# ShawnnnLiu/Robust-NeRF

Hardware: AMD Instinct MI355X
Metric: training rays/sec + test PSNR, lego 800² 64c+128f, at 1/2/4/8 MI355X (higher is better)
Workload: dtype bf16; 1 GPU; lego 800x800 hierarchical 64c+128f training step, 4096 rays per GPU; global_batch=4096, num_samples=64, num_samples_fine=128, parallelism=dp1

## Files before the change

include/nerf_hip.h:

```cpp
#ifndef NERF_HIP_H
#define NERF_HIP_H

#include <stddef.h>
#include <stdint.h>

#ifdef __cplusplus
extern "C" {
#endif

#define NR_OK 0
#define NR_EARG (-22)

typedef void* nr_stream_t;

const char* nr_last_error(void);
int nr_abi_version(void);
int nr_probe_fill(float* out, int n, float value, nr_stream_t stream);
int nr_probe_mfma(int kind, const float* A, const float* B, float* D,
                  nr_stream_t stream);

int nr_ray_directions(int H, int W, float focal, float cx, float cy,
                      float* dirs, nr_stream_t stream);

int nr_get_rays(const float* dirs, const float* c2w, int64_t N,
                float* rays_o, float* rays_d, nr_stream_t stream);
int64_t nr_get_rays_bwd_workspace_bytes(void);
int nr_get_rays_bwd(const float* dirs, const float* c2w, int64_t N,
                    const float* g_rays_o, const float* g_rays_d,
                    float* g_dirs, float* g_c2w, void* workspace,
                    nr_stream_t stream);

int nr_rays_from_pixels_fwd(const int64_t* img_idx, const float* pix,
                            const float* poses, int n_img, int H, int W,
                            float focal, int B, float* rays_o, float* rays_d,
                            int* bad_index, nr_stream_t stream);
int nr_rays_from_pixels_bwd(const int64_t* img_idx, const float* pix,
                            const float* poses, int n_img, int H, int W,
                            float focal, int B, const float* g_rays_o,
                            const float* g_rays_d, float* g_poses,
                            nr_stream_t stream);
int nr_check_index_range(const int64_t* idx, int n, int limit, int* flag,
                         nr_stream_t stream);

int nr_se3_poses_fwd(const float* init_poses, const float* rot_deltas,
                     const float* trans_deltas, const int64_t* indices, int n,
                     float* poses_out, nr_stream_t stream);
int nr_se3_poses_bwd(const float* init_poses, const float* rot_deltas,
                     const int64_t* indices, int n, int n_poses,
                     const float* g_poses,
                     int fixed_small_angle, float* g_rot, float* g_trans,
                     nr_stream_t stream);

int nr_gather_rays(const int64_t* idx, int64_t n_rays, int B,
                   const float* rays_o, const float* rays_d, const float* colors,
                   float* out_o, float* out_d, float* out_rgb, int* bad_index,
                   nr_stream_t stream);

int nr_gather_pixels(const int64_t* idx, int n_img, int H, int W,
                     const float* images, int B, int64_t* out_img,
                     float* out_pix, float* out_rgb, int* bad_index,
                     nr_stream_t stream);

int nr_stratified_sample(const float* rays_o, const float* rays_d,
                         const float* t_rand, float near_, float far_,
                         int lindisp, int B, int N, float* z_vals, float* pts,
                         float* viewdirs, nr_stream_t stream);

int nr_positional_encoding(const float* x, int64_t M, int C, int num_freqs,
                           int include_input, int log_sampling, float* out,
                           nr_stream_t stream);
int nr_positional_encoding_bwd(const float* x, int64_t M, int C, int num_freqs,
                               int include_input, int log_sampling,
                               const float* g_out, float* g_x,
                               nr_stream_t stream);

int nr_sample_pdf(const float* bins, const float* weights, const float* u,
                  int B, int Nb, int Ns, float* samples, nr_stream_t stream);

int nr_sample_hierarchical(const float* rays_o, const float* rays_d,
                           const float* z_coarse, const float* w_coarse,
                           const float* u, int B, int Nc, int Nf,
                           float* z_fine, float* pts_fine, float* viewdirs,
                           nr_stream_t stream);

int nr_composite_fwd(const float* rgb, const float* sigma, const float* z,
                     const float* rays_d, const float* sigma_noise, int B,
                     int S, int white_bg, float* rgb_map, float* depth_map,
                     float* acc_map, float* weights, nr_stream_t stream);
int nr_composite_bwd(const float* rgb, const float* sigma, const float* z,
                     const float* rays_d, const float* sigma_noise, int B,
                     int S, int white_bg, const float* g_rgb_map,
                     const float* g_depth, const float* g_acc,
                     const float* g_weights, float* g_rgb, float* g_sigma,
                     float* g_rays_d, nr_stream_t stream);

typedef struct NrMlpConfig {
    int pos_freqs;
    int dir_freqs;
    int hidden;
    int n_layers;
    uint32_t skip_mask;
    int use_view_dirs;
    int precision;
    int dense_backward;
} NrMlpConfig;

#define NR_PREC_FP32 0
#define NR_PREC_BF16 1
#define NR_PREC_FP16 2

int64_t nr_mlp_param_count(const NrMlpConfig* cfg);
int64_t nr_mlp_packed_bytes(const NrMlpConfig* cfg);
int64_t nr_mlp_saved_bytes(const NrMlpConfig* cfg, int64_t M);
int64_t nr_mlp_workspace_bytes(const NrMlpConfig* cfg, int64_t M);

int nr_mlp_pack(const NrMlpConfig* cfg, const float* params, void* packed,
                nr_stream_t stream);

int nr_mlp_forward(const NrMlpConfig* cfg, const void* packed,
                   const float* params, const float* x, const float* d,
                   int64_t M, float* rgb, float* sigma, void* saved,
                   nr_stream_t stream);

int nr_mlp_backward(const NrMlpConfig* cfg, const void* packed,
                    const float* params, const float* x, const float* d,
                    int64_t M, const float* rgb, const float* sigma,
                    const void* saved, const float* g_rgb,
                    const float* g_sigma, float* g_params, float* g_x,
                    float* g_d, void* workspace, nr_stream_t stream);

int nr_mlp_backward_dx(const NrMlpConfig* cfg, const void* packed,
                       const float* params, const float* x, const float* d,
                       int64_t M, const float* rgb, const float* sigma,
                       const void* saved, const float* g_rgb,
                       const float* g_sigma, float* g_x, float* g_d,
                       void* workspace, nr_stream_t stream);
int nr_mlp_backward_dw(const NrMlpConfig* cfg, int64_t M, const void* saved,
                       void* workspace, nr_stream_t stream);
int nr_mlp_backward_reduce(const NrMlpConfig* cfg, int64_t M,
                           const void* workspace, float* g_params,
                           nr_stream_t stream);
int64_t nr_mlp_active_tiles_offset(const NrMlpConfig* cfg, int64_t M);

int64_t nr_sumsq_workspace_bytes(void);
int nr_sumsq(const float* x, int64_t n, float* acc, void* workspace,
             nr_stream_t stream);
int nr_adam_step(float* params, float* grads, float* exp_avg,
                 float* exp_avg_sq, int64_t n, double lr, double beta1,
                 double beta2, double eps, int64_t step, const float* sumsq,
                 float max_norm, nr_stream_t stream);

int nr_sumsq_partials(const float* const* xs, const int64_t* ns, int nspan,
                      float* partials, nr_stream_t stream);
typedef struct NrAdamSpan {
    float* params;
    float* grads;
    float* exp_avg;
    float* exp_avg_sq;
    int64_t n;
    const float* sumsq_partials;
    float max_norm;
    const uint32_t* pack_table;
    void* packed;
} NrAdamSpan;
int nr_adam_multi(const NrAdamSpan* spans, int nspan, double lr, double beta1,
                  double beta2, double eps, int64_t step, const float* sched,
                  nr_stream_t stream);
int64_t nr_mlp_pack_table_bytes(const NrMlpConfig* cfg);
int nr_mlp_pack_table(const NrMlpConfig* cfg, uint32_t* table,
                      nr_stream_t stream);

int nr_expand_viewdirs(const float* rays_d, int B, int S, float* out,
                       nr_stream_t stream);
int nr_pts_bwd(const float* g_pts, const float* z, int B, int S,
               float* g_rays_o, float* g_rays_d, nr_stream_t stream);
int nr_viewdirs_bwd(const float* rays_d, const float* g_viewdirs, int B,
                    int S, float* g_rays_d, nr_stream_t stream);
int nr_mse_fwd_bwd(const float* pred, const float* target, int B, float scale,
                   float* loss_out, float* g_pred, nr_stream_t stream);
int64_t nr_composite_mse_workspace_bytes(int B);
int nr_composite_mse(const float* rgb, const float* sigma, const float* z,
                     const float* rays_d, const float* sigma_noise,
                     const float* target, int B, int S, int white,
                     float grad_scale, float* rgb_map, float* depth_map,
                     float* acc_map, float* weights, float* loss, float* g_rgb,
                     float* g_sigma, float* g_rays_d, uint32_t* ticket,
                     void* workspace, nr_stream_t stream);

int64_t nr_image_metrics_workspace_bytes(int H, int W, int C);
int nr_image_metrics(const float* pred, const float* target, int H, int W, int C,
                     const float* g, double C1, double C2, double* out,
                     void* workspace, nr_stream_t stream);
int nr_frame_u8(const float* src, int H, int W, int C, uint8_t* dst,
                int64_t dst_stride, int dst_x0, nr_stream_t stream);
int64_t nr_depth_frame_u8_workspace_bytes(void);
int nr_depth_frame_u8(const float* depth, int H, int W, uint8_t* dst,
                      void* workspace, nr_stream_t stream);

#ifdef __cplusplus
}
#endif

#endif
```

robust-nerf_amd/csrc/mlp.hip:

```cpp
#include <cmath>
#include <cstring>

#include "mlp_launch.hpp"

#include "mlp_plan.cpp.inc"

using namespace nr;

namespace {

bool plan_or_error(const NrMlpConfig* cfg, MlpPlan* p) {
    const char* why = "";
    if (!make_plan(cfg, p, &why)) {
        set_error("NrMlpConfig unsupported: %s", why);
        return false;
    }
    return true;
}

void add_stream_layer(StreamDesc& sd, int nchunks, int chunk_kb, int load_kb = -1) {
    for (int c = 0; c < nchunks && sd.nq < kMaxChunks; ++c) {
        sd.ckb[sd.nq] = load_kb < 0 ? chunk_kb : load_kb;
        sd.cadv[sd.nq++] = chunk_kb;
    }
}

}

extern "C" {

int64_t nr_mlp_param_count(const NrMlpConfig* cfg) {
    MlpPlan p;
    return plan_or_error(cfg, &p) ? p.param_count : -1;
}

int64_t nr_mlp_packed_bytes(const NrMlpConfig* cfg) {
    MlpPlan p;
    return plan_or_error(cfg, &p) ? p.packed_bytes : -1;
}

int64_t nr_mlp_saved_bytes(const NrMlpConfig* cfg, int64_t M) {
    MlpPlan p;
    if (!plan_or_error(cfg, &p) || M < 0) return -1;
    return make_sizes(p, M).saved_bytes;
}

int64_t nr_mlp_workspace_bytes(const NrMlpConfig* cfg, int64_t M) {
    MlpPlan p;
    if (!plan_or_error(cfg, &p) || M < 0) return -1;
    return make_sizes(p, M).ws_bytes;
}

int nr_mlp_pack(const NrMlpConfig* cfg, const float* params, void* packed, nr_stream_t stream) {
    MlpPlan p;
    if (!plan_or_error(cfg, &p)) return NR_EARG;
    NR_REQUIRE(params && packed, "nr_mlp_pack: null pointer");
    NR_REQUIRE((reinterpret_cast<uintptr_t>(packed) & 15) == 0, "nr_mlp_pack: packed must be 16-byte aligned");
    return launch_pack(p, params, packed, PackIdx{nullptr, 0}, false, static_cast<hipStream_t>(stream));
}

int64_t nr_mlp_pack_table_bytes(const NrMlpConfig* cfg) {
    MlpPlan p;
    return plan_or_error(cfg, &p) ? static_cast<int64_t>(kPackSlots) * p.param_count * 4 : -1;
}

int nr_mlp_pack_table(const NrMlpConfig* cfg, uint32_t* table, nr_stream_t stream) {
    MlpPlan p;
    if (!plan_or_error(cfg, &p)) return NR_EARG;
    NR_REQUIRE(table, "nr_mlp_pack_table: null pointer");
    NR_REQUIRE((reinterpret_cast<uintptr_t>(table) & 15) == 0, "nr_mlp_pack_table: table must be 16-byte aligned");
    NR_REQUIRE(p.packed_bytes < kDstMaxOff, "nr_mlp_pack_table: packed images beyond 512 MB");
    const hipStream_t s = static_cast<hipStream_t>(stream);
    hipError_t e = hipMemsetAsync(table, 0, static_cast<size_t>(kPackSlots) * p.param_count * 4, s);
    if (e != hipSuccess) {
        set_error("nr_mlp_pack_table: %s", hipGetErrorString(e));
        return static_cast<int>(e);
    }
    return launch_pack(p, nullptr, nullptr, PackIdx{table, p.param_count}, true, s);
}

int nr_adam_multi(const NrAdamSpan* spans, int nspan, double lr, double b1, double b2, double eps, int64_t step,
                  const float* sched, nr_stream_t stream) {
    NR_REQUIRE(spans && nspan >= 1 && nspan <= kMaxAdamSpans && step >= 1,
               "nr_adam_multi: bad arguments (1..%d spans, step >= 1)", kMaxAdamSpans);
    AdamMultiArgs a;
    std::memset(&a, 0, sizeof(a));
    int64_t nmax = 0;
    for (int k = 0; k < nspan; ++k) {
        const NrAdamSpan& x = spans[k];
        NR_REQUIRE(x.params && x.grads && x.exp_avg && x.exp_avg_sq && x.n >= 0, "nr_adam_multi: span %d: null buffer", k);
        NR_REQUIRE(((reinterpret_cast<uintptr_t>(x.params) | reinterpret_cast<uintptr_t>(x.grads) |
                     reinterpret_cast<uintptr_t>(x.exp_avg) | reinterpret_cast<uintptr_t>(x.exp_avg_sq) |
                     reinterpret_cast<uintptr_t>(x.pack_table)) & 15) == 0,
                   "nr_adam_multi: span %d: buffers must be 16-byte aligned", k);
        NR_REQUIRE(!x.pack_table || x.packed, "nr_adam_multi: span %d: pack_table without packed", k);
        a.s[k] = AdamSpanDev{x.params, x.grads, x.exp_avg, x.exp_avg_sq, x.n, x.sumsq_partials, x.max_norm,
                             x.pack_table, static_cast<char*>(x.packed)};
        nmax = x.n > nmax ? x.n : nmax;
    }
    if (nmax == 0) return NR_OK;
    const double bc1 = 1.0 - std::pow(b1, static_cast<double>(step));
    const double bc2 = 1.0 - std::pow(b2, static_cast<double>(step));
    a.omb1 = static_cast<float>(1.0 - b1);
    a.b2 = static_cast<float>(b2);
    a.omb2 = static_cast<float>(1.0 - b2);
    a.eps = static_cast<float>(eps);
    a.step_size = static_cast<float>(lr / bc1);
    a.bc2_sqrt = static_cast<float>(std::sqrt(bc2));
    a.sched = sched;
    const int grid = stream_grid(ceil_div_ll(nmax, 4), kSumsqThreads);
    return launch_adam_multi(a, grid, nspan, static_cast<hipStream_t>(stream));
}

int nr_mlp_forward(const NrMlpConfig* cfg, const void* packed, const float* params, const float* x, const float* d,
                   int64_t M, float* rgb, float* sigma, void* saved, nr_stream_t stream) {
    MlpPlan p;
    if (!plan_or_error(cfg, &p)) return NR_EARG;
    NR_REQUIRE(packed && params && x && rgb && sigma && M >= 0, "nr_mlp_forward: null pointer");
    NR_REQUIRE(!p.use_vd || d, "nr_mlp_forward: use_view_dirs needs d (model.py:187-191)");
    NR_REQUIRE((reinterpret_cast<uintptr_t>(saved) & 15) == 0, "nr_mlp_forward: saved must be 16-byte aligned");
    NR_REQUIRE((reinterpret_cast<uintptr_t>(packed) & 15) == 0, "nr_mlp_forward: packed must be 16-byte aligned");
    if (M == 0) return NR_OK;
    const MlpSizes z = make_sizes(p, M);
    const hipStream_t s = static_cast<hipStream_t>(stream);
    if (p.prec != NR_PREC_FP32) {
        RbmArgs r;
        std::memset(&r, 0, sizeof(r));
        r.packed = static_cast<const char*>(packed);
        r.params = params;
        r.x = x;
        r.d = d;
        r.rgb = rgb;
        r.sigma = sigma;
        r.saved = static_cast<char*>(saved);
        r.M = M;
        r.tiles = z.tiles;
        r.L = p.L;
        r.Ld = p.Ld;
        r.n_layers = p.n_layers;
        r.skips = p.skips;
        r.base = p.lin[0].pk_fwd;
        r.vhead = p.vhead;
        r.sig_b = p.sig_b;
        r.rgb_b = p.rgb_b;
        for (int t = 0; t < p.n_saved; ++t) r.sv_off[t] = z.saved_off[t];
        r.sv_feat = p.sv_feat;
        r.sv_denc = p.sv_denc;
        r.sv_hc = p.sv_hc;
        r.mask_off = z.mask_off;
        r.n_mask = p.n_mask;
        return launch_fwd_rbm(p, r, saved != nullptr, s);
    }
    FwdArgs a;
    std::memset(&a, 0, sizeof(a));
    a.packed = static_cast<const char*>(packed);
    a.params = params;
    a.x = x;
    a.d = d;
    a.rgb = rgb;
    a.sigma = sigma;
    a.saved = static_cast<char*>(saved);
    a.M = M;
    a.tiles = z.tiles;
    a.L = p.L;
    a.Ld = p.Ld;
    a.n_layers = p.n_layers;
    a.skips = p.skips;
    a.sd.base = p.lin[0].pk_fwd;
    for (int l = 0; l < p.n_lin; ++l) {
        const LinearDesc& dl = p.lin[l];
        add_stream_layer(a.sd, dl.KB, dl.NB * p.fpb);
        a.vb[l] = dl.vb;
        a.bo[l] = dl.b_off;
    }
    a.vsig = p.vsig;
    a.vrgb = p.vrgb;
    a.sig_b = p.sig_b;
    a.rgb_b = p.rgb_b;
    for (int t = 0; t < p.n_saved; ++t) a.sv_off[t] = z.saved_off[t];
    a.sv_feat = p.sv_feat;
    a.sv_denc = p.sv_denc;
    a.sv_hc = p.sv_hc;
    a.mask_off = z.mask_off;
    a.n_mask = p.n_mask;
    return launch_fwd(p, a, saved != nullptr, s);
}

int nr_mlp_backward_dx(const NrMlpConfig* cfg, const void* packed, const float* params, const float* x,
                       const float* d, int64_t M, const float* rgb, const float* sigma, const void* saved,
                       const float* g_rgb, const float* g_sigma, float* g_x, float* g_d, void* workspace,
                       nr_stream_t stream) {
    MlpPlan p;
    if (!plan_or_error(cfg, &p)) return NR_EARG;
    NR_REQUIRE(packed && params && x && rgb && sigma && saved && g_rgb && g_sigma && workspace && M >= 0,
               "nr_mlp_backward_dx: null pointer");
    NR_REQUIRE(!g_d || (d && p.use_vd), "nr_mlp_backward_dx: g_d needs d and use_view_dirs");
    NR_REQUIRE((reinterpret_cast<uintptr_t>(workspace) & 15) == 0,
               "nr_mlp_backward_dx: workspace must be 16-byte aligned");
    if (M == 0) return NR_OK;
    const hipStream_t s = static_cast<hipStream_t>(stream);
    const MlpSizes z = make_sizes(p, M);
    NR_REQUIRE(z.tiles_alloc < (int64_t{1} << 32), "nr_mlp_backward_dx: M beyond 2^37 samples");
    char* wsb = static_cast<char*>(workspace);
    uint8_t* tflags = reinterpret_cast<uint8_t*>(wsb + z.flags_off);
    uint32_t* blkcnt = reinterpret_cast<uint32_t*>(wsb + z.blkcnt_off);
    uint32_t* dwlist = reinterpret_cast<uint32_t*>(wsb + z.dwlist_off);
    uint32_t* tcount = reinterpret_cast<uint32_t*>(wsb + z.count_off);
    if (const int rc = launch_tile_flags(g_rgb, g_sigma, M, p.dense_bwd, z.nseg, tflags, blkcnt, s)) return rc;
    const int n = p.n_layers;
    if (p.prec != NR_PREC_FP32) {
        BwdrArgs r;
        std::memset(&r, 0, sizeof(r));
        r.gscale = grad_scale(p.prec);
        r.packed = static_cast<const char*>(packed);
        r.rgb = rgb;
        r.sigma = sigma;
        r.g_rgb = g_rgb;
        r.g_sigma = g_sigma;
        r.saved = static_cast<const char*>(saved);
        r.ws = wsb;
        r.M = M;
        r.tiles = z.tiles;
        r.flags = tflags;
        r.blk_count = blkcnt;
        r.nseg = z.nseg;
        r.dw_list = dwlist;
        r.count = tcount;
        r.scratch_base = z.tiles_alloc - kScratchTiles;
        r.n_layers = n;
        r.base = p.lin[n + 1].pk_bwdr;
        r.vrgb = p.vrgb;
        r.vhead = p.vhead;
        r.mask_off = z.mask_off;
        r.n_mask = p.n_mask;
        for (int t = 0; t < p.n_ws; ++t) r.ws_off[t] = z.ws_off[t];
        r.ws_feat = p.ws_feat;
        r.ws_dir = p.ws_dir;
        r.ws_heads = p.ws_heads;
        const int rc = launch_bwd_rbm(p, r, s);
        if (rc != NR_OK || !(g_x || g_d)) return rc;
        return input_grads16(p, z, r.packed, x, d, g_x, g_d, wsb, M, s);
    }
    const bool wx = g_x != nullptr || g_d != nullptr;
    BwdArgs b;
    std::memset(&b, 0, sizeof(b));
    b.packed = static_cast<const char*>(packed);
    b.gscale = grad_scale(p.prec);
    b.inv_gscale = 1.0f / b.gscale;
    b.params = params;
    b.x = x;
    b.d = d;
    b.rgb = rgb;
    b.sigma = sigma;
    b.g_rgb = g_rgb;
    b.g_sigma = g_sigma;
    b.g_x = g_x;
    b.g_d = g_d;
    b.saved = static_cast<const char*>(saved);
    b.ws = wsb;
    b.M = M;
    b.tiles = z.tiles;
    b.flags = tflags;
    b.blk_count = blkcnt;
    b.nseg = z.nseg;
    b.dw_list = dwlist;
    b.count = tcount;
    b.L = p.L;
    b.Ld = p.Ld;
    b.n_layers = n;
    b.skips = p.skips;
    auto add_T = [&](int l) {
        const bool partial = !wx && ((l > 0 && l < n && is_skip(p, l - 1)) || l == n + 1);
        add_stream_layer(b.sd, p.lin[l].NB, p.lin[l].KB * p.fpb, partial ? kHB * p.fpb : -1);
    };
    b.sd.base = p.lin[n + 1].pk_bwd;
    add_T(n + 1);
    add_T(n);
    for (int i = n - 1; i >= 1; --i) add_T(i);
    if (wx) add_T(0);
    b.vsig = p.vsig;
    b.vrgb = p.vrgb;
    b.mask_off = z.mask_off;
    b.n_mask = p.n_mask;
    for (int t = 0; t < p.n_ws; ++t) b.ws_off[t] = z.ws_off[t];
    b.ws_feat = p.ws_feat;
    b.ws_dir = p.ws_dir;
    b.ws_heads = p.ws_heads;
    if (!p.dense_bwd) {
        for (float* g : {g_x, g_d})
            if (g) {
                const hipError_t e = hipMemsetAsync(g, 0, sizeof(float) * 3 * static_cast<size_t>(M), s);
                if (e != hipSuccess) {
                    set_error("nr_mlp_backward_dx: %s", hipGetErrorString(e));
                    return static_cast<int>(e);
                }
            }
    }
    return launch_bwd(p, b, wx, s);
}

int nr_mlp_backward_dw(const NrMlpConfig* cfg, int64_t M, const void* saved, void* workspace, nr_stream_t stream) {
    MlpPlan p;
    if (!plan_or_error(cfg, &p)) return NR_EARG;
    NR_REQUIRE(saved && workspace && M >= 0, "nr_mlp_backward_dw: null pointer");
    NR_REQUIRE((reinterpret_cast<uintptr_t>(saved) & 15) == 0 && (reinterpret_cast<uintptr_t>(workspace) & 15) == 0,
               "nr_mlp_backward_dw: saved and workspace must be 16-byte aligned");
    if (M == 0) return NR_OK;
    const hipStream_t s = static_cast<hipStream_t>(stream);
    const MlpSizes z = make_sizes(p, M);
    const char* sv = static_cast<const char*>(saved);
    char* ws = static_cast<char*>(workspace);
    DwArgs w;
    std::memset(&w, 0, sizeof(w));
    w.slabs = reinterpret_cast<float*>(ws + z.slab_off);
    w.tiles = z.tiles;
    w.list = reinterpret_cast<const uint32_t*>(ws + z.dwlist_off);
    w.count = reinterpret_cast<const uint32_t*>(ws + z.count_off);
    w.njobs = p.n_jobs;
    int nwg = 0;
    NR_REQUIRE(p.n_jobs <= 32 && z.max_chunks < 2048, "nr_mlp_backward_dw: %d jobs x %d chunks beyond the map",
               p.n_jobs, z.max_chunks);
    for (int c = 0; c < z.max_chunks; ++c)
        for (int j = 0; j < p.n_jobs; ++j)
            if (c < z.job_chunks[j]) {
                NR_REQUIRE(nwg < kDwMaxWgs, "nr_mlp_backward_dw: more than %d workgroups", kDwMaxWgs);
                w.wg_map[nwg++] = static_cast<uint16_t>(j | c << 5);
            }
    for (int j = 0; j < p.n_jobs; ++j) w.job_chunks[j] = z.job_chunks[j];
    w.slab_floats_per_chunk = p.slab_floats_per_chunk;
    int max_blk = 0;
    for (int j = 0; j < p.n_jobs; ++j) {
        const DwJob& jb = p.job[j];
        w.job_NBz[j] = jb.NBz;
        w.job_KB[j] = jb.KB;
        for (int v = 0; v < kDwWaves; ++v) {
            if (v >= jb.nwaves) {
                w.job_wave[j][v] = 0;
                continue;
            }
            const DwWave& sh = jb.w[v];
            NR_REQUIRE(sh.np >= 1 && sh.np <= kDwMaxP && sh.nq >= 1 && sh.nq <= kDwMaxQ && sh.row0 >= 0 &&
                           sh.row0 + sh.np <= jb.NBz && sh.col0 >= 0 && sh.col0 + sh.nq <= jb.KB && jb.NBz < 64 &&
                           jb.KB < 64,
                       "nr_mlp_backward_dw: job %d wave %d share out of its %dx%d grid", j, v, jb.NBz, jb.KB);
            w.job_wave[j][v] = dw_wave_pack(sh.row0, sh.np, sh.col0, sh.nq, sh.bias);
        }
        int ns = 0;
        for (int q = 0; q < jb.ndz; ++q, ++ns) {
            w.seg_ptr[j][ns] = (jb.dz[q].is_ws ? ws : sv) + (jb.dz[q].is_ws ? z.ws_off : z.saved_off)[jb.dz[q].tensor];
            w.seg_blocks[j][ns] = static_cast<uint8_t>(jb.dz[q].blocks);
        }
        for (int q = 0; q < jb.nin; ++q, ++ns) {
            w.seg_ptr[j][ns] = (jb.in[q].is_ws ? ws : sv) + (jb.in[q].is_ws ? z.ws_off : z.saved_off)[jb.in[q].tensor];
            w.seg_blocks[j][ns] = static_cast<uint8_t>(jb.in[q].blocks);
        }
        w.job_slab[j] = jb.slab_off;
        NR_REQUIRE((jb.NBz + jb.KB) * p.fpb <= kDwWaves * dw_max_pieces(p.fpb == 2),
                   "nr_mlp_backward_dw: job %d stages %d blocks, beyond the kernel's per-wave pieces", j, jb.NBz + jb.KB);
        max_blk = jb.NBz + jb.KB > max_blk ? jb.NBz + jb.KB : max_blk;
    }
    w.stage_bytes = max_blk * p.fpb * kFragBytes;
    w.nstage = static_cast<int>((160 * 1024 - kFragBytes) / w.stage_bytes);
    if (w.nstage > NR_DW_NSTAGE) w.nstage = NR_DW_NSTAGE;
    size_t lds = static_cast<size_t>(w.nstage) * w.stage_bytes + kFragBytes;
    int min_chunks = z.job_chunks[0];
    for (int j = 1; j < p.n_jobs; ++j) min_chunks = z.job_chunks[j] < min_chunks ? z.job_chunks[j] : min_chunks;
    const size_t list_bytes = (static_cast<size_t>(ceil_div_ll(z.tiles, min_chunks)) * 4 + 15) / 16 * 16;
    if (lds + list_bytes <= 160 * 1024) {
        w.list_lds = static_cast<int>(lds);
        lds += list_bytes;
    }
    NR_REQUIRE(w.nstage >= 2, "nr_mlp_backward_dw: a %d-byte stage does not fit twice in LDS", w.stage_bytes);
    NR_REQUIRE(lds <= 160 * 1024, "nr_mlp_backward_dw: %zu bytes of LDS staging exceeds 160 KiB", lds);
    return launch_dw(p.prec, w, nwg, lds, s);
}

int nr_mlp_backward_reduce(const NrMlpConfig* cfg, int64_t M, const void* workspace, float* g_params,
                           nr_stream_t stream) {
    MlpPlan p;
    if (!plan_or_error(cfg, &p)) return NR_EARG;
    NR_REQUIRE(workspace && g_params && M >= 0, "nr_mlp_backward_reduce: null pointer");
    const hipStream_t s = static_cast<hipStream_t>(stream);
    if (M == 0) {
        (void)hipMemsetAsync(g_params, 0, sizeof(float) * p.param_count, s);
        return check_launch("nr_mlp_backward_reduce");
    }
    const MlpSizes z = make_sizes(p, M);
    ReduceArgs r;
    std::memset(&r, 0, sizeof(r));
    r.slabs = reinterpret_cast<const float*>(static_cast<const char*>(workspace) + z.slab_off);
    r.g = g_params;
    r.inv_gscale = 1.0f / grad_scale(p.prec);
    r.param_count = p.param_count;
    r.slab_floats_per_chunk = p.slab_floats_per_chunk;
    r.n_red = p.n_red;
    for (int k = 0; k < p.n_red; ++k) {
        const ReduceRange& rr = p.red[k];
        r.rows[k] = rr.rows;
        r.in[k] = rr.in;
        r.nseg[k] = rr.nseg;
        r.bjob[k] = rr.bjob;
        r.brow0[k] = rr.brow0;
        r.w_off[k] = rr.w_off;
        r.b_off[k] = rr.b_off;
        for (int q = 0; q < rr.nseg; ++q) r.seg[k][q] = rr.seg[q];
    }
    for (int j = 0; j < p.n_jobs; ++j) {
        r.job_slab[j] = p.job[j].slab_off;
        r.job_KB[j] = p.job[j].KB;
        r.job_chunks[j] = z.job_chunks[j];
    }
    int max_rows = 1;
    for (int k = 0; k < p.n_red; ++k) max_rows = p.red[k].rows > max_rows ? p.red[k].rows : max_rows;
    return launch_dw_reduce(r, max_rows, s);
}

int64_t nr_mlp_active_tiles_offset(const NrMlpConfig* cfg, int64_t M) {
    MlpPlan p;
    if (!plan_or_error(cfg, &p) || M <= 0) return -1;
    return make_sizes(p, M).count_off;
}

int nr_mlp_backward(const NrMlpConfig* cfg, const void* packed, const float* params, const float* x, const float* d,
                    int64_t M, const float* rgb, const float* sigma, const void* saved, const float* g_rgb,
                    const float* g_sigma, float* g_params, float* g_x, float* g_d, void* workspace,
                    nr_stream_t stream) {
    NR_REQUIRE(g_params, "nr_mlp_backward: null g_params");
    int rc = nr_mlp_backward_dx(cfg, packed, params, x, d, M, rgb, sigma, saved, g_rgb, g_sigma, g_x, g_d, workspace,
                                stream);
    if (rc) return rc;
    rc = nr_mlp_backward_dw(cfg, M, saved, workspace, stream);
    if (rc) return rc;
    return nr_mlp_backward_reduce(cfg, M, workspace, g_params, stream);
}

}
```

robust-nerf_amd/csrc/mlp_16.hip:

```cpp
#include <algorithm>
#include <cstring>

#include "mlp_dev.hpp"
#include "mlp_launch.hpp"

namespace nr {

#include "mlp_fwd_rbm.inc"
#include "mlp_bwd_rbm.inc"

struct DinArgs {
    const char* packed;
    const char* ws;
    const float* x;
    const float* d;
    float* g_x;
    float* g_d;
    int64_t M, tiles;
    const uint8_t* flags;
    int L, Ld;
    float inv_gscale;
    int nsrc;
    int64_t a_off[kMaxTrunk];
    int a_kb[kMaxTrunk];
    int a_p0[kMaxTrunk];
    int64_t dz_off[kMaxTrunk];
    int64_t dir_a_off, dz_dir_off;
    int dir_kb, dir_p0, nc;
};

constexpr int kDinNT = 512;

__host__ __device__ inline int din_frags(int nsrc, int XB, int DB, int nc) { return 2 * (nsrc * kHB * XB + nc * DB); }

template <int PREC, int XB, int DB, bool ALDS>
__global__ __launch_bounds__(kDinNT) void mlp_dinput_kernel(DinArgs a) {
    static_assert(k16<PREC>, "16-bit images only");
    extern __shared__ __attribute__((aligned(16))) char lds[];
    const int lane = threadIdx.x & 63, h = lane >> 5, ml = lane & 31;
    auto frag_src = [&](int f) -> const char* {
        const int nx = 2 * a.nsrc * kHB * XB;
        if (f < nx) {
            const int s = f / (2 * kHB * XB), r = f % (2 * kHB * XB);
            const int ob = r / (2 * XB), q = r % (2 * XB);
            return a.packed + a.a_off[s] + static_cast<int64_t>((ob * a.a_kb[s] + a.a_p0[s]) * 2 + q) * kFragBytes;
        }
        const int r = f - nx, ob = r / (2 * DB > 0 ? 2 * DB : 1), q = r % (2 * DB > 0 ? 2 * DB : 1);
        return a.packed + a.dir_a_off + static_cast<int64_t>((ob * a.dir_kb + a.dir_p0) * 2 + q) * kFragBytes;
    };
    if constexpr (ALDS) {
        const int nf = din_frags(a.nsrc, XB, DB, a.nc);
        for (int i = threadIdx.x; i < nf * 64; i += kDinNT) {
            const int f = i >> 6, l = i & 63;
            *reinterpret_cast<u32x4*>(lds + f * kFragBytes + l * 16) =
                *reinterpret_cast<const u32x4*>(frag_src(f) + l * 16);
        }
        __syncthreads();
    }
    auto afrag = [&](int f) -> bf16x8 {
        if constexpr (ALDS)
            return *reinterpret_cast<const bf16x8*>(lds + f * kFragBytes + lane * 16);
        else
            return *reinterpret_cast<const bf16x8*>(frag_src(f) + lane * 16);
    };
    const int64_t waves = static_cast<int64_t>(gridDim.x) * (kDinNT / 64);
    for (int64_t tile = static_cast<int64_t>(blockIdx.x) * (kDinNT / 64) + (threadIdx.x >> 6); tile < a.tiles;
         tile += waves) {
        const int64_t tile_u = __builtin_amdgcn_readfirstlane(static_cast<int>(tile));
        const int64_t m = tile * 32 + ml;
        const bool valid = m < a.M;
        if (!a.flags[tile_u]) {
            if (valid && h == 0)
#pragma unroll
                for (int c = 0; c < 3; ++c) {
                    if (a.g_x) a.g_x[3 * m + c] = 0.f;
                    if (a.g_d) a.g_d[3 * m + c] = 0.f;
                }
            continue;
        }
        if (a.g_x) {
            f32x16 dxe[XB];
#pragma unroll
            for (int q = 0; q < XB; ++q) zero(dxe[q]);
            for (int s = 0; s < a.nsrc; ++s) {
                InBlk<PREC> b[kHB];
#pragma unroll
                for (int ob = 0; ob < kHB; ++ob) load_img<PREC>(a.ws + a.dz_off[s], tile_u, kHB, ob, b[ob], lane);
#pragma unroll
                for (int ob = 0; ob < kHB; ++ob)
#pragma unroll
                    for (int q = 0; q < XB; ++q) {
                        const int f = ((s * kHB + ob) * XB + q) * 2;
                        dxe[q] = mfma16<PREC>(afrag(f), b[ob].s[0], dxe[q]);
                        dxe[q] = mfma16<PREC>(afrag(f + 1), b[ob].s[1], dxe[q]);
                    }
            }
            const PeRev pr = pe_rev(valid ? a.x[3 * m] : 0.f, valid ? a.x[3 * m + 1] : 0.f,
                                    valid ? a.x[3 * m + 2] : 0.f);
            float g0 = 0.f, g1 = 0.f, g2 = 0.f;
#pragma unroll
            for (int kb = 0; kb < XB; ++kb)
#pragma unroll
                for (int r = 0; r < 16; ++r)
                    pe_fast_bwd(pr, 32 * kb + acc_row(r, 0), 32 * kb + acc_row(r, 1), h != 0, a.L, dxe[kb][r], g0, g1,
                                g2);
            g0 += __shfl_xor(g0, 32);
            g1 += __shfl_xor(g1, 32);
            g2 += __shfl_xor(g2, 32);
            if (valid && h == 0) {
                a.g_x[3 * m] = g0 * a.inv_gscale;
                a.g_x[3 * m + 1] = g1 * a.inv_gscale;
                a.g_x[3 * m + 2] = g2 * a.inv_gscale;
            }
        }
        if constexpr (DB > 0) {
            if (a.g_d) {
                f32x16 dd[DB];
#pragma unroll
                for (int q = 0; q < DB; ++q) zero(dd[q]);
                const int f0 = 2 * a.nsrc * kHB * XB;
                for (int ob = 0; ob < a.nc; ++ob) {
                    InBlk<PREC> b;
                    load_img<PREC>(a.ws + a.dz_dir_off, tile_u, a.nc, ob, b, lane);
#pragma unroll
                    for (int q = 0; q < DB; ++q) {
                        const int f = f0 + (ob * DB + q) * 2;
                        dd[q] = mfma16<PREC>(afrag(f), b.s[0], dd[q]);
                        dd[q] = mfma16<PREC>(afrag(f + 1), b.s[1], dd[q]);
                    }
                }
                const PeRev pr = pe_rev(valid ? a.d[3 * m] : 0.f, valid ? a.d[3 * m + 1] : 0.f,
                                        valid ? a.d[3 * m + 2] : 0.f);
                float g0 = 0.f, g1 = 0.f, g2 = 0.f;
#pragma unroll
                for (int kb = 0; kb < DB; ++kb)
#pragma unroll
                    for (int r = 0; r < 16; ++r)
                        pe_fast_bwd(pr, 32 * kb + acc_row(r, 0), 32 * kb + acc_row(r, 1), h != 0, a.Ld, dd[kb][r], g0,
                                    g1, g2);
                g0 += __shfl_xor(g0, 32);
                g1 += __shfl_xor(g1, 32);
                g2 += __shfl_xor(g2, 32);
                if (valid && h == 0) {
                    a.g_d[3 * m] = g0 * a.inv_gscale;
                    a.g_d[3 * m + 1] = g1 * a.inv_gscale;
                    a.g_d[3 * m + 2] = g2 * a.inv_gscale;
                }
            }
        }
    }
}

namespace {

template <int PREC, bool TRAIN>
int launch_fwd_rbm_t(const MlpPlan& p, const RbmArgs& a, hipStream_t s) {
    constexpr int W = kRbmWaves;
    const dim3 grid(static_cast<unsigned>(ceil_div_ll(a.tiles, W))), block(W * 64);
    const size_t lds = rbm_lds_bytes(p.XB, W);
#define NR_FWDR(XB_, DB_)                                                                           \
    if (p.XB == XB_ && p.DB == DB_) {                                                               \
        hipLaunchKernelGGL((mlp_fwd_rbm_kernel<PREC, XB_, DB_, TRAIN, W>), grid, block, lds, s, a); \
        return check_launch("nr_mlp_forward");                                                      \
    }
    NR_FWDR(2, 1)
#ifndef NR_MLP_DEV
    NR_FWDR(2, 0)
    NR_FWDR(1, 1)
    NR_FWDR(1, 0)
#endif
#undef NR_FWDR
    set_error("nr_mlp_forward: no kernel instance for XB=%d DB=%d", p.XB, p.DB);
    return NR_EARG;
}

template <int PREC>
int launch_bwd_rbm_t(const MlpPlan& p, const BwdrArgs& a, hipStream_t s) {
    constexpr int W = kRbmWaves;
    const size_t lds = bwdr_lds_bytes(p.n_mask, W);
    if (lds > 160 * 1024) {
        set_error("nr_mlp_backward_dx: %zu bytes of LDS exceed 160 KiB", lds);
        return NR_EARG;
    }
    const dim3 grid(static_cast<unsigned>(a.nseg * (kSegTiles / W))), block(W * 64);
    hipLaunchKernelGGL((mlp_bwd_rbm_kernel<PREC, W>), grid, block, lds, s, a);
    return check_launch("nr_mlp_backward_dx");
}

template <int PREC>
int launch_dinput(const MlpPlan& p, const DinArgs& a, hipStream_t s) {
    const size_t lds = static_cast<size_t>(din_frags(a.nsrc, p.XB, p.DB, a.nc)) * kFragBytes;
    const bool alds = lds <= 160 * 1024;
    const dim3 grid(static_cast<unsigned>(std::min<int64_t>(ceil_div_ll(a.tiles, kDinNT / 64), 512))),
        block(kDinNT);
#define NR_DIN(XB_, DB_)                                                                                  \
    if (p.XB == XB_ && p.DB == DB_) {                                                                     \
        if (alds)                                                                                         \
            hipLaunchKernelGGL((mlp_dinput_kernel<PREC, XB_, DB_, true>), grid, block, lds, s, a);        \
        else                                                                                              \
            hipLaunchKernelGGL((mlp_dinput_kernel<PREC, XB_, DB_, false>), grid, block, 0, s, a);         \
        return check_launch("nr_mlp_backward_dx (input gradients)");                                     \
    }
    NR_DIN(2, 1)
#ifndef NR_MLP_DEV
    NR_DIN(2, 0)
    NR_DIN(1, 1)
    NR_DIN(1, 0)
#endif
#undef NR_DIN
    set_error("nr_mlp_backward_dx: no input-gradient kernel for XB=%d DB=%d", p.XB, p.DB);
    return NR_EARG;
}

}

int launch_fwd_rbm(const MlpPlan& p, const RbmArgs& a, bool train, hipStream_t s) {
    if (p.prec == NR_PREC_BF16)
        return train ? launch_fwd_rbm_t<NR_PREC_BF16, true>(p, a, s) : launch_fwd_rbm_t<NR_PREC_BF16, false>(p, a, s);
    return train ? launch_fwd_rbm_t<NR_PREC_FP16, true>(p, a, s) : launch_fwd_rbm_t<NR_PREC_FP16, false>(p, a, s);
}

int launch_bwd_rbm(const MlpPlan& p, const BwdrArgs& a, hipStream_t s) {
    return p.prec == NR_PREC_BF16 ? launch_bwd_rbm_t<NR_PREC_BF16>(p, a, s) : launch_bwd_rbm_t<NR_PREC_FP16>(p, a, s);
}

int input_grads16(const MlpPlan& p, const MlpSizes& z, const char* packed, const float* x, const float* d, float* g_x,
                  float* g_d, const char* ws, int64_t M, hipStream_t s) {
    const int n = p.n_layers;
    DinArgs da;
    std::memset(&da, 0, sizeof(da));
    da.packed = packed;
    da.ws = ws;
    da.flags = reinterpret_cast<const uint8_t*>(ws + z.flags_off);
    da.x = x;
    da.d = d;
    da.g_x = g_x;
    da.g_d = g_d;
    da.M = M;
    da.tiles = z.tiles;
    da.L = p.L;
    da.Ld = p.Ld;
    da.inv_gscale = 1.0f / grad_scale(p.prec);
    for (int l = 0; l < n; ++l) {
        if (l > 0 && !is_skip(p, l - 1)) continue;
        da.a_off[da.nsrc] = p.lin[l].pk_bwd;
        da.a_kb[da.nsrc] = p.lin[l].KB;
        da.a_p0[da.nsrc] = p.lin[l].KB - p.XB;
        da.dz_off[da.nsrc] = z.ws_off[WS_DZ0 + l];
        da.nsrc++;
    }
    da.dir_a_off = p.lin[n + 1].pk_bwd;
    da.dir_kb = p.lin[n + 1].KB;
    da.dir_p0 = kHB;
    da.nc = p.lin[n + 1].NB;
    da.dz_dir_off = z.ws_off[p.ws_dir];
    return p.prec == NR_PREC_BF16 ? launch_dinput<NR_PREC_BF16>(p, da, s) : launch_dinput<NR_PREC_FP16>(p, da, s);
}

}
```

robust-nerf_amd/csrc/mlp_bwd_rbm.inc:

```

constexpr int kBwdrSlot = 32 * 1024;
__host__ __device__ constexpr int bwdr_mask_off() { return 2 * kBwdrSlot; }
__host__ __device__ constexpr int bwdr_sig_off(int n_mask, int W) { return 2 * kBwdrSlot + W * n_mask * 1024; }
__host__ __device__ constexpr int bwdr_lds_bytes(int n_mask, int W) { return bwdr_sig_off(n_mask, W) + 1024; }

template <int PREC>
struct BwdrTrunkFin {
    InBlk<PREC> (&out)[kHB];
    u32x4 mw;
    char* dst;
    int64_t tile;
    int& nvm;
    bool sig;
    float dzs;
    const float* wsig;
    __device__ __forceinline__ void operator()(int rb, f32x16& a, const bf16x8&) const {
        if (sig)
#pragma unroll
            for (int g = 0; g < 4; ++g) {
                const f32x4 w = *reinterpret_cast<const f32x4*>(wsig + rb * 32 + 4 * g);
#pragma unroll
                for (int e = 0; e < 4; ++e) a[4 * g + e] = fmaf(w[e], dzs, a[4 * g + e]);
            }
        to_in_masked<PREC>(a, mw, rb, out[rb]);
        store_img<PREC>(dst, tile, kHB, rb, out[rb], 0);
        nvm += 2;
    }
};

template <int PREC>
struct BwdrFeatFin {
    InBlk<PREC> (&out)[kHB];
    char* dst;
    int64_t tile;
    int& nvm;
    __device__ __forceinline__ void operator()(int rb, f32x16& a, const bf16x8&) const {
        to_in<PREC>(a, out[rb]);
        store_img<PREC>(dst, tile, kHB, rb, out[rb], 0);
        nvm += 2;
    }
};

template <int PREC, int W>
__global__ __launch_bounds__(W * 64, 1) void mlp_bwd_rbm_kernel(BwdrArgs a) {
    static_assert(kSegTiles % W == 0, "whole parts per segment");
    extern __shared__ __attribute__((aligned(16))) char lds[];
    const int tid = threadIdx.x, lane = tid & 63, h = lane >> 5, ml = lane & 31;
    const int wv = __builtin_amdgcn_readfirstlane(tid >> 6);
    const TileSel ts = select_tile(a.flags, a.blk_count, a.nseg, a.tiles, W, wv);
    if (ts.idle) {
        finish_tiles(ts, a.nseg, a.tiles, a.dw_list, a.count);
        return;
    }
    const int64_t tile = ts.live ? ts.tile : a.scratch_base + ((blockIdx.x * W + wv) & (kScratchTiles - 1));
    const int64_t m = tile * 32 + ml;
    const bool valid = m < a.M;
    const int n = a.n_layers;
    constexpr int NC = kHB / 2;

    char* mlds = lds + bwdr_mask_off() + wv * a.n_mask * 1024;
    const char* msrc = a.saved + a.mask_off + tile * a.n_mask * 1024;
    for (int l = 0; l < a.n_mask; ++l)
        __builtin_amdgcn_global_load_lds((const __attribute__((address_space(1))) void*)(msrc + l * 1024 + lane16()),
                                         (__attribute__((address_space(3))) void*)(mlds + l * 1024), 16, 0, 0);
    if (wv == 0)
        __builtin_amdgcn_global_load_lds(
            (const __attribute__((address_space(1))) void*)(a.packed + a.vhead + lane16()),
            (__attribute__((address_space(3))) void*)(lds + bwdr_sig_off(a.n_mask, W)), 16, 0, 0);
    const u32x4 mwc = *reinterpret_cast<const u32x4*>(msrc + n * 1024 + lane16());
    auto mask_of = [&](int layer) { return *reinterpret_cast<const u32x4*>(mlds + layer * 1024 + lane16()); };
    const float* wsig = reinterpret_cast<const float*>(lds + bwdr_sig_off(a.n_mask, W)) + 16 * h;

    RStream s{lds, a.packed + a.base, -1, 0, wv, kBwdrSlot, W};
    constexpr int CK_DIR = rbm_chunk_kb(NC, 0), CK_H = rbm_chunk_kb(kHB, 0);
    static_assert(CK_DIR * 1024 <= kBwdrSlot && CK_H * 1024 <= kBwdrSlot, "dX chunk");
    rbm_dma(s, CK_DIR);
    s.q = 0;

    float dr[3] = {0.f, 0.f, 0.f}, dzs = 0.f;
    if (valid) {
#pragma unroll
        for (int c = 0; c < 3; ++c) {
            const float y = a.rgb[3 * m + c];
            dr[c] = ((a.g_rgb[3 * m + c] * (1.0f - y)) * y) * a.gscale;
        }
        dzs = (a.sigma[m] > 0.f ? a.g_sigma[m] : 0.f) * a.gscale;
    }
    {
        f32x16 hb;
        zero(hb);
        if (h == 0) {
            hb[0] = dzs;
            hb[1] = dr[0];
            hb[2] = dr[1];
            hb[3] = dr[2];
        }
        InBlk<PREC> hv;
        to_in<PREC>(hb, hv);
        store_img<PREC>(a.ws + a.ws_off[a.ws_heads], tile, 1, 0, hv, 0);
        s.nvm += 2;
    }
    InBlk<PREC> cin[NC];
    {
        const PImg wr0 = pimg(a.packed, a.vrgb), wr1 = pimg(a.packed, a.vrgb + NC * 128),
                   wr2 = pimg(a.packed, a.vrgb + 2 * NC * 128);
#pragma unroll
        for (int nb = 0; nb < NC; ++nb) {
            f32x16 dc;
#pragma unroll
            for (int r = 0; r < 16; ++r) {
                f32x2 v = wr0.at(nb, r) * bcast2(dr[0]);
                v = __builtin_elementwise_fma(wr1.at(nb, r), bcast2(dr[1]), v);
                v = __builtin_elementwise_fma(wr2.at(nb, r), bcast2(dr[2]), v);
                dc[r] = h ? v[1] : v[0];
            }
            to_in_masked<PREC>(dc, mwc, nb, cin[nb]);
            store_img<PREC>(a.ws + a.ws_off[a.ws_dir], tile, NC, nb, cin[nb], 0);
            s.nvm += 2;
        }
    }

    InBlk<PREC> hA[kHB], hB[kHB];
    {
        BwdrFeatFin<PREC> fin{hA, a.ws + a.ws_off[a.ws_feat], tile, s.nvm};
        auto in = [&](int kb) -> const InBlk<PREC>& { return cin[kb]; };
        rbm_layer<PREC, NC, kHB, 0, decltype(in), decltype(fin), 0>(s, CK_H, in, fin);
    }
    {
        BwdrTrunkFin<PREC> fin{hB, mask_of(n - 1), a.ws + a.ws_off[WS_DZ0 + n - 1], tile, s.nvm, true, dzs, wsig};
        auto in = [&](int kb) -> const InBlk<PREC>& { return hA[kb]; };
        rbm_layer<PREC, kHB, kHB, 0, decltype(in), decltype(fin), 0>(s, n > 1 ? CK_H : 0, in, fin);
    }
    auto trunk = [&](int i, InBlk<PREC>(&hin)[kHB], InBlk<PREC>(&hout)[kHB]) {
        BwdrTrunkFin<PREC> fin{hout, mask_of(i - 1), a.ws + a.ws_off[WS_DZ0 + i - 1], tile, s.nvm, false, 0.f, wsig};
        auto in = [&](int kb) -> const InBlk<PREC>& { return hin[kb]; };
        rbm_layer<PREC, kHB, kHB, 0, decltype(in), decltype(fin), 0>(s, i > 1 ? CK_H : 0, in, fin);
    };
    for (int i = n - 1; i >= 1; i -= 2) {
        trunk(i, hB, hA);
        if (i == 1) break;
        trunk(i - 1, hA, hB);
    }
    finish_tiles(ts, a.nseg, a.tiles, a.dw_list, a.count);
}
```

robust-nerf_amd/csrc/mlp_dev.hpp:

```cpp
#pragma once

#include <type_traits>
#include <utility>

#include "common.hpp"
#include "mfma.hpp"
#include "mlp_plan.hpp"

namespace nr {

template <int PREC>
constexpr bool k16 = PREC != NR_PREC_FP32;

template <int PREC>
struct InBlk {
    bf16x8 s[2];
};
template <>
struct InBlk<NR_PREC_FP32> {
    f32x16 v;
};

template <int PREC>
constexpr int kFPB = k16<PREC> ? 2 : 4;

typedef _Float16 f16x8 __attribute__((ext_vector_type(8)));
typedef _Float16 f16x2 __attribute__((ext_vector_type(2)));

template <int PREC>
__device__ __forceinline__ f32x16 mfma16(bf16x8 a, bf16x8 b, f32x16 c) {
    if constexpr (PREC == NR_PREC_FP16)
        return __builtin_amdgcn_mfma_f32_32x32x16_f16(__builtin_bit_cast(f16x8, a), __builtin_bit_cast(f16x8, b), c,
                                                      0, 0, 0);
    else
        return mfma_bf16(a, b, c);
}

typedef float f32x2 __attribute__((ext_vector_type(2)));
typedef __bf16 bf16x2 __attribute__((ext_vector_type(2)));
__device__ __forceinline__ unsigned cvt_pk_bf16(float lo, float hi) {
    return __builtin_bit_cast(unsigned, __builtin_convertvector(f32x2{lo, hi}, bf16x2));
}
template <int PREC>
__device__ __forceinline__ unsigned cvt_pk16(float lo, float hi) {
    if constexpr (PREC == NR_PREC_FP16)
        return __builtin_bit_cast(unsigned, __builtin_convertvector(f32x2{lo, hi}, f16x2));
    else
        return cvt_pk_bf16(lo, hi);
}
template <int PREC>
__device__ __forceinline__ float from16_lo(unsigned w) {
    if constexpr (PREC == NR_PREC_FP16)
        return static_cast<float>(__builtin_bit_cast(f16x2, w)[0]);
    else
        return __uint_as_float(w << 16);
}

template <int PREC = NR_PREC_BF16>
__device__ __forceinline__ bf16x8 pack8(const f32x16& a, int hf) {
    u32x4 w;
#pragma unroll
    for (int m = 0; m < 4; ++m) w[m] = cvt_pk16<PREC>(a[8 * hf + 2 * m], a[8 * hf + 2 * m + 1]);
    return __builtin_bit_cast(bf16x8, w);
}

template <int PREC>
__device__ __forceinline__ void to_in(const f32x16& a, InBlk<PREC>& o) {
    if constexpr (k16<PREC>) {
        o.s[0] = pack8<PREC>(a, 0);
        o.s[1] = pack8<PREC>(a, 1);
    } else {
        o.v = a;
    }
}

__device__ __forceinline__ void zero(f32x16& a) {
#pragma unroll
    for (int r = 0; r < 16; ++r) a[r] = 0.f;
}

#ifndef NR_SIN
#define NR_SIN sinf
#define NR_COS cosf
#endif
__device__ __forceinline__ uint32_t lane16() {
    uint32_t v;
    asm volatile("v_mbcnt_lo_u32_b32 %0, -1, 0\n\tv_mbcnt_hi_u32_b32 %0, -1, %0\n\tv_lshlrev_b32 %0, 4, %0" : "=v"(v));
    return v;
}

__device__ __forceinline__ float pe_feat(float x0, float x1, float x2, int f, int L) {
    if (f < 3) return f == 0 ? x0 : (f == 1 ? x1 : x2);
    const int fp = f - 3;
    const int k = fp / 6;
    if (k >= L) return 0.f;
    const int rem = fp - 6 * k;
    const int c = rem % 3;
    const float xv = c == 0 ? x0 : (c == 1 ? x1 : x2);
    const float v = exp2f(static_cast<float>(k)) * xv;
    return rem < 3 ? NR_SIN(v) : NR_COS(v);
}

__device__ __forceinline__ void pe_feat_bwd(float x0, float x1, float x2, int f, int L, float g, float& g0,
                                            float& g1, float& g2) {
    int c;
    float d;
    if (f < 3) {
        c = f;
        d = g;
    } else {
        const int fp = f - 3;
        const int k = fp / 6;
        if (k >= L) return;
        const int rem = fp - 6 * k;
        c = rem % 3;
        const float xv = c == 0 ? x0 : (c == 1 ? x1 : x2);
        const float fr = exp2f(static_cast<float>(k));
        const float v = fr * xv;
        d = rem < 3 ? (g * cosf(v)) * fr : (g * -sinf(v)) * fr;
    }
    g0 += c == 0 ? d : 0.f;
    g1 += c == 1 ? d : 0.f;
    g2 += c == 2 ? d : 0.f;
}

struct PeRev {
    float x[3], hi[3], lo[3];
};

__device__ __forceinline__ PeRev pe_rev(float x0, float x1, float x2) {
    constexpr float C1 = 0.15915494f, C2 = 6.4206382e-09f;
    PeRev p;
    const float xs[3] = {x0, x1, x2};
#pragma unroll
    for (int c = 0; c < 3; ++c) {
        p.x[c] = xs[c];
        p.hi[c] = xs[c] * C1;
        p.lo[c] = fmaf(xs[c], C1, -p.hi[c]) + xs[c] * C2;
    }
    return p;
}

__device__ __forceinline__ float pe_fast(const PeRev& p, int f0, int f1, bool h1, int L) {
    auto kind = [](int f) { return f < 3 ? 0 : 1; };
    auto trig = [&](int f, float& hi, float& lo) {
        const int fp = f - 3, k = fp / 6, rem = fp - 6 * k, c = rem % 3;
        const float sc = static_cast<float>(1 << (k < 24 ? k : 0));
        hi = p.hi[c] * sc;
        lo = fmaf(p.lo[c], sc, rem < 3 ? 0.f : 0.25f);
        return k < L;
    };
    if (kind(f0) == 1 && kind(f1) == 1) {
        float h0, l0, hh, lh;
        const bool v0 = trig(f0, h0, l0), v1 = trig(f1, hh, lh);
        const float hi = h1 ? hh : h0, lo = h1 ? lh : l0;
        const float v = __builtin_amdgcn_sinf(__builtin_amdgcn_fractf(hi) + lo);
        return (h1 ? v1 : v0) ? v : 0.f;
    }
    auto one = [&](int f) -> float {
        if (f < 3) return p.x[f];
        float hi, lo;
        const bool ok = trig(f, hi, lo);
        return ok ? __builtin_amdgcn_sinf(__builtin_amdgcn_fractf(hi) + lo) : 0.f;
    };
    const float a0 = one(f0), a1 = one(f1);
    return h1 ? a1 : a0;
}

__device__ __forceinline__ void pe_fast_bwd(const PeRev& p, int f0, int f1, bool h1, int L, float g, float& g0,
                                            float& g1, float& g2) {
    auto chan = [](int f) { return f < 3 ? f : ((f - 3) - 6 * ((f - 3) / 6)) % 3; };
    auto sel = [](const float (&v)[3], int c) { return c == 0 ? v[0] : (c == 1 ? v[1] : v[2]); };
    auto live = [&](int f) { return f < 3 || (f - 3) / 6 < L; };
    auto dgamma = [&](int f) -> float {
        const int fp = f - 3, k = fp / 6, rem = fp - 6 * k, c = rem % 3;
        const float sc = static_cast<float>(1 << (k < 24 ? k : 0));
        const float hi = sel(p.hi, c) * sc, lo = fmaf(sel(p.lo, c), sc, rem < 3 ? 0.25f : 0.5f);
        return __builtin_amdgcn_sinf(__builtin_amdgcn_fractf(hi) + lo) * sc;
    };
    float d;
    if (f0 >= 3 && f1 >= 3) {
        const int fp0 = f0 - 3, k0 = fp0 / 6, r0 = fp0 - 6 * k0;
        const int fp1 = f1 - 3, k1 = fp1 / 6, r1 = fp1 - 6 * k1;
        const float s0 = static_cast<float>(1 << (k0 < 24 ? k0 : 0)), s1 = static_cast<float>(1 << (k1 < 24 ? k1 : 0));
        const float hi = h1 ? sel(p.hi, r1 % 3) * s1 : sel(p.hi, r0 % 3) * s0;
        const float lo = h1 ? fmaf(sel(p.lo, r1 % 3), s1, r1 < 3 ? 0.25f : 0.5f) : fmaf(sel(p.lo, r0 % 3), s0, r0 < 3 ? 0.25f : 0.5f);
        d = g * (__builtin_amdgcn_sinf(__builtin_amdgcn_fractf(hi) + lo) * (h1 ? s1 : s0));
    } else {
        const float a0 = f0 < 3 ? 1.f : (live(f0) ? dgamma(f0) : 0.f);
        const float a1 = f1 < 3 ? 1.f : (live(f1) ? dgamma(f1) : 0.f);
        d = g * (h1 ? a1 : a0);
    }
    if (!(h1 ? live(f1) : live(f0))) return;
    const int c = h1 ? chan(f1) : chan(f0);
    g0 += c == 0 ? d : 0.f;
    g1 += c == 1 ? d : 0.f;
    g2 += c == 2 ? d : 0.f;
}

template <int PREC>
__device__ __forceinline__ bf16x8 bias_frag(float b) {
    const unsigned w0 = cvt_pk16<PREC>(b, 0.f);
    const float r1 = b - from16_lo<PREC>(w0);
    const unsigned w1 = cvt_pk16<PREC>(r1, 0.f);
    const float r2 = r1 - from16_lo<PREC>(w1);
    const unsigned w2 = cvt_pk16<PREC>(r2, 0.f);
    return __builtin_bit_cast(bf16x8, u32x4{w0 | (w1 << 16), w2, 0u, 0u});
}

template <int PREC>
__device__ __forceinline__ bf16x8 ones16() {
    const unsigned one = PREC == NR_PREC_FP16 ? 0x3C003C00u : 0x3F803F80u;
    return __builtin_bit_cast(bf16x8, u32x4{one, one, one, one});
}

typedef short s16x2 __attribute__((ext_vector_type(2)));
typedef unsigned short u16x2 __attribute__((ext_vector_type(2)));

__device__ __forceinline__ unsigned relu_pk(unsigned w) {
    return __builtin_bit_cast(unsigned, __builtin_elementwise_max(__builtin_bit_cast(s16x2, w), s16x2{0, 0}));
}
__device__ __forceinline__ unsigned nz_pk(unsigned w) {
    unsigned r;
    asm("v_pk_min_u16 %0, %1, %2" : "=v"(r) : "v"(w), "s"(0x10001u));
    return r;
}

template <int PREC, bool RELU, bool MASK>
__device__ __forceinline__ void epi16_blk(const f32x16& a, bf16x8 (&out)[2], unsigned* mw, int nb) {
#pragma unroll
    for (int hf = 0; hf < 2; ++hf) {
        u32x4 wd = __builtin_bit_cast(u32x4, pack8<PREC>(a, hf));
#pragma unroll
        for (int m = 0; m < 4; ++m) {
            if constexpr (RELU) wd[m] = relu_pk(wd[m]);
            if constexpr (MASK) mw[nb >> 1] |= nz_pk(wd[m]) << (8 * (nb & 1) + 4 * hf + m);
        }
        out[hf] = __builtin_bit_cast(bf16x8, wd);
    }
}

__device__ __forceinline__ void mask_pk(bf16x8 (&v)[2], unsigned word, int nb) {
#pragma unroll
    for (int hf = 0; hf < 2; ++hf) {
        u32x4 wd = __builtin_bit_cast(u32x4, v[hf]);
#pragma unroll
        for (int m = 0; m < 4; ++m) {
            const unsigned t = (word >> (8 * (nb & 1) + 4 * hf + m)) & 0x10001u;
            wd[m] &= t * 0xFFFFu;
        }
        v[hf] = __builtin_bit_cast(bf16x8, wd);
    }
}

template <int PREC>
__device__ __forceinline__ void to_in_masked(f32x16 a, const u32x4& mw, int nb, InBlk<PREC>& o) {
    if constexpr (k16<PREC>) {
        to_in<PREC>(a, o);
        mask_pk(o.s, mw[nb >> 1], nb);
    } else {
#pragma unroll
        for (int r = 0; r < 16; ++r) {
            const unsigned bit = (mw[nb >> 1] >> ((nb & 1) * 16 + r)) & 1u;
            a[r] = bit ? a[r] : 0.f;
        }
        o.v = a;
    }
}

template <int PREC>
__device__ __forceinline__ void store_img(char* __restrict__ region, int64_t tile, int nblk, int blk,
                                          const InBlk<PREC>& v, int) {
    char* base = region + ((tile * nblk + blk) * kFPB<PREC>) * static_cast<int64_t>(kFragBytes) + lane16();
    if constexpr (k16<PREC>) {
        __builtin_nontemporal_store(__builtin_bit_cast(u32x4, v.s[0]), reinterpret_cast<u32x4*>(base));
        __builtin_nontemporal_store(__builtin_bit_cast(u32x4, v.s[1]), reinterpret_cast<u32x4*>(base + kFragBytes));
    } else {
#pragma unroll
        for (int tq = 0; tq < 4; ++tq)
            *reinterpret_cast<f32x4*>(base + tq * kFragBytes) =
                f32x4{v.v[4 * tq], v.v[4 * tq + 1], v.v[4 * tq + 2], v.v[4 * tq + 3]};
    }
}

template <int PREC>
__device__ __forceinline__ void load_img(const char* __restrict__ region, int64_t tile, int nblk, int blk,
                                         InBlk<PREC>& v, int) {
    const char* base = region + ((tile * nblk + blk) * kFPB<PREC>) * static_cast<int64_t>(kFragBytes) + lane16();
    if constexpr (k16<PREC>) {
        v.s[0] = *reinterpret_cast<const bf16x8*>(base);
        v.s[1] = *reinterpret_cast<const bf16x8*>(base + kFragBytes);
    } else {
#pragma unroll
        for (int tq = 0; tq < 4; ++tq) {
            const f32x4 q = *reinterpret_cast<const f32x4*>(base + tq * kFragBytes);
#pragma unroll
            for (int e = 0; e < 4; ++e) v.v[4 * tq + e] = q[e];
        }
    }
}

typedef const __attribute__((address_space(4))) float cfloat;

struct VImg {
    cfloat* p;
    bool hi;
    __device__ __forceinline__ f32x4 g4(int nb, int g) const {
        f32x4 r;
#pragma unroll
        for (int e = 0; e < 4; ++e) {
            const float lo = p[(2 * nb) * 16 + 4 * g + e], up = p[(2 * nb + 1) * 16 + 4 * g + e];
            r[e] = hi ? up : lo;
        }
        return r;
    }
};

__device__ __forceinline__ VImg vimg(const char* packed, int64_t off, int lane) {
    const char* q = packed + off;
    asm volatile("" : "+s"(q));
    return VImg{(cfloat*)(q), (lane >> 5) != 0};
}
#define NR_VEC(img, nb, g) ((img).g4((nb), (g)))

typedef const __attribute__((address_space(4))) f32x2 cf32x2;
struct PImg {
    cf32x2* p;
    __device__ __forceinline__ f32x2 at(int nb, int r) const { return p[nb * 16 + r]; }
};
__device__ __forceinline__ PImg pimg(const char* packed, int64_t off) {
    const char* q = packed + off;
    asm volatile("" : "+s"(q));
    return PImg{(cf32x2*)(q)};
}
__device__ __forceinline__ f32x2 bcast2(float x) { return f32x2{x, x}; }
__device__ __forceinline__ float relu_f(float x) { return __int_as_float(max(__float_as_int(x), 0)); }

struct SegFlags {
    uint32_t word;
    int count, incl, total;
};
__device__ __forceinline__ uint32_t seg_flag_word(const uint8_t* __restrict__ flags, int64_t sg) {
    static_assert(kSegTiles == 4 * 64, "one flag word per lane");
    return reinterpret_cast<const uint32_t*>(flags + sg * kSegTiles)[threadIdx.x & 63];
}
__device__ __forceinline__ SegFlags seg_scan(uint32_t word) {
    const int lane = threadIdx.x & 63;
    SegFlags f;
    f.word = word;
    f.count = __popc(f.word);
    f.incl = f.count;
#pragma unroll
    for (int d = 1; d < 64; d <<= 1) {
        const int o = __shfl_up(f.incl, d);
        if (lane >= d) f.incl += o;
    }
    f.total = __builtin_amdgcn_readfirstlane(__shfl(f.incl, 63));
    return f;
}

__device__ __forceinline__ int64_t seg_entry(const SegFlags& f, int64_t sg, int k) {
    const uint64_t over = __ballot(f.incl > k);
    const int L = __builtin_ctzll(over);
    const uint32_t w = __builtin_amdgcn_readfirstlane(__shfl(f.word, L));
    int r = k - __builtin_amdgcn_readfirstlane(__shfl(f.incl - f.count, L));
    int b = 0;
#pragma unroll
    for (int q = 0; q < 4; ++q) {
        const bool set = (w >> (8 * q)) & 1u;
        if (set && r == 0) b = q;
        r -= set ? 1 : 0;
        if (r < 0) r = 1 << 20;
    }
    return sg * kSegTiles + 4 * L + b;
}

__device__ __forceinline__ void place_segment(const SegFlags& f, uint32_t before, int64_t nseg, int64_t sg,
                                              uint32_t* __restrict__ list, uint32_t* __restrict__ count) {
    const int lane = threadIdx.x & 63;
    uint32_t slot = before + static_cast<uint32_t>(f.incl - f.count);
#pragma unroll
    for (int q = 0; q < 4; ++q)
        if ((f.word >> (8 * q)) & 1u) list[slot++] = static_cast<uint32_t>(sg * kSegTiles + 4 * lane + q);
    if (sg == nseg - 1 && lane == 0) *count = before + static_cast<uint32_t>(f.total);
}

constexpr int64_t kDenseCheckSegs = 1024;

struct TileSel {
    SegFlags sf;
    int64_t seg, tile;
    uint32_t before;
    bool dense, live, idle, leader;
};
__device__ __forceinline__ TileSel select_tile(const uint8_t* __restrict__ flags,
                                               const uint32_t* __restrict__ blk_count, int64_t nseg,
                                               int64_t tiles, int W, int wv) {
    constexpr int BPS = kSegTiles / 64;
    const int lane = threadIdx.x & 63;
    const int64_t b = blockIdx.x;
    TileSel t;
    const int part = static_cast<int>(b / nseg);
    t.seg = (b % nseg + nseg - part % nseg) % nseg;
    static_assert(BPS == 4, "a segment's block counts are one uint4");
    const bool check = nseg <= kDenseCheckSegs;
    const int64_t lim = check ? nseg : (part == 0 && wv == 0 ? t.seg : 0);
    const uint32_t word = seg_flag_word(flags, t.seg);
    const uint4* __restrict__ bc4 = reinterpret_cast<const uint4*>(blk_count);
    uint32_t all = 0, before = 0;
    for (int64_t s0 = 0; s0 < lim; s0 += 4 * 64) {
        uint4 c[4];
#pragma unroll
        for (int i = 0; i < 4; ++i) {
            const int64_t sg = s0 + i * 64 + lane;
            c[i] = sg < lim ? bc4[sg] : uint4{0u, 0u, 0u, 0u};
        }
#pragma unroll
        for (int i = 0; i < 4; ++i) {
            const uint32_t n = ((c[i].x + c[i].y) + c[i].z) + c[i].w;
            all += n;
            before += (s0 + i * 64 + lane) < t.seg ? n : 0u;
        }
    }
    t.sf = seg_scan(word);
#pragma unroll
    for (int d = 32; d > 0; d >>= 1) {
        all += __shfl_xor(all, d);
        before += __shfl_xor(before, d);
    }
    t.before = __builtin_amdgcn_readfirstlane(before);
    t.dense = check && static_cast<int64_t>(__builtin_amdgcn_readfirstlane(all)) == tiles;
    if (t.dense) {
        const int64_t first = b * W;
        t.tile = first + wv;
        t.live = t.tile < tiles;
        t.idle = first >= tiles;
        t.leader = b == 0 && wv == 0;
    } else {
        const int k = part * W + wv;
        t.idle = part * W >= t.sf.total;
        t.live = k < t.sf.total;
        t.tile = t.live ? seg_entry(t.sf, t.seg, k) : 0;
        t.leader = part == 0 && wv == 0;
    }
    return t;
}

__device__ __forceinline__ void finish_tiles(const TileSel& t, int64_t nseg, int64_t tiles, uint32_t* __restrict__ list,
                                             uint32_t* __restrict__ count) {
    if (!t.leader) return;
    if (t.dense) {
        if ((threadIdx.x & 63) == 0) *count = static_cast<uint32_t>(tiles);
    } else {
        place_segment(t.sf, t.before, nseg, t.seg, list, count);
    }
}

template <int... Js, class F>
__device__ __forceinline__ void rbm_static_for(std::integer_sequence<int, Js...>, F&& f) {
    (f(std::integral_constant<int, Js>{}), ...);
}
template <int NN, class F>
__device__ __forceinline__ void rbm_static_for(F&& f) {
    rbm_static_for(std::make_integer_sequence<int, NN>{}, f);
}

}
```

robust-nerf_amd/csrc/mlp_dw.hip:

```cpp
#include "mlp_dev.hpp"
#include "mlp_launch.hpp"

namespace nr {

constexpr int kTileFlagThreads = 256;

__global__ __launch_bounds__(kTileFlagThreads) void tile_flags_kernel(const float* __restrict__ g_rgb,
                                                                      const float* __restrict__ g_sigma, int64_t M,
                                                                      int dense,
                                                                      uint8_t* __restrict__ flags,
                                                                      uint32_t* __restrict__ blk_count) {
    __shared__ uint32_t wcnt[kTileFlagThreads / 64];
    const int lane = threadIdx.x & 63, wv = threadIdx.x >> 6;
    const int64_t tw = static_cast<int64_t>(blockIdx.x) * 64 + wv * 16;
    bool nz[8];
#pragma unroll
    for (int it = 0; it < 8; ++it) {
        const int64_t m = (tw + 2 * it + (lane >> 5)) * 32 + (lane & 31);
        bool v = false;
        if (m < M) {
            if (dense) {
                v = true;
            } else {
                const float r0 = g_rgb[3 * m], r1 = g_rgb[3 * m + 1], r2 = g_rgb[3 * m + 2], s0 = g_sigma[m];
                v = (r0 != 0.f) | (r1 != 0.f) | (r2 != 0.f) | (s0 != 0.f);
            }
        }
        nz[it] = v;
    }
    uint32_t mask = 0;
#pragma unroll
    for (int it = 0; it < 8; ++it) {
        const uint64_t b = __ballot(nz[it]);
        mask |= (static_cast<uint32_t>(b & 0xffffffffull) != 0 ? 1u : 0u) << (2 * it);
        mask |= (static_cast<uint32_t>(b >> 32) != 0 ? 1u : 0u) << (2 * it + 1);
    }
    if (lane < 16) flags[tw + lane] = static_cast<uint8_t>((mask >> lane) & 1u);
    if (lane == 0) wcnt[wv] = __popc(mask);
    __syncthreads();
    if (threadIdx.x == 0) blk_count[blockIdx.x] = ((wcnt[0] + wcnt[1]) + wcnt[2]) + wcnt[3];
}

#ifndef NR_DW_AUX
#define NR_DW_AUX 0
#endif

__device__ __forceinline__ int dw_feat(int r) { return acc_row(r & 15, r >> 4); }

__device__ __forceinline__ int dw_slot(int L, int s) { return L ^ (((L >> 5) & 1) << 2) ^ (s << 3); }
__device__ __forceinline__ int dw_slot32(int L, int f) { return L ^ (2 * (f + 4 * ((L >> 5) & 1))); }

template <int OFF>
__device__ __forceinline__ void tr16(uint64_t& out, uint32_t addr) {
    asm volatile("ds_read_b64_tr_b16 %0, %1 offset:%2" : "=v"(out) : "v"(addr), "i"(OFF));
}

typedef unsigned long long u64x2_t __attribute__((ext_vector_type(2)));
template <int OFF>
__device__ __forceinline__ void ds_rd32(float& out, uint32_t addr) {
    asm volatile("ds_read_b32 %0, %1 offset:%2" : "=v"(out) : "v"(addr), "i"(OFF));
}

__device__ __forceinline__ bf16x8 tr_pair(uint64_t lo, uint64_t hi) {
    return __builtin_bit_cast(bf16x8, u64x2_t{lo, hi});
}

__device__ __forceinline__ uint32_t dw_tr_off(int ks, int half, int lane) {
    const int g = lane >> 4, h = g & 1, hh = g >> 1;
    const int lam = lane & 15, q = lam >> 2, p = lam & 3;
    const int s = p >> 1;
    const int L = 16 * ks + 8 * hh + q + 32 * h + 4 * half;
    return static_cast<uint32_t>(s * kFragBytes + dw_slot(L, s) * 16 + 8 * (p & 1));
}

template <int PREC>
__device__ __forceinline__ float dw_acc4(uint64_t v, float acc) {
    const unsigned w0 = static_cast<unsigned>(v), w1 = static_cast<unsigned>(v >> 32);
    if constexpr (PREC == NR_PREC_FP16) {
        typedef _Float16 h2 __attribute__((ext_vector_type(2)));
        const h2 one = __builtin_bit_cast(h2, 0x3c003c00u);
        acc = __builtin_amdgcn_fdot2(__builtin_bit_cast(h2, w0), one, acc, false);
        return __builtin_amdgcn_fdot2(__builtin_bit_cast(h2, w1), one, acc, false);
    } else {
        typedef __bf16 b2 __attribute__((ext_vector_type(2)));
        const b2 one = __builtin_bit_cast(b2, 0x3f803f80u);
        acc = __builtin_amdgcn_fdot2_f32_bf16(__builtin_bit_cast(b2, w0), one, acc, false);
        return __builtin_amdgcn_fdot2_f32_bf16(__builtin_bit_cast(b2, w1), one, acc, false);
    }
}

template <int PREC>
__global__ __launch_bounds__(kDwThreads, 1) void mlp_dw_kernel(DwArgs a) {
    extern __shared__ __attribute__((aligned(16))) char lds[];
    const int tid = threadIdx.x, lane = tid & 63;
    const int wv = __builtin_amdgcn_readfirstlane(tid >> 6);
    const int wmap = a.wg_map[blockIdx.x];
    const int j = wmap & 31, chunk = wmap >> 5;
    const int NBz = a.job_NBz[j], KB = a.job_KB[j];
    const int winfo = a.job_wave[j][wv];
    const int row0 = winfo & 63, np = (winfo >> 6) & 7, col0 = (winfo >> 9) & 63, nq = (winfo >> 15) & 3;
    const bool active = np > 0;
    const bool do_bias = active && ((winfo >> 17) & 1);
    const int64_t cnt = *a.count;
    const int64_t tpc = (cnt + a.job_chunks[j] - 1) / a.job_chunks[j];
    const int64_t t0 = static_cast<int64_t>(chunk) * tpc;
    int64_t t1 = t0 + tpc;
    if (t1 > cnt) t1 = cnt;
    constexpr int FPB = kFPB<PREC>;
    constexpr int BLK = FPB * kFragBytes;

    const int total = (NBz + KB) * FPB;
    const int per_wave = (total + kDwWaves - 1) / kDwWaves;
    constexpr int kMaxPW = dw_max_pieces(k16<PREC>);
    const char* psrc[kMaxPW];
    int64_t pstride[kMaxPW];
    int pdst[kMaxPW];
#pragma unroll
    for (int k = 0; k < kMaxPW; ++k) {
        psrc[k] = nullptr;
        pstride[k] = 0;
        pdst[k] = -1;
        if (k < per_wave) {
            int pc = wv + k * kDwWaves;
            const bool pad = pc >= total;
            if (pad) pc = 0;
            int sg = 0, p0 = 0;
            while (pc >= p0 + a.seg_blocks[j][sg] * FPB) p0 += a.seg_blocks[j][sg++] * FPB;
            const int nb = a.seg_blocks[j][sg];
            const int L = k16<PREC> ? dw_slot(lane, (pc - p0) % FPB) : dw_slot32(lane, (pc - p0) % FPB);
            pstride[k] = static_cast<int64_t>(nb) * BLK;
            psrc[k] = a.seg_ptr[j][sg] + (pc - p0) * kFragBytes + L * 16;
            pdst[k] = pad ? -1 : pc * kFragBytes;
        }
    }
    const uint32_t* lds_list = nullptr;
    if (a.list_lds && cnt != a.tiles) {
        uint32_t* dst = reinterpret_cast<uint32_t*>(lds + a.list_lds);
        for (int64_t q = t0 + tid; q < t1; q += kDwThreads) dst[q - t0] = a.list[q];
        __syncthreads();
        lds_list = dst;
    }
    const bool ident = cnt == a.tiles;
    const uint32_t list_base = static_cast<uint32_t>(reinterpret_cast<uintptr_t>(lds_list));
    auto tile_at = [&](int64_t pos) -> int64_t {
        if (ident) return pos;
        if (!lds_list) return a.list[pos];
        uint32_t v;
        asm volatile("ds_read_b32 %0, %1\n\ts_waitcnt lgkmcnt(0)"
                     : "=v"(v)
                     : "v"(list_base + 4u * static_cast<uint32_t>(pos - t0))
                     : "memory");
        return __builtin_amdgcn_readfirstlane(v);
    };
    auto stage = [&](int b, int64_t tile) {
        char* dst = lds + b * a.stage_bytes;
        char* scratch = lds + a.nstage * a.stage_bytes;
#pragma unroll
        for (int k = 0; k < kMaxPW; ++k) {
            if (k < per_wave) {
                char* d = pdst[k] < 0 ? scratch : dst + pdst[k];
                __builtin_amdgcn_global_load_lds(
                    (const __attribute__((address_space(1))) void*)(psrc[k] + tile * pstride[k]),
                    (__attribute__((address_space(3))) void*)(d), 16, 0, NR_DW_AUX);
            }
        }
    };
    auto wait_pieces = [](int n) {
        switch (n) {
            case 4: asm volatile("s_waitcnt vmcnt(4)" ::: "memory"); break;
            case 5: asm volatile("s_waitcnt vmcnt(5)" ::: "memory"); break;
            case 8: asm volatile("s_waitcnt vmcnt(8)" ::: "memory"); break;
            case 10: asm volatile("s_waitcnt vmcnt(10)" ::: "memory"); break;
            default: asm volatile("s_waitcnt vmcnt(0)" ::: "memory"); break;
        }
    };

    uint32_t trof[2][2];
#pragma unroll
    for (int ks = 0; ks < 2; ++ks)
#pragma unroll
        for (int hf = 0; hf < 2; ++hf) trof[ks][hf] = dw_tr_off(ks, hf, lane);
    const int NS = a.nstage;
    float* slab = a.slabs + static_cast<int64_t>(chunk) * a.slab_floats_per_chunk + a.job_slab[j];
    const int ld = KB * 32 + 1;
    const int hl = lane >> 5, ml = lane & 31;

    using std::integral_constant;
    auto run = [&](auto npc, auto nqc) {
        constexpr int NP = decltype(npc)::value, NQ = decltype(nqc)::value;
        f32x16 acc[NP][NQ];
#pragma unroll
        for (int p = 0; p < NP; ++p)
#pragma unroll
            for (int q = 0; q < NQ; ++q) zero(acc[p][q]);
        float bsum[NP];
#pragma unroll
        for (int p = 0; p < NP; ++p) bsum[p] = 0.f;
        bool nval[NP], kval[NQ];
#pragma unroll
        for (int p = 0; p < NP; ++p) nval[p] = p < np;
#pragma unroll
        for (int q = 0; q < NQ; ++q) kval[q] = q < nq;

        for (int k = 0; k < NS - 1; ++k)
            if (t0 + k < t1) stage(k, tile_at(t0 + k));
        int bcur = 0, bnext = NS - 1;
        for (int64_t t = t0; t < t1; ++t) {
            int64_t ahead = t1 - 1 - t;
            if (ahead > NS - 2) ahead = NS - 2;
            wait_pieces(per_wave * static_cast<int>(ahead));
            asm volatile("s_waitcnt lgkmcnt(0)" ::: "memory");
            __builtin_amdgcn_s_barrier();
            if (t + NS - 1 < t1) stage(bnext, tile_at(t + NS - 1));
            bnext = bnext + 1 == NS ? 0 : bnext + 1;
            const char* buf = lds + bcur * a.stage_bytes;
            bcur = bcur + 1 == NS ? 0 : bcur + 1;
            if (!active) continue;
            if constexpr (k16<PREC>) {
                const uint32_t base = static_cast<uint32_t>(reinterpret_cast<uintptr_t>(buf));
                const uint32_t bufA = base + row0 * BLK, bufB = base + (NBz + col0) * BLK;
#pragma unroll
                for (int ks = 0; ks < 2; ++ks) {
                    uint64_t ra[NP][2], rb[NQ][2];
#pragma unroll
                    for (int hf = 0; hf < 2; ++hf) {
                        const uint32_t oa = bufA + trof[ks][hf], ob = bufB + trof[ks][hf];
                        rbm_static_for<NP>(
                            [&](auto pp) { tr16<decltype(pp)::value * BLK>(ra[decltype(pp)::value][hf], oa); });
                        rbm_static_for<NQ>(
                            [&](auto qq) { tr16<decltype(qq)::value * BLK>(rb[decltype(qq)::value][hf], ob); });
                    }
                    asm volatile("s_waitcnt lgkmcnt(0)" ::: "memory");
#pragma unroll
                    for (int hf = 0; hf < 2; ++hf) {
#pragma unroll
                        for (int p = 0; p < NP; ++p) asm volatile("" : "+v"(ra[p][hf]));
#pragma unroll
                        for (int q = 0; q < NQ; ++q) asm volatile("" : "+v"(rb[q][hf]));
                    }
                    bf16x8 A[NP], Bm[NQ];
#pragma unroll
                    for (int p = 0; p < NP; ++p) A[p] = tr_pair(ra[p][0], ra[p][1]);
#pragma unroll
                    for (int q = 0; q < NQ; ++q) Bm[q] = tr_pair(rb[q][0], rb[q][1]);
#pragma unroll
                    for (int p = 0; p < NP; ++p)
#pragma unroll
                        for (int q = 0; q < NQ; ++q) acc[p][q] = mfma16<PREC>(A[p], Bm[q], acc[p][q]);
                    if (do_bias)
#pragma unroll
                        for (int p = 0; p < NP; ++p) bsum[p] = dw_acc4<PREC>(ra[p][1], dw_acc4<PREC>(ra[p][0], bsum[p]));
                }
            } else {
                const int r = lane & 31, kk = lane >> 5;
                const int hh = r >> 4, i = r & 15;
                const int k2 = (i >> 2) + 4 * hh;
                const uint32_t base = static_cast<uint32_t>(reinterpret_cast<uintptr_t>(buf)) +
                                      ((i >> 2) * 64 + 32 * hh + kk) * 16 + (i & 3) * 4;
                const uint32_t bufA = base + row0 * BLK, bufB = base + (NBz + col0) * BLK;
                const uint32_t kx = static_cast<uint32_t>(k2) << 5;
                float Ar[2][NP], Br[2][NQ];
                auto rd = [&](auto sc) {
                    constexpr int ss = decltype(sc)::value;
                    uint32_t o;
                    asm volatile("v_xor_b32 %0, %1, %2" : "=v"(o) : "i"(ss << 5), "v"(kx));
                    const uint32_t oa = bufA + o, ob = bufB + o;
                    rbm_static_for<NP>([&](auto pp) { ds_rd32<decltype(pp)::value * BLK>(Ar[ss & 1][decltype(pp)::value], oa); });
                    rbm_static_for<NQ>([&](auto qq) { ds_rd32<decltype(qq)::value * BLK>(Br[ss & 1][decltype(qq)::value], ob); });
                };
                rd(integral_constant<int, 0>{});
                rbm_static_for<16>([&](auto sc) {
                    constexpr int ss = decltype(sc)::value;
                    if constexpr (ss + 1 < 16) {
                        rd(integral_constant<int, ss + 1>{});
                        asm volatile("s_waitcnt lgkmcnt(%0)" ::"n"(NP + NQ) : "memory");
                    } else {
                        asm volatile("s_waitcnt lgkmcnt(0)" ::: "memory");
                    }
#pragma unroll
                    for (int p = 0; p < NP; ++p) asm volatile("" : "+v"(Ar[ss & 1][p]));
#pragma unroll
                    for (int q = 0; q < NQ; ++q) asm volatile("" : "+v"(Br[ss & 1][q]));
#pragma unroll
                    for (int p = 0; p < NP; ++p) {
                        bsum[p] += Ar[ss & 1][p];
#pragma unroll
                        for (int q = 0; q < NQ; ++q) acc[p][q] = mfma_f32(Ar[ss & 1][p], Br[ss & 1][q], acc[p][q]);
                    }
                });
            }
        }
        if (!active) return;
#pragma unroll
        for (int p = 0; p < NP; ++p) {
            if (!nval[p]) continue;
#pragma unroll
            for (int q = 0; q < NQ; ++q) {
                if (!kval[q]) continue;
#pragma unroll
                for (int r = 0; r < 16; ++r) {
                    const int row = 32 * (row0 + p) + dw_feat(acc_row(r, hl));
                    const int col = 32 * (col0 + q) + dw_feat(ml);
                    slab[static_cast<int64_t>(row) * ld + col] = acc[p][q][r];
                }
            }
            if (do_bias) {
                const float tot = bsum[p] + __shfl_xor(bsum[p], 32);
                if (hl == 0) slab[static_cast<int64_t>(32 * (row0 + p) + dw_feat(ml)) * ld + KB * 32] = tot;
            }
        }
    };
    if constexpr (!k16<PREC>) {
        run(integral_constant<int, 4>{}, integral_constant<int, kDwMaxQ>{});
    } else {
        if (np <= 1)
            run(integral_constant<int, 1>{}, integral_constant<int, 2>{});
        else if (np <= 4 && nq <= 1)
            run(integral_constant<int, 4>{}, integral_constant<int, 1>{});
        else if (np <= 4)
            run(integral_constant<int, 4>{}, integral_constant<int, 2>{});
        else
            run(integral_constant<int, kDwMaxP>{}, integral_constant<int, kDwMaxQ>{});
    }
}

__global__ void mlp_dw_reduce_kernel(ReduceArgs a) {
    const int k = blockIdx.y, r = blockIdx.x;
    if (r >= a.rows[k]) return;
    const int in = a.in[k];
    const int64_t st = a.slab_floats_per_chunk;
    for (int c = threadIdx.x; c <= in; c += blockDim.x) {
        int job = -1, row = 0, col = 0;
        int64_t dst;
        if (c < in) {
            for (int q = 0; q < a.nseg[k]; ++q) {
                const RedSeg& sg = a.seg[k][q];
                if (c >= sg.col0 && c < sg.col0 + sg.width) {
                    job = sg.job;
                    row = sg.slab_row0 + r;
                    col = sg.slab_col0 + (c - sg.col0);
                }
            }
            dst = a.w_off[k] + static_cast<int64_t>(r) * in + c;
        } else {
            job = a.bjob[k];
            row = a.brow0[k] + r;
            col = a.job_KB[job] * 32;
            dst = a.b_off[k] + r;
        }
        if (job < 0) continue;
        const int ld = a.job_KB[job] * 32 + 1;
        const float* s = a.slabs + a.job_slab[job] + static_cast<int64_t>(row) * ld + col;
        const int nch = a.job_chunks[job];
        float acc = 0.f;
        int ch = 0;
        for (; ch + 4 <= nch; ch += 4) {
            const float v0 = s[ch * st], v1 = s[(ch + 1) * st], v2 = s[(ch + 2) * st], v3 = s[(ch + 3) * st];
            acc = (((acc + v0) + v1) + v2) + v3;
        }
        for (; ch < nch; ++ch) acc += s[ch * st];
        a.g[dst] = acc * a.inv_gscale;
    }
}

int launch_tile_flags(const float* g_rgb, const float* g_sigma, int64_t M, int dense, int64_t nseg, uint8_t* flags,
                      uint32_t* blk_count, hipStream_t s) {
    hipLaunchKernelGGL(tile_flags_kernel, dim3(static_cast<unsigned>(nseg * (kSegTiles / 64))), dim3(kTileFlagThreads),
                       0, s, g_rgb, g_sigma, M, dense, flags, blk_count);
    return check_launch("nr_mlp_backward_dx (tile flags)");
}

int launch_dw(int prec, const DwArgs& a, int nwg, size_t lds, hipStream_t s) {
    const dim3 grid(static_cast<unsigned>(nwg)), block(kDwThreads);
    if (prec == NR_PREC_BF16)
        hipLaunchKernelGGL(mlp_dw_kernel<NR_PREC_BF16>, grid, block, lds, s, a);
    else if (prec == NR_PREC_FP16)
        hipLaunchKernelGGL(mlp_dw_kernel<NR_PREC_FP16>, grid, block, lds, s, a);
    else
        hipLaunchKernelGGL(mlp_dw_kernel<NR_PREC_FP32>, grid, block, lds, s, a);
    return check_launch("nr_mlp_backward_dw");
}

int launch_dw_reduce(const ReduceArgs& a, int max_rows, hipStream_t s) {
    hipLaunchKernelGGL(mlp_dw_reduce_kernel, dim3(static_cast<unsigned>(max_rows), static_cast<unsigned>(a.n_red)),
                       dim3(256), 0, s, a);
    return check_launch("nr_mlp_backward_reduce");
}

}
```

robust-nerf_amd/csrc/mlp_fp32.hip:

```cpp
#include "mlp_dev.hpp"
#include "mlp_launch.hpp"

namespace nr {

constexpr int kNT = 256;
constexpr int TPW = 1;
constexpr int kFP = NR_PREC_FP32;
typedef InBlk<kFP> Blk;
constexpr int kFPB32 = kFPB<kFP>;

template <int NBO, bool RELU>
__device__ __forceinline__ void bias_act(f32x16 (&acc)[NBO], const VImg& bias, unsigned (&w)[4]) {
#pragma unroll
    for (int q = 0; q < 4; ++q) w[q] = 0u;
#pragma unroll
    for (int nb = 0; nb < NBO; ++nb) {
#pragma unroll
        for (int g = 0; g < 4; ++g) {
            const f32x4 b = NR_VEC(bias, nb, g);
#pragma unroll
            for (int e = 0; e < 4; ++e) {
                const int r = 4 * g + e;
                float v = acc[nb][r] + b[e];
                if (RELU) v = v > 0.f ? v : 0.f;
                acc[nb][r] = v;
                w[nb >> 1] |= (v > 0.f ? 1u : 0u) << ((nb & 1) * 16 + r);
            }
        }
    }
}

struct Ring {
    char* lds;
    int slot_bytes;
    int q;
    const char* src;
    int wv;
};

#ifndef NR_APF
#define NR_APF 3
#endif

struct Stager {
    __device__ __forceinline__ void load(Ring& ring, const StreamDesc& sd, int q) {
        if (q >= sd.nq) return;
        load_sized(ring, q, sd.ckb[q], sd.cadv[q]);
    }
    __device__ __forceinline__ void load_sized(Ring& ring, int q, int ckb, int cadv) {
        const int bytes = ckb * 1024;
        char* slot = ring.lds + (q & 1) * ring.slot_bytes;
        const uint32_t l16 = lane16();
        for (int pc = ring.wv; pc * 1024 < bytes; pc += kNT / 64)
            __builtin_amdgcn_global_load_lds(
                (const __attribute__((address_space(1))) void*)(ring.src + pc * 1024 + l16),
                (__attribute__((address_space(3))) void*)(slot + pc * 1024), 16, 0, 0);
        ring.src += cadv * 1024;
    }

    __device__ __forceinline__ void wait(int after = 0) {
        switch (after) {
            case 2: asm volatile("s_waitcnt vmcnt(2)" ::: "memory"); break;
            case 4: asm volatile("s_waitcnt vmcnt(4)" ::: "memory"); break;
            case 8: asm volatile("s_waitcnt vmcnt(8)" ::: "memory"); break;
            default: asm volatile("s_waitcnt vmcnt(0)" ::: "memory"); break;
        }
    }
};

template <int NBLK>
struct Act {
    Blk v[TPW][NBLK];
    __device__ __forceinline__ Blk operator()(int t, int kb) const { return v[t][kb]; }
    __device__ __forceinline__ void put(int t, int nb, const Blk& x) { v[t][nb] = x; }
};

struct Sink {
    char* region;
    int nblk;
    int64_t tile0;
    unsigned tok;
    __device__ __forceinline__ void operator()(int t, int kb, const Blk& v) const {
        if (region != nullptr && ((tok >> t) & 1u)) store_img(region, tile0 + t, nblk, kb, v, 0);
    }
    __device__ __forceinline__ int stores() const {
        return region == nullptr ? 0 : kFPB32 * __builtin_popcount(tok & ((1u << TPW) - 1u));
    }
};

__device__ __forceinline__ void stream_barrier() {
    asm volatile("s_waitcnt lgkmcnt(0)" ::: "memory");
    __builtin_amdgcn_s_barrier();
    asm volatile("" ::: "memory");
}

__device__ __forceinline__ void ds_read_quad(f32x4 (&dst)[4], uint32_t addr) {
    asm volatile("ds_read_b128 %0, %1" : "=v"(dst[0]) : "v"(addr));
    asm volatile("ds_read_b128 %0, %1 offset:1024" : "=v"(dst[1]) : "v"(addr));
    asm volatile("ds_read_b128 %0, %1 offset:2048" : "=v"(dst[2]) : "v"(addr));
    asm volatile("ds_read_b128 %0, %1 offset:3072" : "=v"(dst[3]) : "v"(addr));
}
__device__ __forceinline__ void lgkm_wait_one(int n, f32x4& a) {
    switch (n) {
        case 0: asm volatile("s_waitcnt lgkmcnt(0)" : "+v"(a)); break;
        case 1: asm volatile("s_waitcnt lgkmcnt(1)" : "+v"(a)); break;
        case 2: asm volatile("s_waitcnt lgkmcnt(2)" : "+v"(a)); break;
        case 3: asm volatile("s_waitcnt lgkmcnt(3)" : "+v"(a)); break;
        case 4: asm volatile("s_waitcnt lgkmcnt(4)" : "+v"(a)); break;
        case 5: asm volatile("s_waitcnt lgkmcnt(5)" : "+v"(a)); break;
        case 6: asm volatile("s_waitcnt lgkmcnt(6)" : "+v"(a)); break;
        default: asm volatile("s_waitcnt lgkmcnt(7)" : "+v"(a)); break;
    }
}

template <int N1, int N2, int KBN, class Src>
__device__ __forceinline__ void stream_gemm(f32x16 (&acc1)[TPW][N1 > 0 ? N1 : 1],
                                            f32x16 (&acc2)[TPW][N2 > 0 ? N2 : 1], int nb0, const Src& src,
                                            Ring& ring, Stager& st, const StreamDesc& sd,
                                            const Sink& sink = Sink{nullptr, 0, 0, 0u}) {
    const int q0 = ring.q;
    const int ckb_this = sd.ckb[q0], adv_this = sd.cadv[q0];
    const bool has_next = q0 + KBN < sd.nq;
    const int ckb_next = has_next ? sd.ckb[q0 + KBN] : 0, adv_next = has_next ? sd.cadv[q0 + KBN] : 0;
#pragma unroll
    for (int kb = 0; kb < KBN; ++kb) {
        if (kb < KBN - 1)
            st.load_sized(ring, ring.q + 1, ckb_this, adv_this);
        else if (has_next)
            st.load_sized(ring, ring.q + 1, ckb_next, adv_next);
        asm volatile("" ::: "memory");
        const char* slot = ring.lds + (ring.q & 1) * ring.slot_bytes + lane16();
        Blk in[TPW];
#pragma unroll
        for (int t = 0; t < TPW; ++t) in[t] = src(t, kb);
        constexpr int NRB = N1 + N2;
        const uint32_t abase = static_cast<uint32_t>(reinterpret_cast<uintptr_t>(slot)) +
                               static_cast<uint32_t>(nb0 * kFPB32 * kFragBytes);
        f32x4 aq[2][4];
        if constexpr (NR_APF > 0) ds_read_quad(aq[0], abase);
#pragma unroll
        for (int t = 0; t < TPW; ++t) sink(t, kb, in[t]);
#pragma unroll
        for (int r = 0; r < NRB; ++r) {
            const char* fp = slot + (nb0 + r) * kFPB32 * kFragBytes;
            constexpr int I2 = N2 > 0 ? N2 : 1;
            const int r1 = r < N1 ? r : 0;
            const int r2 = r >= N1 ? (r - N1) % I2 : 0;
            if constexpr (NR_APF > 0)
                if (r + 1 < NRB) ds_read_quad(aq[(r + 1) & 1], abase + (r + 1) * 4 * kFragBytes);
#pragma unroll
            for (int tq = 0; tq < 4; ++tq) {
                f32x4 a;
                if constexpr (NR_APF > 0) {
                    a = aq[r & 1][tq];
                    lgkm_wait_one((r + 1 < NRB ? 4 : 0) + 3 - tq, a);
                } else {
                    a = *reinterpret_cast<const f32x4*>(fp + tq * kFragBytes);
                }
#pragma unroll
                for (int e = 0; e < 4; ++e)
#pragma unroll
                    for (int t = 0; t < TPW; ++t) {
                        if (r < N1)
                            acc1[t][r1] = mfma_f32(a[e], in[t].v[4 * tq + e], acc1[t][r1]);
                        else
                            acc2[t][r2] = mfma_f32(a[e], in[t].v[4 * tq + e], acc2[t][r2]);
                    }
            }
        }
        st.wait(sink.stores());
        stream_barrier();
        ++ring.q;
    }
}

__device__ __forceinline__ void stream_begin(Ring& ring, Stager& st, const char* __restrict__ packed,
                                             const StreamDesc& sd) {
    ring.q = 0;
    ring.src = packed + sd.base;
    st.load(ring, sd, 0);
    st.wait();
    __syncthreads();
}

template <int XB, int DB, bool TRAIN>
__global__ __launch_bounds__(kNT, 1) void mlp_fwd_kernel(FwdArgs a) {
    extern __shared__ __attribute__((aligned(16))) char lds[];
    const int tid = threadIdx.x, lane = tid & 63, h = lane >> 5, ml = lane & 31;
    const int wv = __builtin_amdgcn_readfirstlane(tid >> 6);
    const int64_t tile0 = (static_cast<int64_t>(blockIdx.x) * (kNT / 64) + wv) * TPW;
    const int n = a.n_layers;
    float px[TPW][3];
    bool tok[TPW];
#pragma unroll
    for (int t = 0; t < TPW; ++t) {
        const int64_t m = (tile0 + t) * 32 + ml;
        tok[t] = tile0 + t < a.tiles;
        const bool valid = m < a.M;
        px[t][0] = valid ? a.x[3 * m] : 0.f;
        px[t][1] = valid ? a.x[3 * m + 1] : 0.f;
        px[t][2] = valid ? a.x[3 * m + 2] : 0.f;
    }
    u32x4* masks = reinterpret_cast<u32x4*>(a.saved + a.mask_off);
    unsigned tokm = 0u;
#pragma unroll
    for (int t = 0; t < TPW; ++t) tokm |= (tok[t] ? 1u : 0u) << t;
    auto sink_of = [&](int sv, int nblk) {
        return Sink{TRAIN ? a.saved + a.sv_off[sv] : nullptr, nblk, tile0, tokm};
    };

    Ring ring{lds, a.slot_bytes, 0, nullptr, wv};
    Stager st;
    stream_begin(ring, st, a.packed, a.sd);

    f32x16 acc[TPW][kHB];
    Act<kHB> hin;
    f32x16 dummy[TPW][1];
    unsigned w[TPW][4];
    for (int i = 0; i < n; ++i) {
#pragma unroll
        for (int t = 0; t < TPW; ++t)
#pragma unroll
            for (int nb = 0; nb < kHB; ++nb) zero(acc[t][nb]);
        const bool skip_in = i > 0 && ((a.skips >> (i - 1)) & 1u);
        if (i == 0 || skip_in) {
            Act<XB> xe;
#pragma unroll
            for (int t = 0; t < TPW; ++t) {
                if (TRAIN && i > 0) {
#pragma unroll
                    for (int kb = 0; kb < XB; ++kb) {
                        if (tok[t])
                            load_img(a.saved + a.sv_off[SV_XENC], tile0 + t, XB, kb, xe.v[t][kb], lane);
                        else
                            xe.v[t][kb] = Blk{};
                    }
                    continue;
                }
                float p0 = px[t][0], p1 = px[t][1], p2 = px[t][2];
                asm volatile("" : "+v"(p0), "+v"(p1), "+v"(p2));
#pragma unroll
                for (int kb = 0; kb < XB; ++kb) {
                    f32x16 v;
#pragma unroll
                    for (int r = 0; r < 16; ++r) v[r] = pe_feat(p0, p1, p2, 32 * kb + acc_row(r, h), a.L);
                    Blk o;
                    to_in(v, o);
                    if constexpr (TRAIN)
                        if (tok[t]) store_img(a.saved + a.sv_off[SV_XENC], tile0 + t, XB, kb, o, lane);
#pragma unroll
                    for (int k2 = 0; k2 < XB; ++k2)
                        if (k2 == kb) xe.v[t][k2] = o;
                }
            }
            stream_gemm<kHB, 0, XB>(acc, dummy, 0, xe, ring, st, a.sd);
        }
        if (i > 0) stream_gemm<kHB, 0, kHB>(acc, dummy, 0, hin, ring, st, a.sd, sink_of(SV_H0 + i - 1, kHB));
#pragma unroll
        for (int t = 0; t < TPW; ++t) {
            bias_act<kHB, true>(acc[t], vimg(a.packed, a.vb[i], lane), w[t]);
#pragma unroll
            for (int nb = 0; nb < kHB; ++nb) {
                Blk v;
                to_in(acc[t][nb], v);
                hin.put(t, nb, v);
            }
            if constexpr (TRAIN)
                if (tok[t]) masks[((tile0 + t) * a.n_mask + i) * 64 + lane] = u32x4{w[t][0], w[t][1], w[t][2], w[t][3]};
        }
    }

    float sp[TPW];
    {
        const PImg ws = pimg(a.packed, a.vsig);
#pragma unroll
        for (int t = 0; t < TPW; ++t) {
            f32x2 s2 = {0.f, 0.f};
#pragma unroll
            for (int nb = 0; nb < kHB; ++nb)
#pragma unroll
                for (int r = 0; r < 16; ++r)
                    s2 = __builtin_elementwise_fma(bcast2(relu_f(acc[t][nb][r])), ws.at(nb, r), s2);
            sp[t] = h ? s2[1] : s2[0];
        }
#pragma unroll
        for (int t = 0; t < TPW; ++t) {
            sp[t] += __shfl_xor(sp[t], 32);
            sp[t] = sp[t] + a.params[a.sig_b];
            sp[t] = sp[t] > 0.f ? sp[t] : 0.f;
        }
    }

#pragma unroll
    for (int t = 0; t < TPW; ++t)
#pragma unroll
        for (int nb = 0; nb < kHB; ++nb) zero(acc[t][nb]);
    stream_gemm<kHB, 0, kHB>(acc, dummy, 0, hin, ring, st, a.sd, sink_of(SV_H0 + n - 1, kHB));
#pragma unroll
    for (int t = 0; t < TPW; ++t) {
        bias_act<kHB, false>(acc[t], vimg(a.packed, a.vb[n], lane), w[t]);
#pragma unroll
        for (int nb = 0; nb < kHB; ++nb) {
            Blk v;
            to_in(acc[t][nb], v);
            hin.put(t, nb, v);
        }
    }

    constexpr int NC = kHB / 2;
    f32x16 ac[TPW][NC];
#pragma unroll
    for (int t = 0; t < TPW; ++t)
#pragma unroll
        for (int nb = 0; nb < NC; ++nb) zero(ac[t][nb]);
    stream_gemm<NC, 0, kHB>(ac, dummy, 0, hin, ring, st, a.sd, sink_of(a.sv_feat, kHB));
    if constexpr (DB > 0) {
        Act<DB> de;
#pragma unroll
        for (int t = 0; t < TPW; ++t) {
            const int64_t m = (tile0 + t) * 32 + ml;
            const bool valid = m < a.M;
            const float d0 = valid ? a.d[3 * m] : 0.f, d1 = valid ? a.d[3 * m + 1] : 0.f,
                        d2 = valid ? a.d[3 * m + 2] : 0.f;
#pragma unroll
            for (int kb = 0; kb < DB; ++kb) {
                f32x16 v;
#pragma unroll
                for (int r = 0; r < 16; ++r) v[r] = pe_feat(d0, d1, d2, 32 * kb + acc_row(r, h), a.Ld);
                to_in(v, de.v[t][kb]);
                if constexpr (TRAIN)
                    if (tok[t]) store_img(a.saved + a.sv_off[a.sv_denc], tile0 + t, DB, kb, de.v[t][kb], lane);
            }
        }
        stream_gemm<NC, 0, DB>(ac, dummy, 0, de, ring, st, a.sd);
    }
#pragma unroll
    for (int t = 0; t < TPW; ++t) {
        bias_act<NC, true>(ac[t], vimg(a.packed, a.vb[n + 1], lane), w[t]);
        if constexpr (TRAIN) {
            if (tok[t]) {
#pragma unroll
                for (int nb = 0; nb < NC; ++nb) {
                    Blk v;
                    to_in(ac[t][nb], v);
                    store_img(a.saved + a.sv_off[a.sv_hc], tile0 + t, NC, nb, v, lane);
                }
                masks[((tile0 + t) * a.n_mask + n) * 64 + lane] = u32x4{w[t][0], w[t][1], w[t][2], w[t][3]};
            }
        }
        float pr[3];
#pragma unroll
        for (int c = 0; c < 3; ++c) {
            const PImg wr = pimg(a.packed, a.vrgb + c * NC * 128);
            f32x2 s2 = {0.f, 0.f};
#pragma unroll
            for (int nb = 0; nb < NC; ++nb)
#pragma unroll
                for (int r = 0; r < 16; ++r) s2 = __builtin_elementwise_fma(bcast2(ac[t][nb][r]), wr.at(nb, r), s2);
            float s = h ? s2[1] : s2[0];
            s += __shfl_xor(s, 32);
            s = s + a.params[a.rgb_b + c];
            pr[c] = 1.0f / (1.0f + expf(-s));
        }
        const int64_t m = (tile0 + t) * 32 + ml;
        if (m < a.M && h == 0) {
            a.rgb[3 * m] = pr[0];
            a.rgb[3 * m + 1] = pr[1];
            a.rgb[3 * m + 2] = pr[2];
            a.sigma[m] = sp[t];
        }
    }
}

template <int XB, int DB, bool WANT_X>
__global__ __launch_bounds__(kNT, 1) void mlp_bwd_kernel(BwdArgs a) {
    extern __shared__ __attribute__((aligned(16))) char lds[];
    const int tid = threadIdx.x, lane = tid & 63, h = lane >> 5, ml = lane & 31;
    const int wv = __builtin_amdgcn_readfirstlane(tid >> 6);
    static_assert(TPW == 1, "the active-tile selection gives each wave one tile");
    const TileSel ts = select_tile(a.flags, a.blk_count, a.nseg, a.tiles, kNT / 64, wv);
    if (ts.idle) {
        finish_tiles(ts, a.nseg, a.tiles, a.dw_list, a.count);
        return;
    }
    const bool live = ts.live;
    const int64_t tile0 = live ? ts.tile : 0;
    const int n = a.n_layers;
    const u32x4* masks = reinterpret_cast<const u32x4*>(a.saved + a.mask_off);
    bool tok[TPW];
#pragma unroll
    for (int t = 0; t < TPW; ++t) tok[t] = live;
    auto store_dz = [&](int wsid, int nblk, int t, int nb, const Blk& v) {
        if (tok[t]) store_img(a.ws + a.ws_off[wsid], tile0 + t, nblk, nb, v, lane);
    };
    auto mask_of = [&](int t, int layer) -> u32x4 {
        return tok[t] ? masks[((tile0 + t) * a.n_mask + layer) * 64 + lane] : u32x4{0u, 0u, 0u, 0u};
    };

    Ring ring{lds, a.slot_bytes, 0, nullptr, wv};
    Stager st;
    stream_begin(ring, st, a.packed, a.sd);

    constexpr int NC = kHB / 2;
    float dzs[TPW];
    Act<NC> cin;
#pragma unroll
    for (int t = 0; t < TPW; ++t) {
        const int64_t m = (tile0 + t) * 32 + ml;
        const bool valid = tok[t] && m < a.M;
        float dr[3] = {0.f, 0.f, 0.f};
        dzs[t] = 0.f;
        if (valid) {
#pragma unroll
            for (int c = 0; c < 3; ++c) {
                const float y = a.rgb[3 * m + c];
                dr[c] = ((a.g_rgb[3 * m + c] * (1.0f - y)) * y) * a.gscale;
            }
            dzs[t] = (a.sigma[m] > 0.f ? a.g_sigma[m] : 0.f) * a.gscale;
        }
        if (tok[t]) {
            f32x16 hb;
            zero(hb);
            if (h == 0) {
                hb[0] = dzs[t];
                hb[1] = dr[0];
                hb[2] = dr[1];
                hb[3] = dr[2];
            }
            Blk hv;
            to_in(hb, hv);
            store_img(a.ws + a.ws_off[a.ws_heads], tile0 + t, 1, 0, hv, lane);
        }
        f32x16 dc[NC];
        const PImg wr0 = pimg(a.packed, a.vrgb), wr1 = pimg(a.packed, a.vrgb + NC * 128),
                   wr2 = pimg(a.packed, a.vrgb + 2 * NC * 128);
#pragma unroll
        for (int nb = 0; nb < NC; ++nb)
#pragma unroll
            for (int r = 0; r < 16; ++r) {
                f32x2 v = wr0.at(nb, r) * bcast2(dr[0]);
                v = __builtin_elementwise_fma(wr1.at(nb, r), bcast2(dr[1]), v);
                v = __builtin_elementwise_fma(wr2.at(nb, r), bcast2(dr[2]), v);
                dc[nb][r] = h ? v[1] : v[0];
            }
        const u32x4 mwc = mask_of(t, n);
#pragma unroll
        for (int nb = 0; nb < NC; ++nb) {
            to_in_masked(dc[nb], mwc, nb, cin.v[t][nb]);
            store_dz(a.ws_dir, NC, t, nb, cin.v[t][nb]);
        }
    }

    f32x16 acc[TPW][kHB];
    Act<kHB> hin;
#pragma unroll
    for (int t = 0; t < TPW; ++t)
#pragma unroll
        for (int nb = 0; nb < kHB; ++nb) zero(acc[t][nb]);
    constexpr int DBX = (WANT_X && DB > 0) ? DB : 0;
    f32x16 dd[TPW][DBX > 0 ? DBX : 1];
#pragma unroll
    for (int t = 0; t < TPW; ++t)
#pragma unroll
        for (int k = 0; k < (DBX > 0 ? DBX : 1); ++k) zero(dd[t][k]);
    stream_gemm<kHB, DBX, NC>(acc, dd, 0, cin, ring, st, a.sd);
    if constexpr (DBX > 0) {
        if (a.g_d) {
#pragma unroll
            for (int t = 0; t < TPW; ++t) {
                const int64_t m = (tile0 + t) * 32 + ml;
                const bool valid = tok[t] && m < a.M;
                const float d0 = valid ? a.d[3 * m] : 0.f, d1 = valid ? a.d[3 * m + 1] : 0.f,
                            d2 = valid ? a.d[3 * m + 2] : 0.f;
                float g0 = 0.f, g1 = 0.f, g2 = 0.f;
#pragma unroll
                for (int kb = 0; kb < DBX; ++kb)
#pragma unroll
                    for (int r = 0; r < 16; ++r)
                        pe_feat_bwd(d0, d1, d2, 32 * kb + acc_row(r, h), a.Ld, dd[t][kb][r], g0, g1, g2);
                g0 += __shfl_xor(g0, 32);
                g1 += __shfl_xor(g1, 32);
                g2 += __shfl_xor(g2, 32);
                if (valid && h == 0) {
                    a.g_d[3 * m] = g0 * a.inv_gscale;
                    a.g_d[3 * m + 1] = g1 * a.inv_gscale;
                    a.g_d[3 * m + 2] = g2 * a.inv_gscale;
                }
            }
        }
    }
#pragma unroll
    for (int t = 0; t < TPW; ++t)
#pragma unroll
        for (int nb = 0; nb < kHB; ++nb) {
            Blk v;
            to_in(acc[t][nb], v);
            hin.put(t, nb, v);
            store_dz(a.ws_feat, kHB, t, nb, v);
        }

    f32x16 dummy[TPW][1];
#pragma unroll
    for (int t = 0; t < TPW; ++t)
#pragma unroll
        for (int nb = 0; nb < kHB; ++nb) zero(acc[t][nb]);
    u32x4 mwf[TPW];
#pragma unroll
    for (int t = 0; t < TPW; ++t) mwf[t] = mask_of(t, n - 1);
    stream_gemm<kHB, 0, kHB>(acc, dummy, 0, hin, ring, st, a.sd);
    {
        const PImg ws = pimg(a.packed, a.vsig);
#pragma unroll
        for (int nb = 0; nb < kHB; ++nb)
#pragma unroll
            for (int r = 0; r < 16; ++r)
#pragma unroll
                for (int t = 0; t < TPW; ++t) {
                    const f32x2 v = __builtin_elementwise_fma(ws.at(nb, r), bcast2(dzs[t]), bcast2(acc[t][nb][r]));
                    acc[t][nb][r] = h ? v[1] : v[0];
                }
    }
#pragma unroll
    for (int t = 0; t < TPW; ++t) {
#pragma unroll
        for (int nb = 0; nb < kHB; ++nb) {
            Blk v;
            to_in_masked(acc[t][nb], mwf[t], nb, v);
            hin.put(t, nb, v);
            store_dz(WS_DZ0 + n - 1, kHB, t, nb, v);
        }
    }

    constexpr int XBX = WANT_X ? XB : 0;
    f32x16 dxe[TPW][XBX > 0 ? XBX : 1];
#pragma unroll
    for (int t = 0; t < TPW; ++t)
#pragma unroll
        for (int k = 0; k < (XBX > 0 ? XBX : 1); ++k) zero(dxe[t][k]);
    for (int i = n - 1; i >= 1; --i) {
#pragma unroll
        for (int t = 0; t < TPW; ++t)
#pragma unroll
            for (int nb = 0; nb < kHB; ++nb) zero(acc[t][nb]);
        u32x4 mwt[TPW];
#pragma unroll
        for (int t = 0; t < TPW; ++t) mwt[t] = mask_of(t, i - 1);
        if ((a.skips >> (i - 1)) & 1u) {
            if constexpr (XBX > 0)
                stream_gemm<kHB, XBX, kHB>(acc, dxe, 0, hin, ring, st, a.sd);
            else
                stream_gemm<kHB, 0, kHB>(acc, dummy, 0, hin, ring, st, a.sd);
        } else {
            stream_gemm<kHB, 0, kHB>(acc, dummy, 0, hin, ring, st, a.sd);
        }
#pragma unroll
        for (int t = 0; t < TPW; ++t) {
#pragma unroll
            for (int nb = 0; nb < kHB; ++nb) {
                Blk v;
                to_in_masked(acc[t][nb], mwt[t], nb, v);
                hin.put(t, nb, v);
                store_dz(WS_DZ0 + i - 1, kHB, t, nb, v);
            }
        }
    }
    if constexpr (XBX > 0) {
        stream_gemm<XBX, 0, kHB>(dxe, dummy, 0, hin, ring, st, a.sd);
        if (a.g_x) {
#pragma unroll
            for (int t = 0; t < TPW; ++t) {
                const int64_t m = (tile0 + t) * 32 + ml;
                const bool valid = tok[t] && m < a.M;
                const float x0 = valid ? a.x[3 * m] : 0.f, x1 = valid ? a.x[3 * m + 1] : 0.f,
                            x2 = valid ? a.x[3 * m + 2] : 0.f;
                float g0 = 0.f, g1 = 0.f, g2 = 0.f;
#pragma unroll
                for (int kb = 0; kb < XBX; ++kb)
#pragma unroll
                    for (int r = 0; r < 16; ++r)
                        pe_feat_bwd(x0, x1, x2, 32 * kb + acc_row(r, h), a.L, dxe[t][kb][r], g0, g1, g2);
                g0 += __shfl_xor(g0, 32);
                g1 += __shfl_xor(g1, 32);
                g2 += __shfl_xor(g2, 32);
                if (valid && h == 0) {
                    a.g_x[3 * m] = g0 * a.inv_gscale;
                    a.g_x[3 * m + 1] = g1 * a.inv_gscale;
                    a.g_x[3 * m + 2] = g2 * a.inv_gscale;
                }
            }
        }
    }
    finish_tiles(ts, a.nseg, a.tiles, a.dw_list, a.count);
}

namespace {

int max_chunk(const StreamDesc& sd) {
    int m = 0;
    for (int q = 0; q < sd.nq; ++q) m = sd.ckb[q] * 1024 > m ? sd.ckb[q] * 1024 : m;
    return m;
}

}

int launch_fwd(const MlpPlan& p, FwdArgs& a, bool train, hipStream_t s) {
    a.slot_bytes = max_chunk(a.sd);
    if (a.slot_bytes > 32 * 1024) {
        set_error("nr_mlp_forward: chunk of %d bytes exceeds the stager", a.slot_bytes);
        return NR_EARG;
    }
    const size_t lds = 2 * static_cast<size_t>(a.slot_bytes);
    const dim3 grid(static_cast<unsigned>(ceil_div_ll(a.tiles, kNT / 64))), block(kNT);
#define NR_FWD(XB_, DB_)                                                                      \
    if (p.XB == XB_ && p.DB == DB_) {                                                         \
        if (train)                                                                            \
            hipLaunchKernelGGL((mlp_fwd_kernel<XB_, DB_, true>), grid, block, lds, s, a);     \
        else                                                                                  \
            hipLaunchKernelGGL((mlp_fwd_kernel<XB_, DB_, false>), grid, block, lds, s, a);    \
        return check_launch("nr_mlp_forward");                                                \
    }
    NR_FWD(2, 1)
#ifndef NR_MLP_DEV
    NR_FWD(2, 0)
    NR_FWD(1, 1)
    NR_FWD(1, 0)
#endif
#undef NR_FWD
    set_error("nr_mlp_forward: no kernel instance for XB=%d DB=%d", p.XB, p.DB);
    return NR_EARG;
}

int launch_bwd(const MlpPlan& p, BwdArgs& a, bool want_x, hipStream_t s) {
    a.slot_bytes = max_chunk(a.sd);
    if (a.slot_bytes > 40 * 1024) {
        set_error("nr_mlp_backward_dx: chunk of %d bytes exceeds the stager", a.slot_bytes);
        return NR_EARG;
    }
    const size_t lds = 2 * static_cast<size_t>(a.slot_bytes);
    const dim3 grid(static_cast<unsigned>(a.nseg * (kSegTiles / (kNT / 64)))), block(kNT);
#define NR_BWD(XB_, DB_)                                                                      \
    if (p.XB == XB_ && p.DB == DB_) {                                                         \
        if (want_x)                                                                           \
            hipLaunchKernelGGL((mlp_bwd_kernel<XB_, DB_, true>), grid, block, lds, s, a);     \
        else                                                                                  \
            hipLaunchKernelGGL((mlp_bwd_kernel<XB_, DB_, false>), grid, block, lds, s, a);    \
        return check_launch("nr_mlp_backward_dx");                                            \
    }
    NR_BWD(2, 1)
#ifndef NR_MLP_DEV
    NR_BWD(2, 0)
    NR_BWD(1, 1)
    NR_BWD(1, 0)
#endif
#undef NR_BWD
    set_error("nr_mlp_backward_dx: no kernel instance for XB=%d DB=%d", p.XB, p.DB);
    return NR_EARG;
}

}
```

robust-nerf_amd/csrc/mlp_launch.hpp:

```cpp
#pragma once

#include "common.hpp"
#include "mlp_plan.hpp"
#include "optim.hpp"

#pragma GCC visibility push(hidden)
namespace nr {

inline float grad_scale(int prec) { return prec == NR_PREC_FP16 ? 16384.0f : 1.0f; }

constexpr int kMaxChunks = 176;

struct StreamDesc {
    int64_t base;
    int nq;
    int ckb[kMaxChunks];
    int cadv[kMaxChunks];
};

struct FwdArgs {
    const char* packed;
    const float* params;
    const float* x;
    const float* d;
    float* rgb;
    float* sigma;
    char* saved;
    int64_t M, tiles;
    int L, Ld, n_layers;
    uint32_t skips;
    int slot_bytes;
    StreamDesc sd;
    int64_t vb[kMaxMfmaLayers];
    int64_t bo[kMaxMfmaLayers];
    int64_t vsig, vrgb, sig_b, rgb_b;
    int64_t sv_off[kMaxTrunk + 4];
    int sv_feat, sv_denc, sv_hc;
    int64_t mask_off;
    int n_mask;
};

struct BwdArgs {
    float gscale, inv_gscale;
    const char* packed;
    const float* params;
    const float* x;
    const float* d;
    const float* rgb;
    const float* sigma;
    const float* g_rgb;
    const float* g_sigma;
    float* g_x;
    float* g_d;
    const char* saved;
    char* ws;
    int64_t M, tiles;
    const uint8_t* flags;
    const uint32_t* blk_count;
    int64_t nseg;
    uint32_t* dw_list;
    uint32_t* count;
    int L, Ld, n_layers;
    uint32_t skips;
    int slot_bytes;
    StreamDesc sd;
    int64_t vsig, vrgb;
    int64_t mask_off;
    int n_mask;
    int64_t ws_off[kMaxTrunk + 3];
    int ws_feat, ws_dir, ws_heads;
};

int launch_fwd(const MlpPlan& p, FwdArgs& a, bool train, hipStream_t s);
int launch_bwd(const MlpPlan& p, BwdArgs& a, bool want_x, hipStream_t s);

struct RbmArgs {
    const char* packed;
    const float* params;
    const float* x;
    const float* d;
    float* rgb;
    float* sigma;
    char* saved;
    int64_t M, tiles;
    int L, Ld, n_layers;
    uint32_t skips;
    int64_t base;
    int64_t vhead, sig_b, rgb_b;
    int64_t sv_off[kMaxTrunk + 4];
    int sv_feat, sv_denc, sv_hc;
    int64_t mask_off;
    int n_mask;
};

struct BwdrArgs {
    float gscale;
    const char* packed;
    const float* rgb;
    const float* sigma;
    const float* g_rgb;
    const float* g_sigma;
    const char* saved;
    char* ws;
    int64_t M, tiles;
    const uint8_t* flags;
    const uint32_t* blk_count;
    int64_t nseg;
    uint32_t* dw_list;
    uint32_t* count;
    int64_t scratch_base;
    int n_layers;
    int64_t base;
    int64_t vrgb, vhead;
    int64_t mask_off;
    int n_mask;
    int64_t ws_off[kMaxTrunk + 3];
    int ws_feat, ws_dir, ws_heads;
};

int launch_fwd_rbm(const MlpPlan& p, const RbmArgs& a, bool train, hipStream_t s);
int launch_bwd_rbm(const MlpPlan& p, const BwdrArgs& a, hipStream_t s);
int input_grads16(const MlpPlan& p, const MlpSizes& z, const char* packed, const float* x, const float* d, float* g_x,
                  float* g_d, const char* ws, int64_t M, hipStream_t s);

#ifndef NR_DW_NSTAGE
#define NR_DW_NSTAGE 4
#endif
constexpr int kDwThreads = 512;
constexpr int kDwWaves = kDwThreads / 64;
static_assert(kDwWaves == kDwMaxWaves, "dW wave shares are planned for 8-wave workgroups");

constexpr int kDwMaxWgs = 256;
struct DwArgs {
    float* slabs;
    int njobs;
    int64_t tiles;
    const uint32_t* list;
    const uint32_t* count;
    int list_lds;
    int job_chunks[kMaxJobs];
    uint16_t wg_map[kDwMaxWgs];
    int stage_bytes, nstage;
    int64_t slab_floats_per_chunk;
    int job_NBz[kMaxJobs], job_KB[kMaxJobs];
    int64_t job_slab[kMaxJobs];
    const char* seg_ptr[kMaxJobs][2 * kMaxJobSeg];
    uint8_t seg_blocks[kMaxJobs][2 * kMaxJobSeg];
    int job_wave[kMaxJobs][kDwWaves];
};
static_assert(sizeof(DwArgs) <= 4096, "dW kernel arguments exceed 4 KiB");

__host__ __device__ constexpr int dw_wave_pack(int row0, int np, int col0, int nq, int bias) {
    return row0 | np << 6 | col0 << 9 | nq << 15 | bias << 17;
}

struct ReduceArgs {
    const float* slabs;
    float* g;
    float inv_gscale;
    int64_t param_count;
    int64_t slab_floats_per_chunk;
    int n_red;
    int rows[kMaxRed], in[kMaxRed], nseg[kMaxRed], bjob[kMaxRed], brow0[kMaxRed];
    int64_t w_off[kMaxRed], b_off[kMaxRed];
    RedSeg seg[kMaxRed][kMaxSeg];
    int64_t job_slab[kMaxJobs];
    int job_KB[kMaxJobs];
    int job_chunks[kMaxJobs];
};

int launch_tile_flags(const float* g_rgb, const float* g_sigma, int64_t M, int dense, int64_t nseg, uint8_t* flags,
                      uint32_t* blk_count, hipStream_t s);
int launch_dw(int prec, const DwArgs& a, int nwg, size_t lds, hipStream_t s);
int launch_dw_reduce(const ReduceArgs& a, int max_rows, hipStream_t s);

constexpr int kPackSlots = 3;
constexpr int64_t kDstMaxOff = int64_t(1) << 29;
struct PackIdx {
    uint32_t* table;
    int64_t n;
};

struct AdamSpanDev {
    float *p, *g, *m, *v;
    int64_t n;
    const float* partials;
    float max_norm;
    const uint32_t* table;
    char* packed;
};
struct AdamMultiArgs {
    AdamSpanDev s[kMaxAdamSpans];
    float omb1, b2, omb2, eps, step_size, bc2_sqrt;
    const float* sched;
};

int launch_pack(const MlpPlan& p, const float* params, void* packed, PackIdx t, bool idx, hipStream_t s);
int launch_adam_multi(const AdamMultiArgs& a, int grid, int nspan, hipStream_t s);

}
#pragma GCC visibility pop
```

robust-nerf_amd/csrc/mlp_plan.cpp.inc:

```

namespace nr {

static int blocks_of(int n) { return (n + 31) / 32; }

bool make_plan(const NrMlpConfig* c, MlpPlan* p, const char** why) {
    std::memset(p, 0, sizeof(*p));
    if (!c) {
        *why = "null config";
        return false;
    }
    if (c->hidden != kHidden) {
        *why = "hidden_dim must be 256 (the MFMA tiling is specialised for it)";
        return false;
    }
    if (c->n_layers < 1 || c->n_layers > kMaxTrunk) {
        *why = "num_hidden_layers must be in [1, 16]";
        return false;
    }
    if (c->precision != NR_PREC_FP32 && c->precision != NR_PREC_BF16 && c->precision != NR_PREC_FP16) {
        *why = "precision must be NR_PREC_FP32, NR_PREC_BF16 or NR_PREC_FP16";
        return false;
    }
    if ((c->skip_mask >> (c->n_layers - 1)) != 0) {
        *why = "skips must index trunk layers 0..num_hidden_layers-2";
        return false;
    }
    if (c->pos_freqs < 0 || c->dir_freqs < 0) {
        *why = "negative frequency count";
        return false;
    }
    p->L = c->pos_freqs;
    p->Ld = c->dir_freqs;
    p->n_layers = c->n_layers;
    p->skips = c->skip_mask;
    p->use_vd = c->use_view_dirs ? 1 : 0;
    p->prec = c->precision;
    p->dense_bwd = c->dense_backward ? 1 : 0;
    p->pos_dim = 3 * (1 + 2 * p->L);
    p->dir_dim = 3 * (1 + 2 * p->Ld);
    p->XB = blocks_of(p->pos_dim);
    p->DB = p->use_vd ? blocks_of(p->dir_dim) : 0;
    if (p->XB > 2 || p->DB > 1) {
        *why = "pos_freqs <= 10 and dir_freqs <= 4 are supported by the compiled kernels";
        return false;
    }
    const int n = p->n_layers;
    int64_t off = 0;
    auto set_lin = [&](LinearDesc& d, int out, int nseg, const Seg* segs) {
        d.out = out;
        d.in = 0;
        d.nseg = nseg;
        d.KB = 0;
        for (int s = 0; s < nseg; ++s) {
            d.seg[s] = segs[s];
            d.in += segs[s].width;
            d.KB += segs[s].blocks;
        }
        d.NB = blocks_of(out);
        d.w_off = off;
        off += static_cast<int64_t>(out) * d.in;
        d.b_off = off;
        off += out;
    };
    for (int i = 0; i < n; ++i) {
        Seg segs[2];
        int ns;
        if (i == 0) {
            segs[0] = {0, p->pos_dim, p->XB};
            ns = 1;
        } else if (is_skip(*p, i - 1)) {
            segs[0] = {0, p->pos_dim, p->XB};
            segs[1] = {p->pos_dim, kHidden, kHB};
            ns = 2;
        } else {
            segs[0] = {0, kHidden, kHB};
            ns = 1;
        }
        set_lin(p->lin[i], kHidden, ns, segs);
    }
    p->sig_w = off;
    off += kHidden;
    p->sig_b = off;
    off += 1;
    {
        Seg s0[1] = {{0, kHidden, kHB}};
        set_lin(p->lin[n], kHidden, 1, s0);
    }
    {
        Seg s1[2] = {{0, kHidden, kHB}, {kHidden, p->dir_dim, p->DB}};
        set_lin(p->lin[n + 1], kHidden / 2, p->use_vd ? 2 : 1, s1);
    }
    p->rgb_w = off;
    off += 3 * (kHidden / 2);
    p->rgb_b = off;
    off += 3;
    p->param_count = off;
    p->n_lin = n + 2;

    p->fpb = p->prec != NR_PREC_FP32 ? 2 : 4;
    int64_t pk = 0;
    for (int l = 0; l < p->n_lin; ++l) {
        LinearDesc& d = p->lin[l];
        d.pk_fwd = pk;
        const int bias_frag = p->fpb == 2 ? 1 : 0;
        pk += static_cast<int64_t>(d.NB) * (d.KB * p->fpb + bias_frag) * kFragBytes;
    }
    auto put_bwd = [&](int l) {
        LinearDesc& d = p->lin[l];
        d.pk_bwd = pk;
        pk += static_cast<int64_t>(d.NB) * d.KB * p->fpb * kFragBytes;
    };
    put_bwd(n + 1);
    put_bwd(n);
    for (int i = n - 1; i >= 0; --i) put_bwd(i);
    if (p->fpb == 2) {
        auto put_bwdr = [&](int l) {
            LinearDesc& d = p->lin[l];
            d.pk_bwdr = pk;
            pk += static_cast<int64_t>(kHB) * d.NB * 2 * kFragBytes;
        };
        put_bwdr(n + 1);
        put_bwdr(n);
        for (int i = n - 1; i >= 1; --i) put_bwdr(i);
    }
    for (int l = 0; l < p->n_lin; ++l) {
        p->lin[l].vb = pk;
        pk += static_cast<int64_t>(p->lin[l].NB) * 32 * 4;
    }
    p->vsig = pk;
    pk += kHidden * 4;
    p->vrgb = pk;
    pk += 3 * (kHidden / 2) * 4;
    p->vhead = pk;
    pk += 3 * 1024;
    p->packed_bytes = pk;
    p->esize = p->prec != NR_PREC_FP32 ? 2 : 4;

    p->sv_F[SV_XENC] = p->XB * 32;
    for (int i = 0; i < n; ++i) p->sv_F[SV_H0 + i] = kHidden;
    p->sv_feat = n + 1;
    p->sv_denc = n + 2;
    p->sv_hc = n + 3;
    p->sv_F[p->sv_feat] = kHidden;
    p->sv_F[p->sv_denc] = p->DB * 32;
    p->sv_F[p->sv_hc] = kHidden / 2;
    p->n_saved = n + 4;
    p->n_mask = n + 1;
    for (int i = 0; i < n; ++i) p->ws_F[WS_DZ0 + i] = kHidden;
    p->ws_feat = n;
    p->ws_dir = n + 1;
    p->ws_heads = n + 2;
    p->ws_F[p->ws_feat] = kHidden;
    p->ws_F[p->ws_dir] = kHidden / 2;
    p->ws_F[p->ws_heads] = 32;
    p->n_ws = n + 3;

    int64_t slab = 0;
    int nj = 0;
    bool fits = true;
    auto add_job = [&](int ndz, const DwSeg* dz, int nin, const DwSeg* in) {
        if (nj == kMaxJobs) {
            fits = false;
            nj = kMaxJobs - 1;
        }
        DwJob& j = p->job[nj];
        j.ndz = ndz;
        j.nin = nin;
        j.NBz = 0;
        j.KB = 0;
        for (int s = 0; s < ndz; ++s) {
            j.dz[s] = dz[s];
            j.NBz += dz[s].blocks;
        }
        for (int s = 0; s < nin; ++s) {
            j.in[s] = in[s];
            j.KB += in[s].blocks;
        }
        j.slab_off = slab;
        slab += static_cast<int64_t>(j.NBz) * 32 * (j.KB * 32 + 1);
        j.nwaves = 0;
        return nj++;
    };
    auto add_waves = [&](int j, int r0, int r1, int c0, int c1, bool bias) {
        DwJob& jb = p->job[j];
        for (int c = c0; c < c1; c += kDwMaxQ)
            for (int r = r0; r < r1; r += 4) {
                if (jb.nwaves == kDwMaxWaves) {
                    fits = false;
                    return;
                }
                jb.w[jb.nwaves++] = {r, r1 - r < 4 ? r1 - r : 4, c, c1 - c < kDwMaxQ ? c1 - c : kDwMaxQ,
                                     bias && c == c0 ? 1 : 0};
            }
    };
    int xjob[kMaxTrunk], xrow[kMaxTrunk], hjob[kMaxTrunk];
    {
        int layers[kMaxTrunk], nx = 0;
        for (int i = 0; i < n; ++i)
            if (i == 0 || is_skip(*p, i - 1)) layers[nx++] = i;
        int per = kMaxJobSeg;
        while (per > 1 && ((per * kHB + p->XB) * p->fpb > kDwMaxWaves * dw_max_pieces(p->fpb == 2) ||
                           per * (kHB / 4) * ((p->XB + kDwMaxQ - 1) / kDwMaxQ) > kDwMaxWaves))
            --per;
        for (int a = 0; a < nx; a += per) {
            DwSeg dz[kMaxJobSeg];
            const int cnt = nx - a < per ? nx - a : per;
            for (int b = 0; b < cnt; ++b) dz[b] = {1, WS_DZ0 + layers[a + b], kHB};
            DwSeg in[1] = {{0, SV_XENC, p->XB}};
            const int jb = add_job(cnt, dz, 1, in);
            add_waves(jb, 0, cnt * kHB, 0, p->XB, true);
            for (int b = 0; b < cnt; ++b) {
                xjob[layers[a + b]] = jb;
                xrow[layers[a + b]] = b * kHidden;
            }
        }
    }
    for (int i = 1; i < n; ++i) {
        DwSeg dz[1] = {{1, WS_DZ0 + i, kHB}};
        DwSeg in[1] = {{0, SV_H0 + i - 1, kHB}};
        hjob[i] = add_job(1, dz, 1, in);
        add_waves(hjob[i], 0, kHB, 0, kHB, true);
    }
    int jfeat, jdir, jsig = -1, sig_row = kHidden;
    if (p->fpb == 2) {
        DwSeg dz[2] = {{1, p->ws_feat, kHB}, {1, p->ws_heads, 1}};
        DwSeg in[1] = {{0, SV_H0 + n - 1, kHB}};
        jfeat = add_job(2, dz, 1, in);
        DwJob& jb = p->job[jfeat];
        for (int c = 0; c < kHB; c += kDwMaxQ) jb.w[jb.nwaves++] = {0, 4, c, kDwMaxQ, c == 0 ? 1 : 0};
        for (int c = 0; c < kHB; c += kDwMaxQ) jb.w[jb.nwaves++] = {4, kHB + 1 - 4, c, kDwMaxQ, c == 0 ? 1 : 0};
        jsig = jfeat;
    } else {
        DwSeg dz[1] = {{1, p->ws_feat, kHB}};
        DwSeg in[1] = {{0, SV_H0 + n - 1, kHB}};
        jfeat = add_job(1, dz, 1, in);
        add_waves(jfeat, 0, kHB, 0, kHB, true);
        DwSeg dzh[1] = {{1, p->ws_heads, 1}};
        jsig = add_job(1, dzh, 1, in);
        add_waves(jsig, 0, 1, 0, kHB, false);
        sig_row = 0;
    }
    {
        const int DBu = p->use_vd ? p->DB : 0;
        DwSeg dz[2] = {{1, p->ws_dir, kHB / 2}, {1, p->ws_heads, 1}};
        DwSeg in[3] = {{0, p->sv_feat, kHB}, {0, p->sv_denc, p->DB}, {0, p->sv_hc, kHB / 2}};
        if (!p->use_vd) in[1] = in[2];
        jdir = add_job(2, dz, p->use_vd ? 3 : 2, in);
        add_waves(jdir, 0, kHB / 2, 0, kHB + DBu, true);
        add_waves(jdir, kHB / 2, kHB / 2 + 1, kHB + DBu, kHB + DBu + kHB / 2, true);
    }
    if (!fits) {
        *why = "dW job shares exceed the 8-wave workgroup";
        return false;
    }
    int red = 0;
    auto add_red = [&](int rows, int in, int64_t w_off, int64_t b_off, int bjob, int brow0) -> ReduceRange& {
        ReduceRange& r = p->red[red++];
        r.rows = rows;
        r.in = in;
        r.w_off = w_off;
        r.b_off = b_off;
        r.nseg = 0;
        r.bjob = bjob;
        r.brow0 = brow0;
        return r;
    };
    auto add_seg = [](ReduceRange& r, int col0, int width, int job, int row0, int c0) {
        r.seg[r.nseg++] = {col0, width, job, row0, c0};
    };
    for (int i = 0; i < n; ++i) {
        const LinearDesc& d = p->lin[i];
        const bool has_x = i == 0 || is_skip(*p, i - 1);
        ReduceRange& r = add_red(kHidden, d.in, d.w_off, d.b_off, i > 0 ? hjob[i] : xjob[i], i > 0 ? 0 : xrow[i]);
        if (has_x) add_seg(r, 0, p->pos_dim, xjob[i], xrow[i], 0);
        if (i > 0) add_seg(r, has_x ? p->pos_dim : 0, kHidden, hjob[i], 0, 0);
    }
    {
        const LinearDesc& d = p->lin[n];
        add_seg(add_red(kHidden, kHidden, d.w_off, d.b_off, jfeat, 0), 0, kHidden, jfeat, 0, 0);
    }
    {
        const int hrow = kHidden / 2, hc_col = (kHB + (p->use_vd ? p->DB : 0)) * 32;
        add_seg(add_red(1, kHidden, p->sig_w, p->sig_b, jdir, hrow), 0, kHidden, jsig, sig_row, 0);
        add_seg(add_red(3, kHidden / 2, p->rgb_w, p->rgb_b, jdir, hrow + 1), 0, kHidden / 2, jdir, hrow + 1, hc_col);
    }
    {
        const LinearDesc& d = p->lin[n + 1];
        ReduceRange& r = add_red(kHidden / 2, d.in, d.w_off, d.b_off, jdir, 0);
        add_seg(r, 0, kHidden, jdir, 0, 0);
        if (p->use_vd) add_seg(r, kHidden, p->dir_dim, jdir, 0, kHidden);
    }
    p->n_jobs = nj;
    p->n_red = red;
    p->slab_floats_per_chunk = slab;
    return true;
}

static int64_t align256(int64_t x) { return (x + 255) & ~int64_t(255); }

MlpSizes make_sizes(const MlpPlan& p, int64_t M) {
    MlpSizes s;
    std::memset(&s, 0, sizeof(s));
    s.tiles = (M + 31) / 32;
    s.tiles_alloc = (s.tiles + 16) / 16 * 16 + kScratchTiles;
    int64_t off = 0;
    for (int t = 0; t < p.n_saved; ++t) {
        s.saved_off[t] = off;
        off = align256(off + s.tiles_alloc * p.sv_F[t] * 32 * p.esize);
    }
    s.mask_off = off;
    off = align256(off + s.tiles_alloc * p.n_mask * 64 * 16);
    s.saved_bytes = off;
    off = 0;
    for (int t = 0; t < p.n_ws; ++t) {
        s.ws_off[t] = off;
        off = align256(off + s.tiles_alloc * p.ws_F[t] * 32 * p.esize);
    }
#ifndef NR_DW_WGS
#define NR_DW_WGS 256
#endif
    int64_t ch = NR_DW_WGS / (p.n_jobs > 0 ? p.n_jobs : 1);
    if (ch > s.tiles / 16) ch = s.tiles / 16;
    s.chunks = static_cast<int>(ch < 1 ? 1 : ch);
    for (int j = 0; j < p.n_jobs; ++j) s.job_chunks[j] = s.chunks;
    s.max_chunks = s.chunks;
    if (p.fpb == 4 && p.n_jobs > 0) {
        int64_t cap = s.tiles / 16;
        if (cap < 1) cap = 1;
        int cost[kMaxJobs], left = NR_DW_WGS - p.n_jobs;
        for (int j = 0; j < p.n_jobs; ++j) {
            cost[j] = p.job[j].nwaves > kDwMaxWaves / 2 ? 2 : 1;
            s.job_chunks[j] = 1;
        }
        for (; left > 0; --left) {
            int best = -1;
            for (int j = 0; j < p.n_jobs; ++j) {
                if (s.job_chunks[j] >= cap) continue;
                if (best < 0 || cost[j] * s.job_chunks[best] > cost[best] * s.job_chunks[j]) best = j;
            }
            if (best < 0) break;
            ++s.job_chunks[best];
        }
        s.max_chunks = 1;
        for (int j = 0; j < p.n_jobs; ++j) s.max_chunks = s.job_chunks[j] > s.max_chunks ? s.job_chunks[j] : s.max_chunks;
    }
    s.slab_off = off;
    off = align256(off + static_cast<int64_t>(s.max_chunks) * p.slab_floats_per_chunk * 4);
    s.nseg = (s.tiles + kSegTiles - 1) / kSegTiles;
    s.flags_off = off;
    off = align256(off + std::max<int64_t>(s.tiles_alloc, s.nseg * kSegTiles));
    s.blkcnt_off = off;
    off = align256(off + s.nseg * (kSegTiles / 64) * 4);
    s.dwlist_off = off;
    off = align256(off + s.tiles * 4);
    s.count_off = off;
    off = align256(off + 16);
    s.ws_bytes = off;
    return s;
}

}
```

robust-nerf_amd/csrc/mlp_plan.hpp:

```cpp
#pragma once

#include <cstdint>

#include "nerf_hip.h"

namespace nr {

constexpr int kHidden = 256;
constexpr int kHB = kHidden / 32;
constexpr int kMaxTrunk = 16;
constexpr int kMaxMfmaLayers = kMaxTrunk + 2;
constexpr int kFragBytes = 1024;
constexpr int kScratchTiles = 64;
constexpr int kSegTiles = 256;
constexpr int kMaxJobs = kMaxTrunk + 8;
constexpr int kMaxSeg = 2;
constexpr int kMaxJobSeg = 4;
constexpr int kMaxRed = kMaxTrunk + 4;
__host__ __device__ constexpr int dw_max_pieces(bool k16) { return k16 ? 6 : 10; }

struct Seg {
    int col0, width, blocks;
};

struct LinearDesc {
    int64_t w_off, b_off;
    int out, in;
    int NB, KB;
    int nseg;
    Seg seg[kMaxSeg];
    int64_t pk_fwd, pk_bwd;
    int64_t pk_bwdr;
    int64_t vb;
};

struct DwSeg {
    int is_ws, tensor, blocks;
};

constexpr int kDwMaxWaves = 8;
constexpr int kDwMaxP = 5, kDwMaxQ = 2;
struct DwWave {
    int row0, np, col0, nq, bias;
};

struct DwJob {
    int ndz, nin;
    DwSeg dz[kMaxJobSeg], in[kMaxJobSeg];
    int NBz, KB;
    int64_t slab_off;
    int nwaves;
    DwWave w[kDwMaxWaves];
};

enum SavedId { SV_XENC = 0, SV_H0 = 1  };
enum WsId { WS_DZ0 = 0  };

struct RedSeg {
    int col0, width, job, slab_row0, slab_col0;
};
struct ReduceRange {
    int rows, in;
    int64_t w_off, b_off;
    int nseg;
    RedSeg seg[kMaxSeg];
    int bjob, brow0;
};

struct MlpPlan {
    int L, Ld, n_layers, use_vd, prec;
    int dense_bwd;
    uint32_t skips;
    int pos_dim, dir_dim, XB, DB;
    int64_t param_count;
    int n_lin;
    LinearDesc lin[kMaxMfmaLayers];
    int64_t sig_w, sig_b, rgb_w, rgb_b;
    int64_t packed_bytes;
    int64_t vsig, vrgb;
    int64_t vhead;
    int esize;
    int fpb;
    int n_saved;
    int sv_feat, sv_denc, sv_hc;
    int sv_F[kMaxTrunk + 4];
    int n_mask;
    int n_ws;
    int ws_feat, ws_dir, ws_heads;
    int ws_F[kMaxTrunk + 3];
    int n_jobs;
    DwJob job[kMaxJobs];
    int64_t slab_floats_per_chunk;
    int n_red;
    ReduceRange red[kMaxRed];
};

inline bool is_skip(const MlpPlan& p, int i) { return (p.skips >> i) & 1u; }

bool make_plan(const NrMlpConfig* cfg, MlpPlan* p, const char** why);

struct MlpSizes {
    int64_t tiles;
    int64_t tiles_alloc;
    int64_t saved_off[kMaxTrunk + 4];
    int64_t mask_off;
    int64_t saved_bytes;
    int64_t ws_off[kMaxTrunk + 3];
    int chunks;
    int job_chunks[kMaxJobs];
    int max_chunks;
    int64_t slab_off;
    int64_t nseg;
    int64_t flags_off, blkcnt_off, dwlist_off, count_off;
    int64_t ws_bytes;
};

MlpSizes make_sizes(const MlpPlan& p, int64_t M);

}
```

robust-nerf_amd/noisy_src/_hip.py:

```python

from __future__ import annotations

import ctypes
import os
from pathlib import Path
from typing import Optional

import torch

_LIB_PATH = Path(os.environ.get("NR_HIP_LIB") or Path(__file__).resolve().parent / "lib" / "libnerf_hip.so")

c_vp = ctypes.c_void_p
c_i = ctypes.c_int
c_i64 = ctypes.c_int64
c_f = ctypes.c_float
c_d = ctypes.c_double
c_u32 = ctypes.c_uint32


class NrMlpConfig(ctypes.Structure):

    _fields_ = [
        ("pos_freqs", c_i),
        ("dir_freqs", c_i),
        ("hidden", c_i),
        ("n_layers", c_i),
        ("skip_mask", c_u32),
        ("use_view_dirs", c_i),
        ("precision", c_i),
        ("dense_backward", c_i),
    ]


class NrAdamSpan(ctypes.Structure):

    _fields_ = [
        ("params", c_vp),
        ("grads", c_vp),
        ("exp_avg", c_vp),
        ("exp_avg_sq", c_vp),
        ("n", c_i64),
        ("sumsq_partials", c_vp),
        ("max_norm", c_f),
        ("pack_table", c_vp),
        ("packed", c_vp),
    ]


NR_PREC_FP32 = 0
NR_PREC_BF16 = 1
NR_PREC_FP16 = 2
_cfg_p = ctypes.POINTER(NrMlpConfig)

_SIGNATURES = {
    "nr_last_error": (ctypes.c_char_p, []),
    "nr_abi_version": (c_i, []),
    "nr_probe_fill": (c_i, [c_vp, c_i, c_f, c_vp]),
    "nr_probe_mfma": (c_i, [c_i, c_vp, c_vp, c_vp, c_vp]),
    "nr_ray_directions": (c_i, [c_i, c_i, c_f, c_f, c_f, c_vp, c_vp]),
    "nr_get_rays": (c_i, [c_vp, c_vp, c_i64, c_vp, c_vp, c_vp]),
    "nr_get_rays_bwd_workspace_bytes": (c_i64, []),
    "nr_get_rays_bwd": (c_i, [c_vp, c_vp, c_i64, c_vp, c_vp, c_vp, c_vp, c_vp, c_vp]),
    "nr_rays_from_pixels_fwd": (c_i, [c_vp, c_vp, c_vp, c_i, c_i, c_i, c_f, c_i, c_vp, c_vp, c_vp, c_vp]),
    "nr_rays_from_pixels_bwd": (c_i, [c_vp, c_vp, c_vp, c_i, c_i, c_i, c_f, c_i, c_vp, c_vp, c_vp, c_vp]),
    "nr_se3_poses_fwd": (c_i, [c_vp, c_vp, c_vp, c_vp, c_i, c_vp, c_vp]),
    "nr_check_index_range": (c_i, [c_vp, c_i, c_i, c_vp, c_vp]),
    "nr_se3_poses_bwd": (c_i, [c_vp, c_vp, c_vp, c_i, c_i, c_vp, c_i, c_vp, c_vp, c_vp]),
    "nr_gather_rays": (c_i, [c_vp, c_i64, c_i, c_vp, c_vp, c_vp, c_vp, c_vp, c_vp, c_vp, c_vp]),
    "nr_gather_pixels": (c_i, [c_vp, c_i, c_i, c_i, c_vp, c_i, c_vp, c_vp, c_vp, c_vp, c_vp]),
    "nr_stratified_sample": (c_i, [c_vp, c_vp, c_vp, c_f, c_f, c_i, c_i, c_i, c_vp, c_vp, c_vp, c_vp]),
    "nr_positional_encoding": (c_i, [c_vp, c_i64, c_i, c_i, c_i, c_i, c_vp, c_vp]),
    "nr_positional_encoding_bwd": (c_i, [c_vp, c_i64, c_i, c_i, c_i, c_i, c_vp, c_vp, c_vp]),
    "nr_sample_pdf": (c_i, [c_vp, c_vp, c_vp, c_i, c_i, c_i, c_vp, c_vp]),
    "nr_sample_hierarchical": (c_i, [c_vp, c_vp, c_vp, c_vp, c_vp, c_i, c_i, c_i, c_vp, c_vp, c_vp, c_vp]),
    "nr_composite_fwd": (c_i, [c_vp, c_vp, c_vp, c_vp, c_vp, c_i, c_i, c_i, c_vp, c_vp, c_vp, c_vp, c_vp]),
    "nr_composite_bwd": (c_i, [c_vp, c_vp, c_vp, c_vp, c_vp, c_i, c_i, c_i, c_vp, c_vp, c_vp, c_vp,
                               c_vp, c_vp, c_vp, c_vp]),
    "nr_mlp_param_count": (c_i64, [_cfg_p]),
    "nr_mlp_packed_bytes": (c_i64, [_cfg_p]),
    "nr_mlp_saved_bytes": (c_i64, [_cfg_p, c_i64]),
    "nr_mlp_workspace_bytes": (c_i64, [_cfg_p, c_i64]),
    "nr_mlp_pack": (c_i, [_cfg_p, c_vp, c_vp, c_vp]),
    "nr_mlp_forward": (c_i, [_cfg_p, c_vp, c_vp, c_vp, c_vp, c_i64, c_vp, c_vp, c_vp, c_vp]),
    "nr_mlp_backward": (c_i, [_cfg_p, c_vp, c_vp, c_vp, c_vp, c_i64, c_vp, c_vp, c_vp, c_vp, c_vp,
                              c_vp, c_vp, c_vp, c_vp, c_vp]),
    "nr_mlp_backward_dx": (c_i, [_cfg_p, c_vp, c_vp, c_vp, c_vp, c_i64, c_vp, c_vp, c_vp, c_vp, c_vp, c_vp, c_vp,
                                 c_vp, c_vp]),
    "nr_mlp_backward_dw": (c_i, [_cfg_p, c_i64, c_vp, c_vp, c_vp]),
    "nr_mlp_backward_reduce": (c_i, [_cfg_p, c_i64, c_vp, c_vp, c_vp]),
    "nr_mlp_active_tiles_offset": (c_i64, [_cfg_p, c_i64]),
    "nr_sumsq_workspace_bytes": (c_i64, []),
    "nr_sumsq": (c_i, [c_vp, c_i64, c_vp, c_vp, c_vp]),
    "nr_adam_step": (c_i, [c_vp, c_vp, c_vp, c_vp, c_i64, c_d, c_d, c_d, c_d, c_i64, c_vp, c_f, c_vp]),
    "nr_sumsq_partials": (c_i, [c_vp, c_vp, c_i, c_vp, c_vp]),
    "nr_adam_multi": (c_i, [ctypes.POINTER(NrAdamSpan), c_i, c_d, c_d, c_d, c_d, c_i64, c_vp, c_vp]),
    "nr_mlp_pack_table_bytes": (c_i64, [_cfg_p]),
    "nr_mlp_pack_table": (c_i, [_cfg_p, c_vp, c_vp]),
    "nr_expand_viewdirs": (c_i, [c_vp, c_i, c_i, c_vp, c_vp]),
    "nr_pts_bwd": (c_i, [c_vp, c_vp, c_i, c_i, c_vp, c_vp, c_vp]),
    "nr_viewdirs_bwd": (c_i, [c_vp, c_vp, c_i, c_i, c_vp, c_vp]),
    "nr_composite_mse_workspace_bytes": (c_i64, [c_i]),
    "nr_composite_mse": (c_i, [c_vp, c_vp, c_vp, c_vp, c_vp, c_vp, c_i, c_i, c_i, c_f, c_vp, c_vp, c_vp, c_vp, c_vp,
                               c_vp, c_vp, c_vp, c_vp, c_vp, c_vp]),
    "nr_mse_fwd_bwd": (c_i, [c_vp, c_vp, c_i, c_f, c_vp, c_vp, c_vp]),
    "nr_image_metrics_workspace_bytes": (c_i64, [c_i, c_i, c_i]),
    "nr_image_metrics": (c_i, [c_vp, c_vp, c_i, c_i, c_i, ctypes.POINTER(c_f), c_d, c_d, c_vp, c_vp, c_vp]),
    "nr_frame_u8": (c_i, [c_vp, c_i, c_i, c_i, c_vp, c_i64, c_i, c_vp]),
    "nr_depth_frame_u8_workspace_bytes": (c_i64, []),
    "nr_depth_frame_u8": (c_i, [c_vp, c_i, c_i, c_vp, c_vp, c_vp]),
}

_lib: Optional[ctypes.CDLL] = None


def lib_path() -> Path:
    return _LIB_PATH


def load(require_all: bool = True) -> ctypes.CDLL:
    global _lib
    if _lib is not None:
        return _lib
    if not _LIB_PATH.exists():
        raise RuntimeError(
            f"noisy_src: HIP library {_LIB_PATH} not built; run `make -C robust-nerf_amd` "
            "(or __graft_entry__.build()). There is no CPU fallback."
        )
    lib = ctypes.CDLL(str(_LIB_PATH), mode=os.RTLD_NOW | os.RTLD_GLOBAL)
    for name, (res, args) in _SIGNATURES.items():
        fn = getattr(lib, name, None)
        if fn is None:
            if require_all:
                raise RuntimeError(f"noisy_src: {_LIB_PATH} does not export {name}")
            continue
        fn.restype = res
        fn.argtypes = args
    _lib = lib
    return lib


def exported_symbols() -> list:
    return list(_SIGNATURES)


def last_error() -> str:
    msg = load().nr_last_error()
    return msg.decode() if msg else ""


_raw_stream = getattr(torch._C, "_cuda_getCurrentRawStream", None)


def stream_ptr(device: Optional[torch.device] = None) -> int:
    if _raw_stream is not None and device is None:
        return _raw_stream(torch.cuda.current_device())
    return torch.cuda.current_stream(device).cuda_stream


class CallTimer:

    def __init__(self, names, keys=None):
        self.names = set(names)
        self.keys = None if keys is None else set(keys)
        self.events = {}

    def wants(self, key) -> bool:
        return self.keys is None or key in self.keys

    def record(self, key, fn):
        s = torch.cuda.Event(enable_timing=True)
        e = torch.cuda.Event(enable_timing=True)
        s.record()
        rc = fn()
        e.record()
        self.events.setdefault(key, []).append((s, e))
        return rc

    def summary(self):
        return {k: (len(v), sum(a.elapsed_time(b) for a, b in v) / len(v)) for k, v in self.events.items()}


_timer: Optional[CallTimer] = None


def set_timer(timer: Optional[CallTimer]) -> None:
    global _timer
    _timer = timer


def call(name: str, *args, tag: str = "") -> int:
    fn = getattr(load(), name)
    if _timer is not None and name in _timer.names and _timer.wants(f"{name}{tag}"):
        rc = _timer.record(f"{name}{tag}", lambda: fn(*args))
    else:
        rc = fn(*args)
    if isinstance(rc, int) and fn.restype is c_i and rc != 0:
        raise RuntimeError(f"{name} failed (code {rc}): {last_error()}")
    return rc


def ptr(t: Optional[torch.Tensor]) -> Optional[int]:
    if t is None:
        return None
    if not t.is_cuda:
        raise RuntimeError(
            "noisy_src HIP path: tensor is on the CPU; this framework has no CPU fallback "
            "(move the inputs to a ROCm device)"
        )
    if not t.is_contiguous():
        raise RuntimeError("noisy_src HIP path: tensor must be contiguous")
    return t.data_ptr()


def require_device(*tensors: Optional[torch.Tensor]) -> None:
    for t in tensors:
        if t is not None and not t.is_cuda:
            raise RuntimeError(
                "noisy_src HIP path: got a CPU tensor; there is no CPU fallback "
                "(this is the MI355X framework — run on a ROCm device)"
            )
```

robust-nerf_amd/noisy_src/model.py:

```python

from __future__ import annotations

import ctypes
import os
import weakref
from typing import List, Optional, Tuple

import torch
import torch.nn as nn

from . import _hip, ops
from ._hip import NrMlpConfig, call, ptr
from .config import ModelConfig


class PositionalEncoding(nn.Module):

    def __init__(self, num_freqs: int, include_input: bool = True, log_sampling: bool = True) -> None:
        super().__init__()
        self.num_freqs = num_freqs
        self.include_input = include_input
        self.log_sampling = log_sampling
        if log_sampling:
            freq_bands = 2.0 ** torch.linspace(0.0, num_freqs - 1, num_freqs)
        else:
            freq_bands = torch.linspace(1.0, 2.0 ** (num_freqs - 1), num_freqs)
        self.register_buffer("freq_bands", freq_bands)

    @property
    def output_dim(self) -> int:
        dim = 2 * self.num_freqs
        if self.include_input:
            dim += 1
        return dim

    def forward(self, x: torch.Tensor) -> torch.Tensor:
        return ops.positional_encoding(x, self.num_freqs, self.include_input, self.log_sampling)


_DENSE_BACKWARD = os.environ.get("NR_MLP_DENSE_BACKWARD", "0") not in ("", "0")


def _precision_code(p: str) -> int:
    if p == "fp32":
        return _hip.NR_PREC_FP32
    if p == "bf16":
        return _hip.NR_PREC_BF16
    if p == "fp16":
        return _hip.NR_PREC_FP16
    raise ValueError(f"ModelConfig.precision must be 'fp32', 'bf16' or 'fp16', got {p!r}")


class _MLPFunction(torch.autograd.Function):

    @staticmethod
    def forward(ctx, x, d, net, *params):
        cfg = ctypes.byref(net._nr_cfg)
        flat = net._flat
        packed = net._packed_for_forward(params)
        xc = ops._c(x)
        dc = ops._c(d) if d is not None else None
        M = xc.shape[0]
        rgb = torch.empty(M, 3, device=xc.device, dtype=torch.float32)
        sigma = torch.empty(M, 1, device=xc.device, dtype=torch.float32)
        training = any(ctx.needs_input_grad)
        saved = None
        if training and M > 0:
            saved = torch.empty(int(_hip.load().nr_mlp_saved_bytes(cfg, M)), device=xc.device, dtype=torch.uint8)
        call("nr_mlp_forward", cfg, ptr(packed), ptr(flat), ptr(xc), ptr(dc), M, ptr(rgb), ptr(sigma), ptr(saved),
             _hip.stream_ptr(), tag=f"[M={M}]")
        if training:
            ctx.save_for_backward(xc, dc if dc is not None else xc.new_empty(0), rgb, sigma)
            ctx.has_d = dc is not None
            ctx.keep = (net, saved, packed, flat)
            ctx.shapes = [p.shape for p in params]
        return rgb, sigma

    @staticmethod
    def backward(ctx, g_rgb, g_sigma):
        xc, dc, rgb, sigma = ctx.saved_tensors
        net, saved, packed, flat = ctx.keep
        cfg = ctypes.byref(net._nr_cfg)
        M = xc.shape[0]
        dev = xc.device
        g_rgb = ops._c(g_rgb) if g_rgb is not None else torch.zeros(M, 3, device=dev)
        g_sigma = ops._c(g_sigma) if g_sigma is not None else torch.zeros(M, 1, device=dev)
        gflat = torch.empty(net._param_count, device=dev, dtype=torch.float32)
        g_x = torch.empty(M, 3, device=dev) if ctx.needs_input_grad[0] else None
        g_d = torch.empty(M, 3, device=dev) if (ctx.needs_input_grad[1] and ctx.has_d) else None
        if M > 0:
            ws = torch.empty(int(_hip.load().nr_mlp_workspace_bytes(cfg, M)), device=dev, dtype=torch.uint8)
            st, tag = _hip.stream_ptr(), f"[M={M}]"
            args = (cfg, ptr(packed), ptr(flat), ptr(xc), ptr(dc) if ctx.has_d else None, M, ptr(rgb), ptr(sigma),
                    ptr(saved), ptr(g_rgb), ptr(g_sigma), ptr(g_x), ptr(g_d), ptr(ws), st)
            call("nr_mlp_backward_dx", *args, tag=tag)
            call("nr_mlp_backward_dw", cfg, M, ptr(saved), ptr(ws), st, tag=tag)
            call("nr_mlp_backward_reduce", cfg, M, ptr(ws), ptr(gflat), st, tag=tag)
            if net._tile_counts is not None:
                off = int(_hip.load().nr_mlp_active_tiles_offset(cfg, M))
                net._tile_counts.append((M, ws[off:off + 4].view(torch.int32).clone()))
        else:
            gflat.zero_()
        net._last_gflat = gflat
        if net._grad_ready_hook is not None:
            net._grad_ready_hook(gflat)
        grads = []
        off = 0
        for shape in ctx.shapes:
            n = shape.numel()
            grads.append(gflat[off:off + n].view(shape))
            off += n
        return (g_x, g_d, None, *grads)


def _check_supported(cfg: NrMlpConfig, config: ModelConfig, n_params: int) -> None:
    lib = _hip.load()
    if int(lib.nr_mlp_packed_bytes(ctypes.byref(cfg))) < 0:
        raise NotImplementedError(
            f"ModelConfig(hidden_dim={config.hidden_dim}, pos_freqs={config.pos_freqs}, "
            f"dir_freqs={config.dir_freqs}, num_hidden_layers={config.num_hidden_layers}, skips={config.skips}) "
            f"is outside the envelope of the compiled MI355X kernels: {_hip.last_error()} "
            "(supported: hidden_dim=256, pos_freqs<=10, dir_freqs<=4, 1..16 layers, any skips)")
    want = int(lib.nr_mlp_param_count(ctypes.byref(cfg)))
    if want != n_params:
        raise RuntimeError(f"NeRF parameter layout mismatch: module {n_params} vs kernel plan {want}")


_FLAT_OWNERS: "weakref.WeakValueDictionary[int, NeRF]" = weakref.WeakValueDictionary()


def flat_owner(pflat: torch.Tensor):
    return _FLAT_OWNERS.get(pflat.data_ptr())


class NeRF(nn.Module):

    def __init__(self, config: ModelConfig | None = None) -> None:
        super().__init__()
        if config is None:
            config = ModelConfig()
        self.config = config
        self.pos_encoder = PositionalEncoding(num_freqs=config.pos_freqs, include_input=True)
        self.dir_encoder = PositionalEncoding(num_freqs=config.dir_freqs, include_input=True)
        pos_dim = 3 * self.pos_encoder.output_dim
        dir_dim = 3 * self.dir_encoder.output_dim
        self.pts_linears = nn.ModuleList()
        in_dim = pos_dim
        for i in range(config.num_hidden_layers):
            self.pts_linears.append(nn.Linear(in_dim, config.hidden_dim))
            in_dim = config.hidden_dim
            if i in config.skips:
                in_dim += pos_dim
        self.sigma_linear = nn.Linear(config.hidden_dim, 1)
        self.feature_linear = nn.Linear(config.hidden_dim, config.hidden_dim)
        if config.use_view_dirs:
            self.dir_linear = nn.Linear(config.hidden_dim + dir_dim, config.hidden_dim // 2)
        else:
            self.dir_linear = nn.Linear(config.hidden_dim, config.hidden_dim // 2)
        self.rgb_linear = nn.Linear(config.hidden_dim // 2, 3)

        skip_mask = 0
        for s in config.skips:
            skip_mask |= 1 << int(s)
        self._nr_cfg = NrMlpConfig(
            pos_freqs=config.pos_freqs, dir_freqs=config.dir_freqs, hidden=config.hidden_dim,
            n_layers=config.num_hidden_layers, skip_mask=skip_mask, use_view_dirs=int(bool(config.use_view_dirs)),
            precision=_precision_code(getattr(config, "precision", "fp32")),
            dense_backward=int(_DENSE_BACKWARD))
        self._param_count = sum(p.numel() for p in self.parameters())
        _check_supported(self._nr_cfg, config, self._param_count)
        self._flat: Optional[torch.Tensor] = None
        self._packed: Optional[torch.Tensor] = None
        self._packed_key = None
        self._table: Optional[torch.Tensor] = None
        self._last_gflat: Optional[torch.Tensor] = None
        self._grad_ready_hook = None
        self._tile_counts: Optional[list] = None
        self._tickets = {}

    def loss_ticket(self, device) -> torch.Tensor:
        t = self._tickets.get(device)
        if t is None:
            t = torch.zeros(4, device=device, dtype=torch.int32)
            self._tickets[device] = t
        return t

    @property
    def _param_list(self) -> List[nn.Parameter]:
        return list(self.parameters())

    def flat_params(self) -> torch.Tensor:
        self._ensure_flat()
        return self._flat

    def _ensure_flat(self, params: Optional[List[nn.Parameter]] = None) -> None:
        params = self._param_list if params is None else params
        flat = self._flat
        if flat is not None and flat.device == params[0].device:
            off = 0
            base = flat.data_ptr()
            ok = True
            for p in params:
                if p.data_ptr() != base + 4 * off or not p.is_contiguous():
                    ok = False
                    break
                off += p.numel()
            if ok:
                _FLAT_OWNERS[base] = self
                return
        dev = params[0].device
        _hip.require_device(params[0])
        flat = torch.empty(self._param_count, device=dev, dtype=torch.float32)
        off = 0
        with torch.no_grad():
            for p in params:
                n = p.numel()
                flat[off:off + n].copy_(p.detach().reshape(-1))
                p.data = flat[off:off + n].view(p.shape)
                off += n
        self._flat = flat
        self._packed_key = None
        _FLAT_OWNERS[flat.data_ptr()] = self

    def _packed_for_forward(self, params: Optional[List[nn.Parameter]] = None) -> torch.Tensor:
        params = self._param_list if params is None else params
        key = (self._flat.data_ptr(), tuple(p._version for p in params))
        if self._packed is None or self._packed_key != key or self._packed.device != self._flat.device:
            cfg = ctypes.byref(self._nr_cfg)
            nbytes = int(_hip.load().nr_mlp_packed_bytes(cfg))
            if nbytes < 0:
                raise RuntimeError(f"NeRF config unsupported by the HIP MLP: {_hip.last_error()}")
            if (self._packed is None or self._packed.numel() != nbytes
                    or self._packed.device != self._flat.device):
                self._packed = torch.empty(nbytes, device=self._flat.device, dtype=torch.uint8)
            call("nr_mlp_pack", cfg, ptr(self._flat), ptr(self._packed), _hip.stream_ptr())
            self._packed_key = key
        return self._packed

    def _pack_table(self) -> torch.Tensor:
        t = self._table
        if t is None or t.device != self._flat.device:
            cfg = ctypes.byref(self._nr_cfg)
            nbytes = int(_hip.load().nr_mlp_pack_table_bytes(cfg))
            t = torch.empty(nbytes // 4, device=self._flat.device, dtype=torch.int32)
            call("nr_mlp_pack_table", cfg, ptr(t), _hip.stream_ptr())
            self._table = t
        return t

    def _fused_pack_target(self, pflat: torch.Tensor, params: Optional[List[nn.Parameter]] = None):
        flat, packed = self._flat, self._packed
        if flat is None or packed is None or packed.device != flat.device:
            return None
        if pflat.data_ptr() != flat.data_ptr() or pflat.numel() != flat.numel():
            return None
        params = self._param_list if params is None else params
        if self._packed_key != (flat.data_ptr(), tuple(p._version for p in params)):
            return None
        return self._pack_table(), packed

    def _mark_packed_fresh(self, params: Optional[List[nn.Parameter]] = None) -> None:
        params = self._param_list if params is None else params
        self._packed_key = (self._flat.data_ptr(), tuple(p._version for p in params))

    def forward(self, x: torch.Tensor, d: torch.Tensor | None = None) -> Tuple[torch.Tensor, torch.Tensor]:
        _hip.require_device(x, d)
        if self.config.use_view_dirs and d is None:
            raise ValueError("NeRF with use_view_dirs=True needs view directions d")
        params = self._param_list
        self._ensure_flat(params)
        return _MLPFunction.apply(x, d if self.config.use_view_dirs else None, self, *params)


def create_nerf(config: ModelConfig | None = None) -> Tuple[NeRF, NeRF | None]:
    if config is None:
        config = ModelConfig()
    model_coarse = NeRF(config)
    model_fine = NeRF(config)
    return model_coarse, model_fine
```

Before: 881,700 rays/s.

## Compact sparse active samples into dense tiles for 16-bit MLP backward

Tracks a per-sample activity mask and per-block sample counts. When a segment's live samples would fill noticeably fewer tiles than its active tiles, the samples are packed into dense tiles through a gather map. The backward-input, dW and input-gradient kernels then process only those packed tiles, reading the map to locate saved activations. This cuts wasted MFMA work on partially active tiles, at the cost of extra workspace, prefix-scan and select work, an LDS ring for the map, and gathered (less coalesced) loads.

```diff
diff --git a/include/nerf_hip.h b/include/nerf_hip.h
--- a/include/nerf_hip.h
+++ b/include/nerf_hip.h
@@ -141,6 +141,8 @@
                            const void* workspace, float* g_params,
                            nr_stream_t stream);
 int64_t nr_mlp_active_tiles_offset(const NrMlpConfig* cfg, int64_t M);
+int64_t nr_mlp_executed_tiles_offset(const NrMlpConfig* cfg, int64_t M);
+int nr_mlp_compact_regions(const NrMlpConfig* cfg, int64_t M, int64_t* off_and_bytes);
 
 int64_t nr_sumsq_workspace_bytes(void);
 int nr_sumsq(const float* x, int64_t n, float* acc, void* workspace,
diff --git a/robust-nerf_amd/csrc/mlp.hip b/robust-nerf_amd/csrc/mlp.hip
--- a/robust-nerf_amd/csrc/mlp.hip
+++ b/robust-nerf_amd/csrc/mlp.hip
@@ -206,7 +206,10 @@
     uint32_t* blkcnt = reinterpret_cast<uint32_t*>(wsb + z.blkcnt_off);
     uint32_t* dwlist = reinterpret_cast<uint32_t*>(wsb + z.dwlist_off);
     uint32_t* tcount = reinterpret_cast<uint32_t*>(wsb + z.count_off);
-    if (const int rc = launch_tile_flags(g_rgb, g_sigma, M, p.dense_bwd, z.nseg, tflags, blkcnt, s)) return rc;
+    uint32_t* smask = reinterpret_cast<uint32_t*>(wsb + z.smask_off);
+    uint32_t* blksmp = reinterpret_cast<uint32_t*>(wsb + z.blksmp_off);
+    if (const int rc = launch_tile_flags(g_rgb, g_sigma, M, p.dense_bwd, z.nseg, tflags, blkcnt, smask, blksmp, s))
+        return rc;
     const int n = p.n_layers;
     if (p.prec != NR_PREC_FP32) {
         BwdrArgs r;
@@ -223,6 +226,10 @@
         r.tiles = z.tiles;
         r.flags = tflags;
         r.blk_count = blkcnt;
+        r.smask = smask;
+        r.blk_samples = blksmp;
+        r.map = reinterpret_cast<uint32_t*>(wsb + z.map_off);
+        NR_REQUIRE(z.nseg * kSegTiles < (int64_t{1} << 31), "nr_mlp_backward_dx: M beyond 2^36 samples");
         r.nseg = z.nseg;
         r.dw_list = dwlist;
         r.count = tcount;
@@ -262,6 +269,7 @@
     b.tiles = z.tiles;
     b.flags = tflags;
     b.blk_count = blkcnt;
+    b.blk_samples = blksmp;
     b.nseg = z.nseg;
     b.dw_list = dwlist;
     b.count = tcount;
@@ -316,6 +324,7 @@
     w.tiles = z.tiles;
     w.list = reinterpret_cast<const uint32_t*>(ws + z.dwlist_off);
     w.count = reinterpret_cast<const uint32_t*>(ws + z.count_off);
+    w.map = reinterpret_cast<const uint32_t*>(ws + z.map_off);
     w.njobs = p.n_jobs;
     int nwg = 0;
     NR_REQUIRE(p.n_jobs <= 32 && z.max_chunks < 2048, "nr_mlp_backward_dw: %d jobs x %d chunks beyond the map",
@@ -349,10 +358,12 @@
         for (int q = 0; q < jb.ndz; ++q, ++ns) {
             w.seg_ptr[j][ns] = (jb.dz[q].is_ws ? ws : sv) + (jb.dz[q].is_ws ? z.ws_off : z.saved_off)[jb.dz[q].tensor];
             w.seg_blocks[j][ns] = static_cast<uint8_t>(jb.dz[q].blocks);
+            if (!jb.dz[q].is_ws) w.seg_saved[j] |= static_cast<uint8_t>(1u << ns);
         }
         for (int q = 0; q < jb.nin; ++q, ++ns) {
             w.seg_ptr[j][ns] = (jb.in[q].is_ws ? ws : sv) + (jb.in[q].is_ws ? z.ws_off : z.saved_off)[jb.in[q].tensor];
             w.seg_blocks[j][ns] = static_cast<uint8_t>(jb.in[q].blocks);
+            if (!jb.in[q].is_ws) w.seg_saved[j] |= static_cast<uint8_t>(1u << ns);
         }
         w.job_slab[j] = jb.slab_off;
         NR_REQUIRE((jb.NBz + jb.KB) * p.fpb <= kDwWaves * dw_max_pieces(p.fpb == 2),
@@ -360,9 +371,12 @@
         max_blk = jb.NBz + jb.KB > max_blk ? jb.NBz + jb.KB : max_blk;
     }
     w.stage_bytes = max_blk * p.fpb * kFragBytes;
-    w.nstage = static_cast<int>((160 * 1024 - kFragBytes) / w.stage_bytes);
+    const int ring_bytes = p.fpb == 2 ? kDwMapRing * 256 : 0;
+    w.nstage = static_cast<int>((160 * 1024 - kFragBytes - ring_bytes) / w.stage_bytes);
     if (w.nstage > NR_DW_NSTAGE) w.nstage = NR_DW_NSTAGE;
     size_t lds = static_cast<size_t>(w.nstage) * w.stage_bytes + kFragBytes;
+    w.map_lds = static_cast<int>(lds);
+    lds += ring_bytes;
     int min_chunks = z.job_chunks[0];
     for (int j = 1; j < p.n_jobs; ++j) min_chunks = z.job_chunks[j] < min_chunks ? z.job_chunks[j] : min_chunks;
     const size_t list_bytes = (static_cast<size_t>(ceil_div_ll(z.tiles, min_chunks)) * 4 + 15) / 16 * 16;
@@ -421,6 +435,22 @@
     return make_sizes(p, M).count_off;
 }
 
+int64_t nr_mlp_executed_tiles_offset(const NrMlpConfig* cfg, int64_t M) {
+    MlpPlan p;
+    if (!plan_or_error(cfg, &p) || M <= 0) return -1;
+    return make_sizes(p, M).count_off + 4;
+}
+
+int nr_mlp_compact_regions(const NrMlpConfig* cfg, int64_t M, int64_t* off_and_bytes) {
+    MlpPlan p;
+    if (!plan_or_error(cfg, &p) || M <= 0 || !off_and_bytes) return NR_EARG;
+    const MlpSizes z = make_sizes(p, M);
+    const int64_t v[6] = {z.smask_off, z.nseg * kSegTiles * 4, z.blksmp_off, z.nseg * (kSegTiles / 64) * 4,
+                          z.map_off,   z.nseg * kSegTiles * 32 * 4};
+    for (int i = 0; i < 6; ++i) off_and_bytes[i] = v[i];
+    return NR_OK;
+}
+
 int nr_mlp_backward(const NrMlpConfig* cfg, const void* packed, const float* params, const float* x, const float* d,
                     int64_t M, const float* rgb, const float* sigma, const void* saved, const float* g_rgb,
                     const float* g_sigma, float* g_params, float* g_x, float* g_d, void* workspace,
diff --git a/robust-nerf_amd/csrc/mlp_16.hip b/robust-nerf_amd/csrc/mlp_16.hip
--- a/robust-nerf_amd/csrc/mlp_16.hip
+++ b/robust-nerf_amd/csrc/mlp_16.hip
@@ -17,7 +17,10 @@
     float* g_x;
     float* g_d;
     int64_t M, tiles;
-    const uint8_t* flags;
+    const uint32_t* smask;
+    const uint32_t* list;
+    const uint32_t* count;
+    const uint32_t* map;
     int L, Ld;
     float inv_gscale;
     int nsrc;
@@ -63,21 +66,7 @@
         else
             return *reinterpret_cast<const bf16x8*>(frag_src(f) + lane * 16);
     };
-    const int64_t waves = static_cast<int64_t>(gridDim.x) * (kDinNT / 64);
-    for (int64_t tile = static_cast<int64_t>(blockIdx.x) * (kDinNT / 64) + (threadIdx.x >> 6); tile < a.tiles;
-         tile += waves) {
-        const int64_t tile_u = __builtin_amdgcn_readfirstlane(static_cast<int>(tile));
-        const int64_t m = tile * 32 + ml;
-        const bool valid = m < a.M;
-        if (!a.flags[tile_u]) {
-            if (valid && h == 0)
-#pragma unroll
-                for (int c = 0; c < 3; ++c) {
-                    if (a.g_x) a.g_x[3 * m + c] = 0.f;
-                    if (a.g_d) a.g_d[3 * m + c] = 0.f;
-                }
-            continue;
-        }
+    auto run_tile = [&](int64_t tile_u, int64_t m, bool valid) {
         if (a.g_x) {
             f32x16 dxe[XB];
 #pragma unroll
@@ -147,6 +136,37 @@
                     a.g_d[3 * m + 2] = g2 * a.inv_gscale;
                 }
             }
+        }
+    };
+    const int64_t waves = static_cast<int64_t>(gridDim.x) * (kDinNT / 64);
+    const int64_t wave0 = static_cast<int64_t>(blockIdx.x) * (kDinNT / 64) + (threadIdx.x >> 6);
+    const int64_t cnt = a.count[1];
+    const bool ident = cnt == a.tiles;
+    for (int64_t tile = wave0; tile < a.tiles; tile += waves) {
+        const int64_t tile_u = __builtin_amdgcn_readfirstlane(static_cast<int>(tile));
+        const int64_t m = tile * 32 + ml;
+        const bool valid = m < a.M;
+        if (ident) {
+            run_tile(tile_u, m, valid);
+            continue;
+        }
+        if (valid && h == 0 && !((a.smask[tile_u] >> ml) & 1u))
+#pragma unroll
+            for (int c = 0; c < 3; ++c) {
+                if (a.g_x) a.g_x[3 * m + c] = 0.f;
+                if (a.g_d) a.g_d[3 * m + c] = 0.f;
+            }
+    }
+    if (ident) return;
+    for (int64_t pos = wave0; pos < cnt; pos += waves) {
+        const uint32_t e = __builtin_amdgcn_readfirstlane(a.list[pos]);
+        const int64_t slot = e & ~kGatherBit;
+        if (e & kGatherBit) {
+            const uint32_t mv = a.map[slot * 32 + ml];
+            run_tile(slot, (slot & ~static_cast<int64_t>(kSegTiles - 1)) * 32 + (mv & ~kFillBit), !(mv & kFillBit));
+        } else {
+            const int64_t m = slot * 32 + ml;
+            run_tile(slot, m, m < a.M && ((a.smask[slot] >> ml) & 1u));
         }
     }
 }
@@ -231,7 +251,10 @@
     std::memset(&da, 0, sizeof(da));
     da.packed = packed;
     da.ws = ws;
-    da.flags = reinterpret_cast<const uint8_t*>(ws + z.flags_off);
+    da.smask = reinterpret_cast<const uint32_t*>(ws + z.smask_off);
+    da.list = reinterpret_cast<const uint32_t*>(ws + z.dwlist_off);
+    da.count = reinterpret_cast<const uint32_t*>(ws + z.count_off);
+    da.map = reinterpret_cast<const uint32_t*>(ws + z.map_off);
     da.x = x;
     da.d = d;
     da.g_x = g_x;
diff --git a/robust-nerf_amd/csrc/mlp_bwd_rbm.inc b/robust-nerf_amd/csrc/mlp_bwd_rbm.inc
--- a/robust-nerf_amd/csrc/mlp_bwd_rbm.inc
+++ b/robust-nerf_amd/csrc/mlp_bwd_rbm.inc
@@ -47,27 +47,39 @@
     extern __shared__ __attribute__((aligned(16))) char lds[];
     const int tid = threadIdx.x, lane = tid & 63, h = lane >> 5, ml = lane & 31;
     const int wv = __builtin_amdgcn_readfirstlane(tid >> 6);
-    const TileSel ts = select_tile(a.flags, a.blk_count, a.nseg, a.tiles, W, wv);
+    const TileSel ts = select_tile<true>(a.flags, a.blk_count, a.blk_samples, a.nseg, a.tiles, W, wv);
     if (ts.idle) {
         finish_tiles(ts, a.nseg, a.tiles, a.dw_list, a.count);
         return;
     }
     const int64_t tile = ts.live ? ts.tile : a.scratch_base + ((blockIdx.x * W + wv) & (kScratchTiles - 1));
-    const int64_t m = tile * 32 + ml;
-    const bool valid = m < a.M;
+    int64_t m = tile * 32 + ml;
+    bool valid = m < a.M;
+    int64_t mtile = tile;
+    int mlane = lane;
+    if (ts.compact > 0 && ts.live) {
+        const uint32_t r = static_cast<uint32_t>(ts.k) * 32u + static_cast<uint32_t>(ml);
+        const bool fill = r >= ts.samples;
+        const uint32_t src = seg_nth_sample(a.smask, ts.seg, fill ? ts.samples - 1u : r);
+        m = ts.seg * (kSegTiles * 32) + src;
+        valid = !fill;
+        mtile = ts.seg * kSegTiles + (src >> 5);
+        mlane = 32 * h + static_cast<int>(src & 31u);
+        if (h == 0) a.map[tile * 32 + ml] = src | (fill ? kFillBit : 0u);
+    }
     const int n = a.n_layers;
     constexpr int NC = kHB / 2;
 
     char* mlds = lds + bwdr_mask_off() + wv * a.n_mask * 1024;
-    const char* msrc = a.saved + a.mask_off + tile * a.n_mask * 1024;
+    const char* msrc = a.saved + a.mask_off + mtile * a.n_mask * 1024 + mlane * 16;
     for (int l = 0; l < a.n_mask; ++l)
-        __builtin_amdgcn_global_load_lds((const __attribute__((address_space(1))) void*)(msrc + l * 1024 + lane16()),
+        __builtin_amdgcn_global_load_lds((const __attribute__((address_space(1))) void*)(msrc + l * 1024),
                                          (__attribute__((address_space(3))) void*)(mlds + l * 1024), 16, 0, 0);
     if (wv == 0)
         __builtin_amdgcn_global_load_lds(
             (const __attribute__((address_space(1))) void*)(a.packed + a.vhead + lane16()),
             (__attribute__((address_space(3))) void*)(lds + bwdr_sig_off(a.n_mask, W)), 16, 0, 0);
-    const u32x4 mwc = *reinterpret_cast<const u32x4*>(msrc + n * 1024 + lane16());
+    const u32x4 mwc = *reinterpret_cast<const u32x4*>(msrc + n * 1024);
     auto mask_of = [&](int layer) { return *reinterpret_cast<const u32x4*>(mlds + layer * 1024 + lane16()); };
     const float* wsig = reinterpret_cast<const float*>(lds + bwdr_sig_off(a.n_mask, W)) + 16 * h;
 
diff --git a/robust-nerf_amd/csrc/mlp_dev.hpp b/robust-nerf_amd/csrc/mlp_dev.hpp
--- a/robust-nerf_amd/csrc/mlp_dev.hpp
+++ b/robust-nerf_amd/csrc/mlp_dev.hpp
@@ -375,14 +375,71 @@
     return sg * kSegTiles + 4 * L + b;
 }
 
-__device__ __forceinline__ void place_segment(const SegFlags& f, uint32_t before, int64_t nseg, int64_t sg,
+__device__ __forceinline__ void place_segment(const SegFlags& f, uint32_t before, uint32_t before_tiles,
+                                              uint32_t compact, int64_t nseg, int64_t sg,
                                               uint32_t* __restrict__ list, uint32_t* __restrict__ count) {
     const int lane = threadIdx.x & 63;
-    uint32_t slot = before + static_cast<uint32_t>(f.incl - f.count);
-#pragma unroll
-    for (int q = 0; q < 4; ++q)
-        if ((f.word >> (8 * q)) & 1u) list[slot++] = static_cast<uint32_t>(sg * kSegTiles + 4 * lane + q);
-    if (sg == nseg - 1 && lane == 0) *count = before + static_cast<uint32_t>(f.total);
+    if (compact > 0) {
+#pragma unroll
+        for (int q = 0; q < 4; ++q) {
+            const uint32_t c = 4 * lane + q;
+            if (c < compact) list[before + c] = static_cast<uint32_t>(sg * kSegTiles + c) | kGatherBit;
+        }
+    } else {
+        uint32_t slot = before + static_cast<uint32_t>(f.incl - f.count);
+#pragma unroll
+        for (int q = 0; q < 4; ++q)
+            if ((f.word >> (8 * q)) & 1u) list[slot++] = static_cast<uint32_t>(sg * kSegTiles + 4 * lane + q);
+    }
+    if (sg == nseg - 1 && lane == 0) {
+        count[0] = before_tiles + static_cast<uint32_t>(f.total);
+        count[1] = before + (compact > 0 ? compact : static_cast<uint32_t>(f.total));
+    }
+}
+
+__device__ __forceinline__ uint32_t seg_nth_sample(const uint32_t* __restrict__ smask, int64_t sg, uint32_t r) {
+    static_assert(kSegTiles == 4 * 64, "four sample masks per lane");
+    const int lane = threadIdx.x & 63;
+    const uint4 m4 = reinterpret_cast<const uint4*>(smask + sg * kSegTiles)[lane];
+    const uint32_t ms[4] = {m4.x, m4.y, m4.z, m4.w};
+    const int cnt = (__popc(ms[0]) + __popc(ms[1])) + (__popc(ms[2]) + __popc(ms[3]));
+    int incl = cnt;
+#pragma unroll
+    for (int d = 1; d < 64; d <<= 1) {
+        const int o = __shfl_up(incl, d);
+        if (lane >= d) incl += o;
+    }
+    int lo = 0;
+#pragma unroll
+    for (int step = 32; step > 0; step >>= 1) {
+        const int v = __shfl(incl, lo + step - 1);
+        if (v <= static_cast<int>(r)) lo += step;
+    }
+    int rr = static_cast<int>(r) - __shfl(incl - cnt, lo);
+    uint32_t w[4];
+#pragma unroll
+    for (int q = 0; q < 4; ++q) w[q] = static_cast<uint32_t>(__shfl(static_cast<int>(ms[q]), lo));
+    uint32_t m = w[0];
+    int q = 0;
+#pragma unroll
+    for (int i = 0; i < 3; ++i) {
+        const int c = __popc(w[i]);
+        if (q == i && rr >= c) {
+            rr -= c;
+            q = i + 1;
+            m = w[i + 1];
+        }
+    }
+    int pos = 0;
+#pragma unroll
+    for (int s = 16; s > 0; s >>= 1) {
+        const int c = __popc((m >> pos) & ((1u << s) - 1u));
+        if (rr >= c) {
+            rr -= c;
+            pos += s;
+        }
+    }
+    return static_cast<uint32_t>((4 * lo + q) * 32 + pos);
 }
 
 constexpr int64_t kDenseCheckSegs = 1024;
@@ -391,10 +448,16 @@
     SegFlags sf;
     int64_t seg, tile;
     uint32_t before;
+    uint32_t before_tiles;
+    uint32_t samples;
+    uint32_t compact;
+    int k;
     bool dense, live, idle, leader;
 };
+template <bool PACK>
 __device__ __forceinline__ TileSel select_tile(const uint8_t* __restrict__ flags,
-                                               const uint32_t* __restrict__ blk_count, int64_t nseg,
+                                               const uint32_t* __restrict__ blk_count,
+                                               const uint32_t* __restrict__ blk_samples, int64_t nseg,
                                                int64_t tiles, int W, int wv) {
     constexpr int BPS = kSegTiles / 64;
     const int lane = threadIdx.x & 63;
@@ -404,22 +467,36 @@
     t.seg = (b % nseg + nseg - part % nseg) % nseg;
     static_assert(BPS == 4, "a segment's block counts are one uint4");
     const bool check = nseg <= kDenseCheckSegs;
-    const int64_t lim = check ? nseg : (part == 0 && wv == 0 ? t.seg : 0);
+    const bool lead = part == 0 && wv == 0;
+    const int64_t lim = check ? nseg : (lead ? t.seg : 0);
     const uint32_t word = seg_flag_word(flags, t.seg);
     const uint4* __restrict__ bc4 = reinterpret_cast<const uint4*>(blk_count);
-    uint32_t all = 0, before = 0;
+    const uint4* __restrict__ bs4 = reinterpret_cast<const uint4*>(blk_samples);
+    uint4 own = uint4{0u, 0u, 0u, 0u};
+    if constexpr (PACK) own = bs4[t.seg];
+    uint32_t all = 0, before = 0, before_tiles = 0;
     for (int64_t s0 = 0; s0 < lim; s0 += 4 * 64) {
-        uint4 c[4];
+        uint4 c[4], sm[4];
 #pragma unroll
         for (int i = 0; i < 4; ++i) {
             const int64_t sg = s0 + i * 64 + lane;
             c[i] = sg < lim ? bc4[sg] : uint4{0u, 0u, 0u, 0u};
+            sm[i] = uint4{0u, 0u, 0u, 0u};
+            if constexpr (PACK)
+                if (lead && sg < t.seg) sm[i] = bs4[sg];
         }
 #pragma unroll
         for (int i = 0; i < 4; ++i) {
             const uint32_t n = ((c[i].x + c[i].y) + c[i].z) + c[i].w;
             all += n;
-            before += (s0 + i * 64 + lane) < t.seg ? n : 0u;
+            uint32_t e = n;
+            if constexpr (PACK) {
+                const uint32_t smp = ((sm[i].x + sm[i].y) + sm[i].z) + sm[i].w;
+                if (seg_packs(n, smp)) e = seg_compact_tiles(smp);
+            }
+            const bool prior = (s0 + i * 64 + lane) < t.seg;
+            before += prior ? e : 0u;
+            before_tiles += prior ? n : 0u;
         }
     }
     t.sf = seg_scan(word);
@@ -427,21 +504,33 @@
     for (int d = 32; d > 0; d >>= 1) {
         all += __shfl_xor(all, d);
         before += __shfl_xor(before, d);
+        before_tiles += __shfl_xor(before_tiles, d);
     }
     t.before = __builtin_amdgcn_readfirstlane(before);
+    t.before_tiles = __builtin_amdgcn_readfirstlane(before_tiles);
     t.dense = check && static_cast<int64_t>(__builtin_amdgcn_readfirstlane(all)) == tiles;
+    t.samples = __builtin_amdgcn_readfirstlane(((own.x + own.y) + own.z) + own.w);
+    t.compact = 0;
+    t.k = 0;
     if (t.dense) {
         const int64_t first = b * W;
         t.tile = first + wv;
         t.live = t.tile < tiles;
         t.idle = first >= tiles;
         t.leader = b == 0 && wv == 0;
+    } else if (PACK && seg_packs(static_cast<uint32_t>(t.sf.total), t.samples)) {
+        t.compact = seg_compact_tiles(t.samples);
+        t.k = part * W + wv;
+        t.idle = static_cast<uint32_t>(part * W) >= t.compact;
+        t.live = static_cast<uint32_t>(t.k) < t.compact;
+        t.tile = t.live ? t.seg * kSegTiles + t.k : 0;
+        t.leader = lead;
     } else {
         const int k = part * W + wv;
         t.idle = part * W >= t.sf.total;
         t.live = k < t.sf.total;
         t.tile = t.live ? seg_entry(t.sf, t.seg, k) : 0;
-        t.leader = part == 0 && wv == 0;
+        t.leader = lead;
     }
     return t;
 }
@@ -450,9 +539,9 @@
                                              uint32_t* __restrict__ count) {
     if (!t.leader) return;
     if (t.dense) {
-        if ((threadIdx.x & 63) == 0) *count = static_cast<uint32_t>(tiles);
-    } else {
-        place_segment(t.sf, t.before, nseg, t.seg, list, count);
+        if ((threadIdx.x & 63) == 0) count[0] = count[1] = static_cast<uint32_t>(tiles);
+    } else {
+        place_segment(t.sf, t.before, t.before_tiles, t.compact, nseg, t.seg, list, count);
     }
 }
 
diff --git a/robust-nerf_amd/csrc/mlp_dw.hip b/robust-nerf_amd/csrc/mlp_dw.hip
--- a/robust-nerf_amd/csrc/mlp_dw.hip
+++ b/robust-nerf_amd/csrc/mlp_dw.hip
@@ -9,8 +9,10 @@
                                                                       const float* __restrict__ g_sigma, int64_t M,
                                                                       int dense,
                                                                       uint8_t* __restrict__ flags,
-                                                                      uint32_t* __restrict__ blk_count) {
-    __shared__ uint32_t wcnt[kTileFlagThreads / 64];
+                                                                      uint32_t* __restrict__ blk_count,
+                                                                      uint32_t* __restrict__ smask,
+                                                                      uint32_t* __restrict__ blk_samples) {
+    __shared__ uint32_t wcnt[kTileFlagThreads / 64], wsmp[kTileFlagThreads / 64];
     const int lane = threadIdx.x & 63, wv = threadIdx.x >> 6;
     const int64_t tw = static_cast<int64_t>(blockIdx.x) * 64 + wv * 16;
     bool nz[8];
@@ -29,16 +31,30 @@
         nz[it] = v;
     }
     uint32_t mask = 0;
+    uint32_t mine = 0;
+    uint32_t nsmp = 0;
 #pragma unroll
     for (int it = 0; it < 8; ++it) {
         const uint64_t b = __ballot(nz[it]);
-        mask |= (static_cast<uint32_t>(b & 0xffffffffull) != 0 ? 1u : 0u) << (2 * it);
-        mask |= (static_cast<uint32_t>(b >> 32) != 0 ? 1u : 0u) << (2 * it + 1);
-    }
-    if (lane < 16) flags[tw + lane] = static_cast<uint8_t>((mask >> lane) & 1u);
-    if (lane == 0) wcnt[wv] = __popc(mask);
+        const uint32_t lo = static_cast<uint32_t>(b & 0xffffffffull), up = static_cast<uint32_t>(b >> 32);
+        mask |= (lo != 0 ? 1u : 0u) << (2 * it);
+        mask |= (up != 0 ? 1u : 0u) << (2 * it + 1);
+        mine = lane == 2 * it ? lo : (lane == 2 * it + 1 ? up : mine);
+        nsmp += __popc(lo) + __popc(up);
+    }
+    if (lane < 16) {
+        flags[tw + lane] = static_cast<uint8_t>((mask >> lane) & 1u);
+        smask[tw + lane] = mine;
+    }
+    if (lane == 0) {
+        wcnt[wv] = __popc(mask);
+        wsmp[wv] = nsmp;
+    }
     __syncthreads();
-    if (threadIdx.x == 0) blk_count[blockIdx.x] = ((wcnt[0] + wcnt[1]) + wcnt[2]) + wcnt[3];
+    if (threadIdx.x == 0) {
+        blk_count[blockIdx.x] = ((wcnt[0] + wcnt[1]) + wcnt[2]) + wcnt[3];
+        blk_samples[blockIdx.x] = ((wsmp[0] + wsmp[1]) + wsmp[2]) + wsmp[3];
+    }
 }
 
 #ifndef NR_DW_AUX
@@ -101,7 +117,9 @@
     const int row0 = winfo & 63, np = (winfo >> 6) & 7, col0 = (winfo >> 9) & 63, nq = (winfo >> 15) & 3;
     const bool active = np > 0;
     const bool do_bias = active && ((winfo >> 17) & 1);
-    const int64_t cnt = *a.count;
+    const int64_t cnt = a.count[1];
+    const bool ident = cnt == a.tiles;
+    const bool gmode = k16<PREC> && !ident;
     const int64_t tpc = (cnt + a.job_chunks[j] - 1) / a.job_chunks[j];
     const int64_t t0 = static_cast<int64_t>(chunk) * tpc;
     int64_t t1 = t0 + tpc;
@@ -115,6 +133,7 @@
     const char* psrc[kMaxPW];
     int64_t pstride[kMaxPW];
     int pdst[kMaxPW];
+    int pgm = 0;
 #pragma unroll
     for (int k = 0; k < kMaxPW; ++k) {
         psrc[k] = nullptr;
@@ -131,20 +150,25 @@
             pstride[k] = static_cast<int64_t>(nb) * BLK;
             psrc[k] = a.seg_ptr[j][sg] + (pc - p0) * kFragBytes + L * 16;
             pdst[k] = pad ? -1 : pc * kFragBytes;
+            if (!pad && ((a.seg_saved[j] >> sg) & 1)) pgm |= 1 << k;
         }
     }
     const uint32_t* lds_list = nullptr;
-    if (a.list_lds && cnt != a.tiles) {
+    if (a.list_lds && !ident) {
         uint32_t* dst = reinterpret_cast<uint32_t*>(lds + a.list_lds);
         for (int64_t q = t0 + tid; q < t1; q += kDwThreads) dst[q - t0] = a.list[q];
         __syncthreads();
         lds_list = dst;
     }
-    const bool ident = cnt == a.tiles;
     const uint32_t list_base = static_cast<uint32_t>(reinterpret_cast<uintptr_t>(lds_list));
-    auto tile_at = [&](int64_t pos) -> int64_t {
-        if (ident) return pos;
-        if (!lds_list) return a.list[pos];
+    auto tile_at = [&](int64_t pos) -> uint32_t {
+        if (ident) return static_cast<uint32_t>(pos);
+        if (!lds_list) {
+            const uint32_t* q = a.list + pos;
+            uint32_t v;
+            asm volatile("s_load_dword %0, %1, 0x0\n\ts_waitcnt lgkmcnt(0)" : "=s"(v) : "s"(q) : "memory");
+            return v;
+        }
         uint32_t v;
         asm volatile("ds_read_b32 %0, %1\n\ts_waitcnt lgkmcnt(0)"
                      : "=v"(v)
@@ -152,16 +176,46 @@
                      : "memory");
         return __builtin_amdgcn_readfirstlane(v);
     };
-    auto stage = [&](int b, int64_t tile) {
+    const int mi = dw_slot(lane, wv & 1) & 31;
+    const uint32_t map_base = static_cast<uint32_t>(reinterpret_cast<uintptr_t>(lds + a.map_lds));
+    auto map_dma = [&](int64_t pos) {
+        if (pos > t1 - 1) pos = t1 - 1;
+        const uint32_t e = tile_at(pos);
+        const uint32_t* src = a.map + static_cast<int64_t>(e & ~kGatherBit) * 32 + (lane & 31);
+        __builtin_amdgcn_global_load_lds((const __attribute__((address_space(1))) void*)(src),
+                                         (__attribute__((address_space(3))) void*)(lds + a.map_lds +
+                                                                                   ((pos - t0) & (kDwMapRing - 1)) * 256),
+                                         4, 0, 0);
+    };
+    auto map_read = [&](int64_t pos) -> uint32_t {
+        uint32_t v;
+        asm volatile("ds_read_b32 %0, %1\n\ts_waitcnt lgkmcnt(0)"
+                     : "=v"(v)
+                     : "v"(map_base + static_cast<uint32_t>((pos - t0) & (kDwMapRing - 1)) * 256u + 4u * mi)
+                     : "memory");
+        return v;
+    };
+    auto stage = [&](auto gc, int b, uint32_t e, uint32_t mv) {
+        constexpr bool G = decltype(gc)::value;
         char* dst = lds + b * a.stage_bytes;
         char* scratch = lds + a.nstage * a.stage_bytes;
+        const bool gath = G && (e & kGatherBit) != 0;
+        const int64_t tile = gath ? (e & ~kGatherBit) : e;
+        int64_t tsrc = 0;
+        int dl = 0;
+        if constexpr (G) {
+            tsrc = (tile & ~static_cast<int64_t>(kSegTiles - 1)) + ((mv & (kSegTiles * 32 - 1)) >> 5);
+            dl = (static_cast<int>(mv & 31u) - mi) * 16;
+        }
 #pragma unroll
         for (int k = 0; k < kMaxPW; ++k) {
             if (k < per_wave) {
                 char* d = pdst[k] < 0 ? scratch : dst + pdst[k];
-                __builtin_amdgcn_global_load_lds(
-                    (const __attribute__((address_space(1))) void*)(psrc[k] + tile * pstride[k]),
-                    (__attribute__((address_space(3))) void*)(d), 16, 0, NR_DW_AUX);
+                const char* src = psrc[k] + tile * pstride[k];
+                if constexpr (G)
+                    if (gath && ((pgm >> k) & 1)) src = psrc[k] + tsrc * pstride[k] + dl;
+                __builtin_amdgcn_global_load_lds((const __attribute__((address_space(1))) void*)(src),
+                                                 (__attribute__((address_space(3))) void*)(d), 16, 0, NR_DW_AUX);
             }
         }
     };
@@ -174,6 +228,16 @@
             default: asm volatile("s_waitcnt vmcnt(0)" ::: "memory"); break;
         }
     };
+    auto wait_vm = [](int n) {
+        switch (n) {
+#define NR_VM(N) \
+    case N: asm volatile("s_waitcnt vmcnt(" #N ")" ::: "memory"); break;
+            NR_VM(1) NR_VM(2) NR_VM(3) NR_VM(4) NR_VM(5) NR_VM(6) NR_VM(7) NR_VM(8) NR_VM(9) NR_VM(10) NR_VM(11)
+            NR_VM(12) NR_VM(13)
+#undef NR_VM
+            default: asm volatile("s_waitcnt vmcnt(0)" ::: "memory"); break;
+        }
+    };
 
     uint32_t trof[2][2];
 #pragma unroll
@@ -186,8 +250,9 @@
     const int hl = lane >> 5, ml = lane & 31;
 
     using std::integral_constant;
-    auto run = [&](auto npc, auto nqc) {
+    auto run = [&](auto npc, auto nqc, auto gc) {
         constexpr int NP = decltype(npc)::value, NQ = decltype(nqc)::value;
+        constexpr bool G = decltype(gc)::value;
         f32x16 acc[NP][NQ];
 #pragma unroll
         for (int p = 0; p < NP; ++p)
@@ -202,16 +267,24 @@
 #pragma unroll
         for (int q = 0; q < NQ; ++q) kval[q] = q < nq;
 
+        if (G && t0 < t1) {
+            for (int k = 0; k <= NS; ++k) map_dma(t0 + k);
+            asm volatile("s_waitcnt vmcnt(0)" ::: "memory");
+        }
         for (int k = 0; k < NS - 1; ++k)
-            if (t0 + k < t1) stage(k, tile_at(t0 + k));
+            if (t0 + k < t1) stage(gc, k, tile_at(t0 + k), G ? map_read(t0 + k) : 0u);
         int bcur = 0, bnext = NS - 1;
         for (int64_t t = t0; t < t1; ++t) {
             int64_t ahead = t1 - 1 - t;
             if (ahead > NS - 2) ahead = NS - 2;
-            wait_pieces(per_wave * static_cast<int>(ahead));
+            if constexpr (!G)
+                wait_pieces(per_wave * static_cast<int>(ahead));
+            else
+                wait_vm(NS >= 3 && NS <= 4 ? per_wave * static_cast<int>(ahead) + (t > t0 ? 1 : 0) : 0);
             asm volatile("s_waitcnt lgkmcnt(0)" ::: "memory");
             __builtin_amdgcn_s_barrier();
-            if (t + NS - 1 < t1) stage(bnext, tile_at(t + NS - 1));
+            if constexpr (G) map_dma(t + NS + 1);
+            if (t + NS - 1 < t1) stage(gc, bnext, tile_at(t + NS - 1), G ? map_read(t + NS - 1) : 0u);
             bnext = bnext + 1 == NS ? 0 : bnext + 1;
             const char* buf = lds + bcur * a.stage_bytes;
             bcur = bcur + 1 == NS ? 0 : bcur + 1;
@@ -290,6 +363,7 @@
                 });
             }
         }
+        if constexpr (G) asm volatile("s_waitcnt vmcnt(0)" ::: "memory");
         if (!active) return;
 #pragma unroll
         for (int p = 0; p < NP; ++p) {
@@ -311,16 +385,22 @@
         }
     };
     if constexpr (!k16<PREC>) {
-        run(integral_constant<int, 4>{}, integral_constant<int, kDwMaxQ>{});
+        run(integral_constant<int, 4>{}, integral_constant<int, kDwMaxQ>{}, std::false_type{});
     } else {
-        if (np <= 1)
-            run(integral_constant<int, 1>{}, integral_constant<int, 2>{});
-        else if (np <= 4 && nq <= 1)
-            run(integral_constant<int, 4>{}, integral_constant<int, 1>{});
-        else if (np <= 4)
-            run(integral_constant<int, 4>{}, integral_constant<int, 2>{});
+        auto shapes = [&](auto gc) {
+            if (np <= 1)
+                run(integral_constant<int, 1>{}, integral_constant<int, 2>{}, gc);
+            else if (np <= 4 && nq <= 1)
+                run(integral_constant<int, 4>{}, integral_constant<int, 1>{}, gc);
+            else if (np <= 4)
+                run(integral_constant<int, 4>{}, integral_constant<int, 2>{}, gc);
+            else
+                run(integral_constant<int, kDwMaxP>{}, integral_constant<int, kDwMaxQ>{}, gc);
+        };
+        if (gmode)
+            shapes(std::true_type{});
         else
-            run(integral_constant<int, kDwMaxP>{}, integral_constant<int, kDwMaxQ>{});
+            shapes(std::false_type{});
     }
 }
 
@@ -364,9 +444,9 @@
 }
 
 int launch_tile_flags(const float* g_rgb, const float* g_sigma, int64_t M, int dense, int64_t nseg, uint8_t* flags,
-                      uint32_t* blk_count, hipStream_t s) {
+                      uint32_t* blk_count, uint32_t* smask, uint32_t* blk_samples, hipStream_t s) {
     hipLaunchKernelGGL(tile_flags_kernel, dim3(static_cast<unsigned>(nseg * (kSegTiles / 64))), dim3(kTileFlagThreads),
-                       0, s, g_rgb, g_sigma, M, dense, flags, blk_count);
+                       0, s, g_rgb, g_sigma, M, dense, flags, blk_count, smask, blk_samples);
     return check_launch("nr_mlp_backward_dx (tile flags)");
 }
 
diff --git a/robust-nerf_amd/csrc/mlp_fp32.hip b/robust-nerf_amd/csrc/mlp_fp32.hip
--- a/robust-nerf_amd/csrc/mlp_fp32.hip
+++ b/robust-nerf_amd/csrc/mlp_fp32.hip
@@ -378,7 +378,7 @@
     const int tid = threadIdx.x, lane = tid & 63, h = lane >> 5, ml = lane & 31;
     const int wv = __builtin_amdgcn_readfirstlane(tid >> 6);
     static_assert(TPW == 1, "the active-tile selection gives each wave one tile");
-    const TileSel ts = select_tile(a.flags, a.blk_count, a.nseg, a.tiles, kNT / 64, wv);
+    const TileSel ts = select_tile<false>(a.flags, a.blk_count, a.blk_samples, a.nseg, a.tiles, kNT / 64, wv);
     if (ts.idle) {
         finish_tiles(ts, a.nseg, a.tiles, a.dw_list, a.count);
         return;
diff --git a/robust-nerf_amd/csrc/mlp_launch.hpp b/robust-nerf_amd/csrc/mlp_launch.hpp
--- a/robust-nerf_amd/csrc/mlp_launch.hpp
+++ b/robust-nerf_amd/csrc/mlp_launch.hpp
@@ -57,6 +57,7 @@
     int64_t M, tiles;
     const uint8_t* flags;
     const uint32_t* blk_count;
+    const uint32_t* blk_samples;
     int64_t nseg;
     uint32_t* dw_list;
     uint32_t* count;
@@ -105,6 +106,9 @@
     int64_t M, tiles;
     const uint8_t* flags;
     const uint32_t* blk_count;
+    const uint32_t* smask;
+    const uint32_t* blk_samples;
+    uint32_t* map;
     int64_t nseg;
     uint32_t* dw_list;
     uint32_t* count;
@@ -123,6 +127,7 @@
 int input_grads16(const MlpPlan& p, const MlpSizes& z, const char* packed, const float* x, const float* d, float* g_x,
                   float* g_d, const char* ws, int64_t M, hipStream_t s);
 
+
 #ifndef NR_DW_NSTAGE
 #define NR_DW_NSTAGE 4
 #endif
@@ -130,6 +135,7 @@
 constexpr int kDwWaves = kDwThreads / 64;
 static_assert(kDwWaves == kDwMaxWaves, "dW wave shares are planned for 8-wave workgroups");
 
+constexpr int kDwMapRing = 8;
 constexpr int kDwMaxWgs = 256;
 struct DwArgs {
     float* slabs;
@@ -137,7 +143,9 @@
     int64_t tiles;
     const uint32_t* list;
     const uint32_t* count;
+    const uint32_t* map;
     int list_lds;
+    int map_lds;
     int job_chunks[kMaxJobs];
     uint16_t wg_map[kDwMaxWgs];
     int stage_bytes, nstage;
@@ -146,6 +154,7 @@
     int64_t job_slab[kMaxJobs];
     const char* seg_ptr[kMaxJobs][2 * kMaxJobSeg];
     uint8_t seg_blocks[kMaxJobs][2 * kMaxJobSeg];
+    uint8_t seg_saved[kMaxJobs];
     int job_wave[kMaxJobs][kDwWaves];
 };
 static_assert(sizeof(DwArgs) <= 4096, "dW kernel arguments exceed 4 KiB");
@@ -170,7 +179,7 @@
 };
 
 int launch_tile_flags(const float* g_rgb, const float* g_sigma, int64_t M, int dense, int64_t nseg, uint8_t* flags,
-                      uint32_t* blk_count, hipStream_t s);
+                      uint32_t* blk_count, uint32_t* smask, uint32_t* blk_samples, hipStream_t s);
 int launch_dw(int prec, const DwArgs& a, int nwg, size_t lds, hipStream_t s);
 int launch_dw_reduce(const ReduceArgs& a, int max_rows, hipStream_t s);
 
diff --git a/robust-nerf_amd/csrc/mlp_plan.cpp.inc b/robust-nerf_amd/csrc/mlp_plan.cpp.inc
--- a/robust-nerf_amd/csrc/mlp_plan.cpp.inc
+++ b/robust-nerf_amd/csrc/mlp_plan.cpp.inc
@@ -355,6 +355,12 @@
     off = align256(off + s.tiles * 4);
     s.count_off = off;
     off = align256(off + 16);
+    s.smask_off = off;
+    off = align256(off + s.nseg * kSegTiles * 4);
+    s.blksmp_off = off;
+    off = align256(off + s.nseg * (kSegTiles / 64) * 4);
+    s.map_off = off;
+    off = align256(off + s.nseg * kSegTiles * 32 * 4);
     s.ws_bytes = off;
     return s;
 }
diff --git a/robust-nerf_amd/csrc/mlp_plan.hpp b/robust-nerf_amd/csrc/mlp_plan.hpp
--- a/robust-nerf_amd/csrc/mlp_plan.hpp
+++ b/robust-nerf_amd/csrc/mlp_plan.hpp
@@ -13,6 +13,16 @@
 constexpr int kFragBytes = 1024;
 constexpr int kScratchTiles = 64;
 constexpr int kSegTiles = 256;
+#ifndef NR_PACK_PCT
+#define NR_PACK_PCT 85
+#endif
+constexpr uint32_t kPackPct = NR_PACK_PCT;
+constexpr uint32_t kGatherBit = 0x80000000u;
+constexpr uint32_t kFillBit = 0x80000000u;
+__host__ __device__ constexpr uint32_t seg_compact_tiles(uint32_t samples) { return (samples + 31u) / 32u; }
+__host__ __device__ constexpr bool seg_packs(uint32_t active_tiles, uint32_t samples) {
+    return active_tiles > 0 && seg_compact_tiles(samples) * 100u <= kPackPct * active_tiles;
+}
 constexpr int kMaxJobs = kMaxTrunk + 8;
 constexpr int kMaxSeg = 2;
 constexpr int kMaxJobSeg = 4;
@@ -112,6 +122,7 @@
     int64_t slab_off;
     int64_t nseg;
     int64_t flags_off, blkcnt_off, dwlist_off, count_off;
+    int64_t smask_off, blksmp_off, map_off;
     int64_t ws_bytes;
 };
 
diff --git a/robust-nerf_amd/noisy_src/_hip.py b/robust-nerf_amd/noisy_src/_hip.py
--- a/robust-nerf_amd/noisy_src/_hip.py
+++ b/robust-nerf_amd/noisy_src/_hip.py
@@ -89,6 +89,8 @@
     "nr_mlp_backward_dw": (c_i, [_cfg_p, c_i64, c_vp, c_vp, c_vp]),
     "nr_mlp_backward_reduce": (c_i, [_cfg_p, c_i64, c_vp, c_vp, c_vp]),
     "nr_mlp_active_tiles_offset": (c_i64, [_cfg_p, c_i64]),
+    "nr_mlp_executed_tiles_offset": (c_i64, [_cfg_p, c_i64]),
+    "nr_mlp_compact_regions": (c_i, [_cfg_p, c_i64, c_vp]),
     "nr_sumsq_workspace_bytes": (c_i64, []),
     "nr_sumsq": (c_i, [c_vp, c_i64, c_vp, c_vp, c_vp]),
     "nr_adam_step": (c_i, [c_vp, c_vp, c_vp, c_vp, c_i64, c_d, c_d, c_d, c_d, c_i64, c_vp, c_f, c_vp]),
diff --git a/robust-nerf_amd/noisy_src/model.py b/robust-nerf_amd/noisy_src/model.py
--- a/robust-nerf_amd/noisy_src/model.py
+++ b/robust-nerf_amd/noisy_src/model.py
@@ -99,6 +99,9 @@
             if net._tile_counts is not None:
                 off = int(_hip.load().nr_mlp_active_tiles_offset(cfg, M))
                 net._tile_counts.append((M, ws[off:off + 4].view(torch.int32).clone()))
+            if net._executed_counts is not None:
+                off = int(_hip.load().nr_mlp_executed_tiles_offset(cfg, M))
+                net._executed_counts.append((M, ws[off:off + 4].view(torch.int32).clone()))
         else:
             gflat.zero_()
         net._last_gflat = gflat
@@ -176,6 +179,7 @@
         self._last_gflat: Optional[torch.Tensor] = None
         self._grad_ready_hook = None
         self._tile_counts: Optional[list] = None
+        self._executed_counts: Optional[list] = None
         self._tickets = {}
 
     def loss_ticket(self, device) -> torch.Tensor:
```

Result: no change. 881,600 rays/s (median of 2 runs) (-0.0%).
